# reinterpretcat/qwen3-rs

Measured on NVIDIA B200. Metric: decode_tokens_per_s, higher is better.
Workload: dtype int8 weights x int8 activations, int32 group dots, f32 accumulate

## Files before the change

### qwen3_rs_b200/csrc/q3_engine.cu

```cuda
#include "../../include/qwen3_cuda.h"
#include "q3_kernels.cuh"
#include "q3_mega.cuh"
#include "q3_prefill.cuh"
#include "q3_sampler.cuh"
#include <cudaTypedefs.h>

#include <cuda_runtime.h>
#include <fcntl.h>
#include <math.h>
#include <stdarg.h>
#include <stdio.h>
#include <stdlib.h>
#include <string.h>
#include <sys/mman.h>
#include <sys/stat.h>
#include <unistd.h>

#include <string>
#include <vector>

using namespace q3;

static thread_local char g_err[1024] = "";
static int fail(int code, const char *fmt, ...) {
    va_list ap;
    va_start(ap, fmt);
    vsnprintf(g_err, sizeof g_err, fmt, ap);
    va_end(ap);
    return code;
}
#define CK(call)                                                                                        \
    do {                                                                                                \
        cudaError_t e_ = (call);                                                                        \
        if (e_ != cudaSuccess)                                                                          \
            return fail(Q3_ECUDA, "CUDA error %s at %s:%d: %s", cudaGetErrorName(e_), __FILE__, __LINE__, \
                        cudaGetErrorString(e_));                                                        \
    } while (0)

extern "C" const char *q3_last_error(void) { return g_err; }
extern "C" const char *q3_version(void) { return "qwen3cuda 0.1 (sm_100a)"; }

struct DevQT {
    int8_t *q = nullptr;
    float *s = nullptr;
    int rows = 0, K = 0;
    float *sT = nullptr;
    CUtensorMap map{};
    bool has_map = false;
};

struct LayerDev {
    DevQT qkv;
    DevQT wo;
    DevQT w13;
    DevQT w2;
    float *rms_att = nullptr, *rms_ffn = nullptr, *q_ln = nullptr, *k_ln = nullptr;
};

struct q3_handle {
    q3_config cfg{};
    int device = 0;
    int tp_rank = 0, tp_size = 1;
    int n_heads_l = 0, n_kv_l = 0, AH_l = 0, KV_l = 0, H_l = 0, kv_mul = 1;
    int num_sms = 148;
    std::vector<LayerDev> layers;
    DevQT embed, wcls;
    float *rms_final = nullptr;
    float *rope = nullptr;
    float *x = nullptr, *xb = nullptr, *q = nullptr, *hb = nullptr, *logits = nullptr, *attn_part = nullptr;
    unsigned *att_cnt = nullptr;
    int8_t *xq = nullptr, *hq = nullptr;
    float *xs = nullptr, *hs = nullptr;
    float *kc = nullptr, *vc = nullptr;
    int *d_tokpos = nullptr;
    int *d_history = nullptr;
    int history_cap = 0;
    float *h_logits = nullptr;
    int *h_small = nullptr;
    cudaStream_t stream = nullptr;
    cudaGraphExec_t g_fwd[32] = {}, g_greedy[32] = {};
    int exact = 0;
    float *att = nullptr;
    int decode_path = 0;
    int launches_per_step = 0, graph_launches_per_step = 0;
    bool mega_ok = false;
    std::string mega_why;
    MegaArgs margs{};
    unsigned long long bar_base = 0, xbar_base = 0;
    int *d_status = nullptr;
    unsigned long long *part_buf[2] = {nullptr, nullptr};
    unsigned long long *zq = nullptr, *za = nullptr, *zh = nullptr, *zr[2] = {nullptr, nullptr};
    int logits_root = -1;
    bool poisoned = false;
    unsigned long long *d_best = nullptr, *d_bar = nullptr;
    unsigned int *d_flags = nullptr;
    uint8_t *xchg = nullptr;
    size_t xchg_bytes = 0, off_part[2] = {0, 0}, off_best = 0, off_flags = 0, off_logits = 0;
    size_t off_pf_part[2] = {0, 0}, off_pf_ctr = 0;
    int pf_tp_cap = 0;
    PfPeers pf_peers[2]{};
    unsigned long long pf_xbar_count = 0;
    bool tp_connected = false;
    std::vector<void *> peer_maps;
    size_t mega_smem = 0;
    unsigned long long ll_count = 0;
    void *mega_fn = nullptr;
    bool pf_ok = false;
    std::string pf_why;
    __half *pf_kvh = nullptr;
    size_t pf_kvh_rows = 0;
    int pf_cap = 0;
    float *pf_x = nullptr, *pf_q = nullptr, *pf_att = nullptr, *pf_hb = nullptr, *pf_xsT = nullptr, *pf_hsT = nullptr;
    int8_t *pf_xq = nullptr, *pf_hq = nullptr;
    int *pf_tokens = nullptr;
    float samp_temperature = 0.0f, samp_topp = 0.9f;
    unsigned long long *d_rng = nullptr, *d_keys = nullptr;
    float *d_probs = nullptr;
    size_t dev_bytes = 0;
    std::vector<void *> allocs;
};

static int dmalloc(q3_handle *h, void **p, size_t bytes) {
    CK(cudaMalloc(p, bytes ? bytes : 16));
    h->allocs.push_back(*p);
    h->dev_bytes += bytes;
    return 0;
}

struct HostQT {
    const int8_t *q;
    const float *s;
};
struct Ckpt {
    uint8_t *map = nullptr;
    size_t len = 0, off = 0;
    q3_config cfg{};
    const float *rms_att, *rms_ffn, *rms_final, *q_ln, *k_ln;
    HostQT embed, wcls;
    std::vector<HostQT> wq, wk, wv, wo, w1, w2, w3;
    ~Ckpt() {
        if (map) munmap(map, len);
    }
    const void *take(size_t bytes) {
        if (off + bytes > len) return nullptr;
        const void *p = map + off;
        off += bytes;
        return p;
    }
};

static int open_ckpt(const char *path, int ctx_len, Ckpt &c) {
    int fd = open(path, O_RDONLY);
    if (fd < 0) return fail(Q3_EIO, "Failed to open checkpoint: %s", path);
    struct stat st;
    fstat(fd, &st);
    c.len = (size_t)st.st_size;
    void *m = mmap(nullptr, c.len ? c.len : 1, PROT_READ, MAP_PRIVATE, fd, 0);
    close(fd);
    if (m == MAP_FAILED) return fail(Q3_EIO, "Failed to create memory mapping");
    c.map = (uint8_t *)m;
    const int32_t *hd = (const int32_t *)c.take(13 * 4);
    if (!hd) return fail(Q3_EFORMAT, "Insufficient data for config: need 52 bytes, got %zu", c.len);
    if (hd[0] != 0x616a6331)
        return fail(Q3_EFORMAT, "Invalid checkpoint magic number: expected 0x616a6331, got %#x", hd[0]);
    if (hd[1] != 1) return fail(Q3_EFORMAT, "Unsupported checkpoint version: expected 1, got %d", hd[1]);
    const char *names[8] = {"architecture_id", "dim", "n_layers", "n_heads", "n_kv_heads", "vocab_size", "seq_len", "head_dim"};
    int32_t vals[8] = {hd[2], hd[3], hd[5], hd[6], hd[7], hd[8], hd[9], hd[10]};
    for (int i = 0; i < 8; i++)
        if (vals[i] <= 0) return fail(Q3_EFORMAT, "Invalid %s: must be positive, got %d", names[i], vals[i]);
    if (!c.take(256 - 52)) return fail(Q3_EFORMAT, "Cannot skip %d bytes: insufficient data", 256 - 52);
    q3_config &cf = c.cfg;
    cf.architecture_id = hd[2]; cf.dim = hd[3]; cf.hidden_dim = hd[4]; cf.n_layers = hd[5];
    cf.n_heads = hd[6]; cf.n_kv_heads = hd[7]; cf.vocab_size = hd[8]; cf.seq_len = hd[9];
    cf.head_dim = hd[10]; cf.shared_classifier = hd[11] != 0; cf.group_size = hd[12];
    if (ctx_len > 0 && ctx_len < cf.seq_len) cf.seq_len = ctx_len;
    if (cf.architecture_id != 1) return fail(Q3_EFORMAT, "Unknown architecture_id: %d", cf.architecture_id);
    if (cf.hidden_dim <= 0 || cf.group_size <= 0) return fail(Q3_EFORMAT, "Invalid hidden_dim/group_size");

    const int L = cf.n_layers, dim = cf.dim, hdm = cf.head_dim, gs = cf.group_size;
    const size_t AH = (size_t)cf.n_heads * hdm, KV = (size_t)cf.n_kv_heads * hdm, H = cf.hidden_dim, V = cf.vocab_size;
#define TAKE_F32(dst, n, what)                                                         \
    if (!((dst) = (const float *)c.take((size_t)(n) * 4)))                             \
        return fail(Q3_EFORMAT, "Failed to read %s: Insufficient data", what);
    TAKE_F32(c.rms_att, (size_t)L * dim, "attention normalization weights");
    TAKE_F32(c.rms_ffn, (size_t)L * dim, "FFN normalization weights");
    TAKE_F32(c.rms_final, dim, "final normalization weights");
    TAKE_F32(c.q_ln, (size_t)L * hdm, "query layer norm weights");
    TAKE_F32(c.k_ln, (size_t)L * hdm, "key layer norm weights");
    auto take_qts = [&](std::vector<HostQT> &v, int n, size_t size_each, const char *what) -> int {
        v.resize(n);
        for (int i = 0; i < n; i++) {
            v[i].q = (const int8_t *)c.take(size_each);
            v[i].s = (const float *)c.take(size_each / gs * 4);
            if (!v[i].q || !v[i].s)
                return fail(Q3_EFORMAT, "Failed to read quantized tensor %d data (%s): Insufficient data", i, what);
        }
        return 0;
    };
    std::vector<HostQT> one;
    int rc;
    if ((rc = take_qts(one, 1, V * dim, "token embedding"))) return rc;
    c.embed = one[0];
    if ((rc = take_qts(c.wq, L, (size_t)dim * AH, "wq"))) return rc;
    if ((rc = take_qts(c.wk, L, (size_t)dim * KV, "wk"))) return rc;
    if ((rc = take_qts(c.wv, L, (size_t)dim * KV, "wv"))) return rc;
    if ((rc = take_qts(c.wo, L, AH * dim, "wo"))) return rc;
    if ((rc = take_qts(c.w1, L, (size_t)dim * H, "w1"))) return rc;
    if ((rc = take_qts(c.w2, L, H * dim, "w2"))) return rc;
    if ((rc = take_qts(c.w3, L, (size_t)dim * H, "w3"))) return rc;
    if (cf.shared_classifier) c.wcls = c.embed;
    else {
        if ((rc = take_qts(one, 1, (size_t)dim * V, "classifier"))) return rc;
        c.wcls = one[0];
    }
    return 0;
}

struct Stager {
    uint8_t *buf = nullptr;
    size_t cap = 0;
    ~Stager() {
        if (buf) cudaFreeHost(buf);
    }
    int ensure(size_t n) {
        if (n <= cap) return 0;
        if (buf) cudaFreeHost(buf);
        buf = nullptr;
        cap = 0;
        CK(cudaMallocHost((void **)&buf, n));
        cap = n;
        return 0;
    }
};

struct RowPiece {
    HostQT src;
    int src_row0, nrows, srcK;
};
static int upload_rows(q3_handle *h, Stager &st, DevQT &dst, const std::vector<RowPiece> &pieces, int K, int col0,
                       int gs, bool interleave2 = false) {
    int rows = 0;
    for (auto &p : pieces) rows += p.nrows;
    dst.rows = rows;
    dst.K = K;
    const int ng = K / gs;
    size_t qbytes = (size_t)rows * K, sbytes = (size_t)rows * ng * 4;
    int rc;
    if ((rc = dmalloc(h, (void **)&dst.q, qbytes))) return rc;
    if ((rc = dmalloc(h, (void **)&dst.s, sbytes))) return rc;
    if ((rc = st.ensure(qbytes + sbytes))) return rc;
    int8_t *hq = (int8_t *)st.buf;
    float *hs = (float *)(st.buf + qbytes);
    if (interleave2) {
        const RowPiece &a = pieces[0], &b = pieces[1];
        for (int j = 0; j < a.nrows; j++) {
            const RowPiece *pp[2] = {&a, &b};
            for (int t = 0; t < 2; t++) {
                size_t sr = (size_t)pp[t]->src_row0 + j;
                memcpy(hq + (size_t)(2 * j + t) * K, pp[t]->src.q + sr * pp[t]->srcK + col0, K);
                memcpy(hs + (size_t)(2 * j + t) * ng, pp[t]->src.s + sr * (pp[t]->srcK / gs) + col0 / gs, (size_t)ng * 4);
            }
        }
    } else {
        size_t r = 0;
        for (auto &p : pieces) {
            if (p.srcK == K && col0 == 0) {
                memcpy(hq + r * K, p.src.q + (size_t)p.src_row0 * K, (size_t)p.nrows * K);
                memcpy(hs + r * ng, p.src.s + (size_t)p.src_row0 * ng, (size_t)p.nrows * ng * 4);
            } else {
                for (int j = 0; j < p.nrows; j++) {
                    size_t sr = (size_t)p.src_row0 + j;
                    memcpy(hq + (r + j) * K, p.src.q + sr * p.srcK + col0, K);
                    memcpy(hs + (r + j) * ng, p.src.s + sr * (p.srcK / gs) + col0 / gs, (size_t)ng * 4);
                }
            }
            r += p.nrows;
        }
    }
    CK(cudaMemcpy(dst.q, hq, qbytes, cudaMemcpyHostToDevice));
    CK(cudaMemcpy(dst.s, hs, sbytes, cudaMemcpyHostToDevice));
    return 0;
}
static int upload_f32(q3_handle *h, float **dst, const float *src, size_t n) {
    int rc;
    if ((rc = dmalloc(h, (void **)dst, n * 4))) return rc;
    CK(cudaMemcpy(*dst, src, n * 4, cudaMemcpyHostToDevice));
    return 0;
}

#define GS_DISPATCH(gs, CALL)                \
    switch (gs) {                            \
    case 32: { constexpr int GS = 32; CALL; } break;   \
    case 64: { constexpr int GS = 64; CALL; } break;   \
    case 128: { constexpr int GS = 128; CALL; } break; \
    default: break;                          \
    }

template <int GS, int EPI>
static void launch_gemv_t(const q3_handle *h, GemvArgs a, cudaStream_t s) {
    int npairs = a.rows / 2;
    int grid = (npairs + 7) / 8;
    int cap = h->num_sms * 8;
    if (grid > cap) grid = cap;
    if (grid < 1) grid = 1;
    size_t smem = (size_t)a.K + (size_t)(a.K / GS) * 4;
    const bool expref = EPI == EPI_SWIGLU && (h->exact & 16);
    if (h->exact & 2) {
        smem += (size_t)16 * (a.K / GS) * 4;
        if (expref) k_gemv<GS, EPI, true, true><<<grid, 256, smem, s>>>(a);
        else k_gemv<GS, EPI, true, false><<<grid, 256, smem, s>>>(a);
    } else {
        if (expref) k_gemv<GS, EPI, false, true><<<grid, 256, smem, s>>>(a);
        else k_gemv<GS, EPI, false, false><<<grid, 256, smem, s>>>(a);
    }
}
template <int EPI>
static void launch_gemv(const q3_handle *h, const GemvArgs &a, cudaStream_t s) {
    GS_DISPATCH(h->cfg.group_size, (launch_gemv_t<GS, EPI>(h, a, s)));
}

static int launch_norm_quant(const q3_handle *h, const NormQuantArgs &a, cudaStream_t s) {
    if (h->exact & 1) {
        GS_DISPATCH(h->cfg.group_size, (k_rmsnorm_quant<GS, true><<<1, 1024, (size_t)a.n * 4, s>>>(a)));
    } else {
        GS_DISPATCH(h->cfg.group_size, (k_rmsnorm_quant<GS, false><<<1, 1024, 0, s>>>(a)));
    }
    return 1;
}

static int launch_layer(q3_handle *h, int l, bool first_from_embed, cudaStream_t s) {
    const q3_config &c = h->cfg;
    const LayerDev &W = h->layers[l];
    const int gs = c.group_size, dim = c.dim;
    const int *d_token = h->d_tokpos, *d_pos = h->d_tokpos + 1;
    float *kc_l = h->kc + (size_t)l * c.seq_len * h->KV_l;
    float *vc_l = h->vc + (size_t)l * c.seq_len * h->KV_l;
    int n = 0;
    NormQuantArgs na{};
    na.x = h->x; na.w = W.rms_att; na.q = h->xq; na.s = h->xs; na.n = dim;
    if (first_from_embed) { na.embed_q = h->embed.q; na.embed_s = h->embed.s; na.token = d_token; }
    n += launch_norm_quant(h, na, s);
    GemvArgs g{};
    g.wq = W.qkv.q; g.ws = W.qkv.s; g.xq = h->xq; g.xs = h->xs; g.K = dim; g.rows = W.qkv.rows;
    g.q = h->q; g.kc = kc_l; g.vc = vc_l; g.AH = h->AH_l; g.KV = h->KV_l; g.pos = d_pos;
    launch_gemv<EPI_QKV>(h, g, s); n++;
    int nh = h->n_heads_l + h->n_kv_l;
    if (h->exact & 4)
        k_qknorm_rope<true><<<(nh + 3) / 4, 128, 0, s>>>(h->q, kc_l, W.q_ln, W.k_ln, h->rope, d_pos, h->n_heads_l, h->n_kv_l, h->KV_l);
    else
        k_qknorm_rope<false><<<(nh + 3) / 4, 128, 0, s>>>(h->q, kc_l, W.q_ln, W.k_ln, h->rope, d_pos, h->n_heads_l, h->n_kv_l, h->KV_l);
    n++;
    dim3 ag(h->n_kv_l, ATTN_MAX_SPLITS);
    if (h->exact & 8) {
        k_attn_ordered<<<h->n_heads_l, 128, 0, s>>>(h->q, kc_l, vc_l, h->att, h->xb, d_pos, h->KV_l, h->kv_mul, c.seq_len);
        int n4 = h->AH_l / 4, grid = (n4 + 255) / 256;
        GS_DISPATCH(gs, (k_quantize<GS><<<grid, 256, 0, s>>>(h->xb, h->AH_l, h->xq, h->xs)));
        n += 2;
    } else {
    switch (h->kv_mul) {
    case 1: k_attn_partial<1><<<ag, 128, 0, s>>>(h->q, kc_l, vc_l, h->attn_part, d_pos, h->KV_l, h->n_heads_l); break;
    case 2: k_attn_partial<2><<<ag, 128, 0, s>>>(h->q, kc_l, vc_l, h->attn_part, d_pos, h->KV_l, h->n_heads_l); break;
    case 4: k_attn_partial<4><<<ag, 128, 0, s>>>(h->q, kc_l, vc_l, h->attn_part, d_pos, h->KV_l, h->n_heads_l); break;
    case 8: k_attn_partial<8><<<ag, 128, 0, s>>>(h->q, kc_l, vc_l, h->attn_part, d_pos, h->KV_l, h->n_heads_l); break;
    }
    n++;
    GS_DISPATCH(gs, (k_attn_combine_quant<GS><<<h->n_heads_l, 128, 0, s>>>(h->attn_part, d_pos, h->xb, h->xq, h->xs)));
    n++;
    }
    GemvArgs o{};
    o.wq = W.wo.q; o.ws = W.wo.s; o.xq = h->xq; o.xs = h->xs; o.K = h->AH_l; o.rows = dim; o.out = h->x;
    launch_gemv<EPI_RESID>(h, o, s); n++;
    NormQuantArgs nf{};
    nf.x = h->x; nf.w = W.rms_ffn; nf.q = h->xq; nf.s = h->xs; nf.n = dim;
    n += launch_norm_quant(h, nf, s);
    GemvArgs gu{};
    gu.wq = W.w13.q; gu.ws = W.w13.s; gu.xq = h->xq; gu.xs = h->xs; gu.K = dim; gu.rows = W.w13.rows; gu.out = h->hb;
    launch_gemv<EPI_SWIGLU>(h, gu, s); n++;
    {
        int n4 = h->H_l / 4, grid = (n4 + 255) / 256;
        GS_DISPATCH(gs, (k_quantize<GS><<<grid, 256, 0, s>>>(h->hb, h->H_l, h->hq, h->hs)));
        n++;
    }
    GemvArgs dn{};
    dn.wq = W.w2.q; dn.ws = W.w2.s; dn.xq = h->hq; dn.xs = h->hs; dn.K = h->H_l; dn.rows = dim; dn.out = h->x;
    launch_gemv<EPI_RESID>(h, dn, s); n++;
    return n;
}

static int launch_head(q3_handle *h, cudaStream_t s) {
    const q3_config &c = h->cfg;
    NormQuantArgs na{};
    na.x = h->x; na.w = h->rms_final; na.q = h->xq; na.s = h->xs; na.n = c.dim; na.write_normed = 1;
    int n = launch_norm_quant(h, na, s);
    GemvArgs g{};
    g.wq = h->wcls.q; g.ws = h->wcls.s; g.xq = h->xq; g.xs = h->xs; g.K = c.dim; g.rows = c.vocab_size; g.out = h->logits;
    launch_gemv<EPI_STORE>(h, g, s); n++;
    return n;
}

static int launch_argmax(q3_handle *h, bool feedback, cudaStream_t s) {
    int *tp = h->d_tokpos;
    k_argmax<<<1, 1024, 0, s>>>(h->logits, h->cfg.vocab_size, tp + 2, feedback ? tp : nullptr, feedback ? tp + 1 : nullptr,
                                feedback ? h->d_history : nullptr, tp + 3);
    return 1;
}

static int launch_step(q3_handle *h, bool argmax, bool feedback, cudaStream_t s) {
    int n = 0;
    for (int l = 0; l < h->cfg.n_layers; l++) n += launch_layer(h, l, l == 0, s);
    n += launch_head(h, s);
    if (argmax) n += launch_argmax(h, feedback, s);
    return n;
}

static int build_graphs(q3_handle *h) {
    const int ex = h->exact;
    for (int which = 0; which < 2; which++) {
        cudaGraphExec_t *slot = which ? &h->g_greedy[ex] : &h->g_fwd[ex];
        cudaGraph_t g;
        CK(cudaStreamBeginCapture(h->stream, cudaStreamCaptureModeThreadLocal));
        int n = launch_step(h, which == 1, which == 1, h->stream);
        cudaError_t e = cudaStreamEndCapture(h->stream, &g);
        if (e != cudaSuccess) return fail(Q3_ECUDA, "graph capture failed: %s", cudaGetErrorString(e));
        if (!*slot) CK(cudaGraphInstantiate(slot, g, 0));
        CK(cudaGraphDestroy(g));
        if (which == 1) h->launches_per_step = n;
    }
    return 0;
}

template <class K>
static int allow_smem(K kernel, int bytes) {
    CK(cudaFuncSetAttribute(kernel, cudaFuncAttributeMaxDynamicSharedMemorySize, bytes));
    return 0;
}
static int prepare_exact_kernels() {
    int rc;
    if ((rc = allow_smem(k_rmsnorm_quant<32, true>, 65536))) return rc;
    if ((rc = allow_smem(k_rmsnorm_quant<64, true>, 65536))) return rc;
    if ((rc = allow_smem(k_rmsnorm_quant<128, true>, 65536))) return rc;
#define ALLOW_GEMV(GS)                                                      \
    if ((rc = allow_smem(k_gemv<GS, EPI_STORE, true, false>, 131072))) return rc;  \
    if ((rc = allow_smem(k_gemv<GS, EPI_QKV, true, false>, 131072))) return rc;    \
    if ((rc = allow_smem(k_gemv<GS, EPI_RESID, true, false>, 131072))) return rc;  \
    if ((rc = allow_smem(k_gemv<GS, EPI_SWIGLU, true, false>, 131072))) return rc; \
    if ((rc = allow_smem(k_gemv<GS, EPI_SWIGLU, true, true>, 131072))) return rc;  \
    if ((rc = allow_smem(k_gemv<GS, EPI_STORE, false, false>, 98304))) return rc;  \
    if ((rc = allow_smem(k_gemv<GS, EPI_QKV, false, false>, 98304))) return rc;    \
    if ((rc = allow_smem(k_gemv<GS, EPI_RESID, false, false>, 98304))) return rc;  \
    if ((rc = allow_smem(k_gemv<GS, EPI_SWIGLU, false, false>, 98304))) return rc; \
    if ((rc = allow_smem(k_gemv<GS, EPI_SWIGLU, false, true>, 98304))) return rc;
    ALLOW_GEMV(32)
    ALLOW_GEMV(64)
    ALLOW_GEMV(128)
#undef ALLOW_GEMV
    return 0;
}

static int pick_n_kt(int K, int gs) {
    for (int n = (K + MEGA_MAX_KT - 1) / MEGA_MAX_KT; n <= 64; n++)
        if (K % (n * gs) == 0 && (K / n) % 16 == 0 && K / n <= MEGA_MAX_KT) return n;
    return 0;
}

template <int GS>
static void *mega_kernel_for(int kvmul) {
    switch (kvmul) {
    case 1: return (void *)k_mega_decode<GS, 1>;
    case 2: return (void *)k_mega_decode<GS, 2>;
    case 4: return (void *)k_mega_decode<GS, 4>;
    case 8: return (void *)k_mega_decode<GS, 8>;
    }
    return nullptr;
}

static int build_stream(q3_handle *h, MegaGemv &g, const std::vector<const DevQT *> &src, int units, int K, bool pair) {
    const int gs = h->cfg.group_size;
    g.units = units;
    g.K = K;
    g.n_kt = pick_n_kt(K, gs);
    if (!g.n_kt) return fail(Q3_EUNSUPPORTED, "no K tiling for K=%d gs=%d", K, gs);
    g.KT = K / g.n_kt;
    g.G = g.KT / gs;
    g.tile_bytes = g.KT + ((4 * g.G + 15) & ~15);
    const size_t rows = (size_t)units * (pair ? 2 : 1);
    g.layer_stride = (long long)(rows * g.n_kt * g.tile_bytes);
    uint8_t *buf = nullptr;
    int rc;
    if ((rc = dmalloc(h, (void **)&buf, (size_t)g.layer_stride * src.size()))) return rc;
    g.base = buf;
    for (size_t l = 0; l < src.size(); l++) {
        dim3 grid(units, g.n_kt);
        GS_DISPATCH(gs, (k_build_stream<GS><<<grid, 256, 0, h->stream>>>(src[l]->q, src[l]->s, buf + l * g.layer_stride, units, K,
                                                                        g.n_kt, h->num_sms, pair ? 1 : 0)));
    }
    CK(cudaGetLastError());
    return 0;
}

static PFN_cuTensorMapEncodeTiled_v12000 get_encode_fn();
static int make_map_kv(CUtensorMap *map, const float *base, size_t rows, int KV_l) {
    auto enc = get_encode_fn();
    if (!enc) return fail(Q3_ECUDA, "cuTensorMapEncodeTiled unavailable");
    cuuint64_t dims[2] = {(cuuint64_t)KV_l, (cuuint64_t)rows};
    cuuint64_t strides[1] = {(cuuint64_t)KV_l * 4};
    cuuint32_t box[2] = {(cuuint32_t)HEAD_DIM, (cuuint32_t)MEGA_KV_ROWS};
    cuuint32_t estr[2] = {1, 1};
    CUresult r = enc(map, CU_TENSOR_MAP_DATA_TYPE_FLOAT32, 2, const_cast<float *>(base), dims, strides, box, estr, CU_TENSOR_MAP_INTERLEAVE_NONE,
                     CU_TENSOR_MAP_SWIZZLE_NONE, CU_TENSOR_MAP_L2_PROMOTION_L2_128B, CU_TENSOR_MAP_FLOAT_OOB_FILL_NONE);
    if (r != CUDA_SUCCESS) return fail(Q3_ECUDA, "cuTensorMapEncodeTiled (KV cache) failed (%d) rows %zu KV %d", (int)r, rows, KV_l);
    return 0;
}

static int build_mega(q3_handle *h, const float *rms_att_all, const float *rms_ffn_all, const float *q_ln_all, const float *k_ln_all) {
    const q3_config &c = h->cfg;
    const int gs = c.group_size, L = c.n_layers, dim = c.dim;
    h->mega_ok = false;
    if (dim > MEGA_MAX_KT) { h->mega_why = "dim > 4096 (QKV/gate-up/lm_head phases need a single K tile)"; return 0; }
    if (!pick_n_kt(h->AH_l, gs) || !pick_n_kt(h->H_l, gs)) { h->mega_why = "no K tiling for o_proj/down"; return 0; }
    if (h->AH_l > 16384 || h->H_l > 16384 || dim > 16384) { h->mega_why = "activation vector > 16384"; return 0; }
    if (c.vocab_size % h->tp_size) { h->mega_why = "vocab not divisible by tp"; return 0; }
    if (h->layers[0].qkv.rows < h->num_sms || h->H_l < h->num_sms) { h->mega_why = "fewer qkv rows / FFN units than SMs"; return 0; }
    if (!get_encode_fn()) { h->mega_why = "cuTensorMapEncodeTiled unavailable"; return 0; }
    MegaArgs &a = h->margs;
    a = MegaArgs{};
    {
        int rck;
        if ((rck = make_map_kv(&a.map_k, h->kc, (size_t)L * c.seq_len, h->KV_l))) return rck;
        if ((rck = make_map_kv(&a.map_v, h->vc, (size_t)L * c.seq_len, h->KV_l))) return rck;
    }
    a.dim = dim; a.n_layers = L; a.n_heads_l = h->n_heads_l; a.n_kv_l = h->n_kv_l; a.AH_l = h->AH_l; a.KV_l = h->KV_l;
    a.H_l = h->H_l; a.seq_len = c.seq_len; a.tp_rank = h->tp_rank; a.tp_size = h->tp_size;
    a.vocab_l = c.vocab_size / h->tp_size;
    a.vocab_row0 = a.vocab_l * h->tp_rank;
    int rc;
    std::vector<const DevQT *> v;
    for (auto &W : h->layers) v.push_back(&W.qkv);
    if ((rc = build_stream(h, a.g[PH_QKV], v, h->layers[0].qkv.rows, dim, false))) return rc;
    v.clear();
    for (auto &W : h->layers) v.push_back(&W.wo);
    if ((rc = build_stream(h, a.g[PH_O], v, dim, h->AH_l, false))) return rc;
    v.clear();
    for (auto &W : h->layers) v.push_back(&W.w13);
    if ((rc = build_stream(h, a.g[PH_GU], v, h->H_l, dim, true))) return rc;
    v.clear();
    for (auto &W : h->layers) v.push_back(&W.w2);
    if ((rc = build_stream(h, a.g[PH_DN], v, dim, h->H_l, false))) return rc;
    DevQT head_slice = h->wcls;
    head_slice.q = h->wcls.q + (size_t)a.vocab_row0 * dim;
    head_slice.s = h->wcls.s + (size_t)a.vocab_row0 * (dim / gs);
    v.assign(1, &head_slice);
    if ((rc = build_stream(h, a.g[PH_HEAD], v, a.vocab_l, dim, false))) return rc;
    CK(cudaStreamSynchronize(h->stream));
    float *p;
    if ((rc = upload_f32(h, &p, rms_att_all, (size_t)L * dim))) return rc; a.rms_att = p;
    if ((rc = upload_f32(h, &p, rms_ffn_all, (size_t)L * dim))) return rc; a.rms_ffn = p;
    if ((rc = upload_f32(h, &p, q_ln_all, (size_t)L * HEAD_DIM))) return rc; a.q_ln = p;
    if ((rc = upload_f32(h, &p, k_ln_all, (size_t)L * HEAD_DIM))) return rc; a.k_ln = p;
    a.rms_final = h->rms_final;
    a.embed_q = h->embed.q; a.embed_s = h->embed.s; a.rope = h->rope; a.kc = h->kc; a.vc = h->vc;
    for (int i = 0; i < 2; i++) h->part_buf[i] = (unsigned long long *)(h->xchg + h->off_part[i]);
    {
        struct { unsigned long long **p; size_t words; } zones[] = {
            {&h->zq, (size_t)h->AH_l + 2 * (size_t)h->KV_l},
            {&h->za, (size_t)h->AH_l / 4 + (size_t)h->AH_l / gs},
            {&h->zh, (size_t)h->H_l},
            {&h->zr[0], (size_t)dim},
            {&h->zr[1], (size_t)dim}};
        for (auto &z : zones) {
            if ((rc = dmalloc(h, (void **)z.p, (z.words + 2) * 8))) return rc;
            CK(cudaMemset(*z.p, 0, (z.words + 2) * 8));
        }
    }
    h->d_best = (unsigned long long *)(h->xchg + h->off_best);
    h->d_flags = (unsigned int *)(h->xchg + h->off_flags);
    if ((rc = dmalloc(h, (void **)&h->d_bar, 64))) return rc;
    CK(cudaMemset(h->d_bar, 0, 64));
    if ((rc = dmalloc(h, (void **)&h->d_status, 64))) return rc;
    CK(cudaMemset(h->d_status, 0, 64));
    int *d_status = h->d_status;
    a.x = h->x;
    a.zq = h->zq; a.za = h->za; a.zh = h->zh; a.zr[0] = h->zr[0]; a.zr[1] = h->zr[1];
    a.attn_part = h->attn_part; a.att_cnt = h->att_cnt;
    a.bar = h->d_bar; a.status = d_status; a.tokpos = h->d_tokpos; a.history = h->d_history;
    for (int r = 0; r < MEGA_MAX_TP; r++) {
        a.part[0][r] = h->part_buf[0]; a.part[1][r] = h->part_buf[1];
        a.logits[r] = h->logits; a.best[r] = h->d_best; a.xbar[r] = (unsigned long long *)h->d_flags;
    }
    GS_DISPATCH(gs, (h->mega_fn = mega_kernel_for<GS>(h->kv_mul)));
    if (!h->mega_fn) { h->mega_why = "no kernel for this GQA factor"; return 0; }
    const size_t slot = (size_t)MEGA_GW * (MEGA_MAX_KT + 4 * (MEGA_MAX_KT / gs));
    h->mega_smem = MEGA_NSTAGE * slot + MEGA_SCRATCH + 1024 + MEGA_MAX_KT * 4;
    CK(cudaFuncSetAttribute(h->mega_fn, cudaFuncAttributeMaxDynamicSharedMemorySize, (int)h->mega_smem));
    int occ = 0;
    CK(cudaOccupancyMaxActiveBlocksPerMultiprocessor(&occ, h->mega_fn, MEGA_THREADS, h->mega_smem));
    if (occ < 1) { h->mega_why = "megakernel does not fit on an SM"; return 0; }
    h->mega_ok = true;
    return 0;
}

static int launch_mega(q3_handle *h, int l0, int l1, bool from_embed, bool run_head, bool feedback, bool gather) {
    MegaArgs a = h->margs;
    a.layer0 = l0; a.layer1 = l1; a.from_embed = from_embed; a.run_head = run_head; a.feedback = feedback;
    a.gather_logits = h->tp_size > 1 ? (h->logits_root >= 0 ? (1 << h->logits_root) : (gather ? (1 << h->tp_size) - 1 : 0)) : 0;
    a.bar_base = h->bar_base;
    a.xbar_base = h->xbar_base;
    if (h->poisoned) return fail(Q3_ECOMM, "tensor-parallel handle is unusable after a timed-out wait (ranks may have diverged): destroy and re-create every rank");
    const int nbar = run_head ? 1 : 0;
    const int nx = h->tp_size > 1 ? nbar : 0;
    a.ll_base = (unsigned)(h->ll_count % 0xFFFFFFFFull);
    h->ll_count += (unsigned long long)MEGA_EDGES * (unsigned)(l1 - l0 + 1);
    void *params[] = {&a};
    CK(cudaLaunchCooperativeKernel(h->mega_fn, dim3(h->num_sms), dim3(MEGA_THREADS), params, h->mega_smem, h->stream));
    h->bar_base += (unsigned long long)(nbar - nx) * h->num_sms;
    h->xbar_base += (unsigned long long)nx * h->tp_size * h->num_sms;
    return 0;
}

static int check_tok_pos(const q3_handle *h, int token, int pos);
static int mega_status_async(q3_handle *h) {
    if (!h->d_status || h->decode_path != 1) return 0;
    CK(cudaMemcpyAsync(h->h_small + 16, h->d_status, 4, cudaMemcpyDeviceToHost, h->stream));
    return 0;
}
static int mega_check(q3_handle *h, bool queued = false) {
    if (!h->d_status || h->decode_path != 1) return 0;
    int code = 0;
    if (queued) code = h->h_small[16];
    else CK(cudaMemcpy(&code, h->d_status, 4, cudaMemcpyDeviceToHost));
    if (code) {
        cudaMemset(h->d_status, 0, 64);
        if (h->tp_size > 1) {
            h->poisoned = true;
        } else {
            h->bar_base = 0;
            h->xbar_base = 0;
            cudaMemset(h->d_bar, 0, 64);
            cudaMemset(h->d_flags, 0, 64 * 4);
            if (h->att_cnt) cudaMemset(h->att_cnt, 0, (size_t)h->cfg.n_layers * h->n_kv_l * 4);
        }
        return fail(Q3_ECUDA, "persistent decode kernel: a wait timed out (status %d: 1 grid barrier, 2 stage ring, 3 cross-GPU barrier, 4 producer order, "
                              "6-10 flagged exchange: 6 o/down rows, 7 attention output, 8 SwiGLU outputs, 9 qkv rows, 10 TP partials; 11 prefill cross-GPU barrier)%s", code,
                    h->tp_size > 1 ? "; tensor-parallel handle poisoned" : "");
    }
    return 0;
}
extern "C" int q3_debug_profile(q3_handle *h, int token, int pos, unsigned long long *out, size_t out_words, int *n_rows_out,
                                int *n_events_out) {
    if (!h) return fail(Q3_EINVAL, "null argument");
    if (n_rows_out) *n_rows_out = 3 * h->num_sms;
    if (n_events_out) *n_events_out = MEGA_PROF_EVENTS;
    if (!out) return out_words == 0 ? Q3_OK : fail(Q3_EINVAL, "null argument");
    if (!h->mega_ok) return fail(Q3_EUNSUPPORTED, "persistent decode kernel unavailable: %s", h->mega_why.c_str());
    if (out_words < (size_t)3 * h->num_sms * MEGA_PROF_EVENTS)
        return fail(Q3_EINVAL, "profile buffer too small: %zu words, need %zu", out_words, (size_t)3 * h->num_sms * MEGA_PROF_EVENTS);
    if (int rc0 = check_tok_pos(h, token, pos)) return rc0;
    CK(cudaSetDevice(h->device));
    h->h_small[0] = token; h->h_small[1] = pos; h->h_small[2] = 0; h->h_small[3] = 0;
    CK(cudaMemcpyAsync(h->d_tokpos, h->h_small, 16, cudaMemcpyHostToDevice, h->stream));
    unsigned long long *d = nullptr;
    size_t bytes = (size_t)3 * h->num_sms * MEGA_PROF_EVENTS * 8;
    CK(cudaMalloc((void **)&d, bytes));
    CK(cudaMemsetAsync(d, 0, bytes, h->stream));
    h->margs.prof = d;
    int rc = launch_mega(h, 0, h->cfg.n_layers, true, true, false, false);
    h->margs.prof = nullptr;
    if (!rc) {
        cudaError_t e = cudaStreamSynchronize(h->stream);
        if (e == cudaSuccess) e = cudaMemcpy(out, d, bytes, cudaMemcpyDeviceToHost);
        if (e != cudaSuccess) rc = fail(Q3_ECUDA, "profile run failed: %s", cudaGetErrorString(e));
    }
    cudaFree(d);
    if (!rc) rc = mega_check(h);
    return rc;
}
extern "C" int q3_num_sms(const q3_handle *h) { return h ? h->num_sms : 0; }
extern "C" int q3_debug_set_epoch(q3_handle *h, unsigned long long exchanges_issued) {
    if (!h) return fail(Q3_EINVAL, "null handle");
    h->ll_count = exchanges_issued;
    return Q3_OK;
}

static inline bool use_mega(const q3_handle *h) { return h->decode_path == 1 && h->mega_ok && !h->exact; }
static int tp_ready(const q3_handle *h) {
    if (h->tp_size > 1 && !h->tp_connected) return fail(Q3_ECOMM, "tensor-parallel handle used before q3_tp_connect");
    if (h->tp_size > 1 && !use_mega(h)) return fail(Q3_EUNSUPPORTED, "under tensor parallelism only the persistent fast path is available");
    return 0;
}

static PFN_cuTensorMapEncodeTiled_v12000 get_encode_fn() {
    static PFN_cuTensorMapEncodeTiled_v12000 fn = nullptr;
    if (!fn) {
        void *p = nullptr;
        cudaDriverEntryPointQueryResult qres;
        if (cudaGetDriverEntryPoint("cuTensorMapEncodeTiled", &p, cudaEnableDefault, &qres) == cudaSuccess && qres == cudaDriverEntryPointSuccess)
            fn = (PFN_cuTensorMapEncodeTiled_v12000)p;
    }
    return fn;
}
static int make_map_i8(CUtensorMap *map, const void *base, int rows, int K) {
    auto enc = get_encode_fn();
    if (!enc) return fail(Q3_ECUDA, "cuTensorMapEncodeTiled unavailable");
    cuuint64_t dims[2] = {(cuuint64_t)K, (cuuint64_t)rows};
    cuuint64_t strides[1] = {(cuuint64_t)K};
    cuuint32_t box[2] = {(cuuint32_t)PF_BK, (cuuint32_t)PF_BM};
    cuuint32_t estr[2] = {1, 1};
    CUresult r = enc(map, CU_TENSOR_MAP_DATA_TYPE_UINT8, 2, const_cast<void *>(base), dims, strides, box, estr,
                     CU_TENSOR_MAP_INTERLEAVE_NONE, CU_TENSOR_MAP_SWIZZLE_128B, CU_TENSOR_MAP_L2_PROMOTION_L2_256B,
                     CU_TENSOR_MAP_FLOAT_OOB_FILL_NONE);
    if (r != CUDA_SUCCESS) return fail(Q3_ECUDA, "cuTensorMapEncodeTiled failed (%d) rows %d K %d", (int)r, rows, K);
    return 0;
}

static int make_map_scales(CUtensorMap *map, const float *base, int groups, int cols) {
    auto enc = get_encode_fn();
    if (!enc) return fail(Q3_ECUDA, "cuTensorMapEncodeTiled unavailable");
    cuuint64_t dims[2] = {(cuuint64_t)cols, (cuuint64_t)groups};
    cuuint64_t strides[1] = {(cuuint64_t)cols * 4};
    cuuint32_t box[2] = {128, 2};
    cuuint32_t estr[2] = {1, 1};
    CUresult r = enc(map, CU_TENSOR_MAP_DATA_TYPE_FLOAT32, 2, const_cast<float *>(base), dims, strides, box, estr, CU_TENSOR_MAP_INTERLEAVE_NONE,
                     CU_TENSOR_MAP_SWIZZLE_NONE, CU_TENSOR_MAP_L2_PROMOTION_L2_128B, CU_TENSOR_MAP_FLOAT_OOB_FILL_NONE);
    if (r != CUDA_SUCCESS) return fail(Q3_ECUDA, "cuTensorMapEncodeTiled (scales) failed (%d) groups %d cols %d", (int)r, groups, cols);
    return 0;
}

template <int GS, int EPI, bool EXACT>
static int launch_gemm_q8_t(const CUtensorMap &mx, const CUtensorMap &mw, const PrefillGemmArgs &a, cudaStream_t s) {
    static bool attr = false;
    if (!attr) {
        CK(cudaFuncSetAttribute(k_gemm_q8<GS, EPI, EXACT>, cudaFuncAttributeMaxDynamicSharedMemorySize, PF_SMEM));
        attr = true;
    }
    static int num_sms = 0;
    if (!num_sms) {
        int dev = 0;
        CK(cudaGetDevice(&dev));
        CK(cudaDeviceGetAttribute(&num_sms, cudaDevAttrMultiProcessorCount, dev));
    }
    CUtensorMap mxs, mws;
    int rc;
    if ((rc = make_map_scales(&mxs, a.xsT, a.K / GS, a.Tpad)) || (rc = make_map_scales(&mws, a.wsT, a.K / GS, a.N))) return rc;
    const int tiles = (a.N / PF_BN) * (a.Tpad / PF_BM);
    k_gemm_q8<GS, EPI, EXACT><<<tiles < num_sms ? tiles : num_sms, PF_THREADS, PF_SMEM, s>>>(mx, mw, mxs, mws, a);
    return 0;
}
template <int EPI>
static int launch_gemm_q8(int gs, const CUtensorMap &mx, const CUtensorMap &mw, const PrefillGemmArgs &a, cudaStream_t s, int mode = 0) {
    int rc = 0;
    if (mode == 0) {
        GS_DISPATCH(gs, (rc = launch_gemm_q8_t<GS, EPI, false>(mx, mw, a, s)));
    } else if (mode == 1 && EPI == PF_EPI_STORE) {
        GS_DISPATCH(gs, (rc = launch_gemm_q8_t<GS, PF_EPI_STORE, true>(mx, mw, a, s)));
    } else {
        return fail(Q3_EINVAL, "prefill GEMM mode %d: 0 = fast drain, 1 = exact drain (plain store epilogue only)", mode);
    }
    return rc;
}

static int prefill_prepare_tensor(q3_handle *h, DevQT &t) {
    if (t.has_map) return 0;
    const int gs = h->cfg.group_size, ng = t.K / gs;
    int rc;
    if ((rc = dmalloc(h, (void **)&t.sT, (size_t)ng * t.rows * 4))) return rc;
    dim3 grid((ng + 31) / 32, (t.rows + 31) / 32);
    k_transpose_f32<<<grid, dim3(32, 8), 0, h->stream>>>(t.s, t.sT, t.rows, ng);
    CK(cudaGetLastError());
    if ((rc = make_map_i8(&t.map, t.q, t.rows, t.K))) return rc;
    t.has_map = true;
    return 0;
}

static int prefill_init(q3_handle *h) {
    const q3_config &c = h->cfg;
    h->pf_ok = false;
    if (c.dim % 128 || h->AH_l % 128 || h->H_l % 128 || h->layers[0].qkv.rows % 128 || (2 * h->H_l) % 128) {
        h->pf_why = "matrix dimensions must be multiples of 128";
        return 0;
    }
    if ((c.dim / c.group_size) % 2 || (h->AH_l / c.group_size) % 2 || (h->H_l / c.group_size) % 2) {
        h->pf_why = "the tensor-core GEMM hands accumulators over in pairs: rows need an even number of quantisation groups";
        return 0;
    }
    if (!get_encode_fn()) { h->pf_why = "cuTensorMapEncodeTiled unavailable"; return 0; }
    CK(cudaFuncSetAttribute(k_pf_attention_h<1>, cudaFuncAttributeMaxDynamicSharedMemorySize, PFH_SMEM));
    CK(cudaFuncSetAttribute(k_pf_attention_h<2>, cudaFuncAttributeMaxDynamicSharedMemorySize, PFH_SMEM));
    CK(cudaFuncSetAttribute(k_pf_attention_h<4>, cudaFuncAttributeMaxDynamicSharedMemorySize, PFH_SMEM));
    CK(cudaFuncSetAttribute(k_pf_attention_h<8>, cudaFuncAttributeMaxDynamicSharedMemorySize, PFH_SMEM));
    int rc;
    for (auto &W : h->layers) {
        if ((rc = prefill_prepare_tensor(h, W.qkv))) return rc;
        if ((rc = prefill_prepare_tensor(h, W.wo))) return rc;
        if ((rc = prefill_prepare_tensor(h, W.w13))) return rc;
        if ((rc = prefill_prepare_tensor(h, W.w2))) return rc;
    }
    CK(cudaStreamSynchronize(h->stream));
    h->pf_ok = true;
    return 0;
}

static void prefill_release(q3_handle *h) {
    if (h->pf_kvh) cudaFree(h->pf_kvh);
    h->pf_kvh = nullptr;
    h->pf_kvh_rows = 0;
    void **ps[] = {(void **)&h->pf_x, (void **)&h->pf_q, (void **)&h->pf_att, (void **)&h->pf_hb, (void **)&h->pf_xsT, (void **)&h->pf_hsT,
                   (void **)&h->pf_xq, (void **)&h->pf_hq, (void **)&h->pf_tokens};
    for (void **p : ps) {
        if (*p) cudaFree(*p);
        *p = nullptr;
    }
    h->pf_cap = 0;
}
static int prefill_reserve(q3_handle *h, int T) {
    const int Tpad = (T + 127) / 128 * 128;
    if (Tpad <= h->pf_cap) return 0;
    const q3_config &c = h->cfg;
    const int gs = c.group_size, dim = c.dim, AH = h->AH_l, H = h->H_l;
    const int maxd = AH > dim ? AH : dim;
    prefill_release(h);
    struct { void **p; size_t bytes; } want[] = {
        {(void **)&h->pf_x, (size_t)Tpad * dim * 4},          {(void **)&h->pf_q, (size_t)Tpad * AH * 4},
        {(void **)&h->pf_att, (size_t)Tpad * AH * 4},         {(void **)&h->pf_hb, (size_t)Tpad * H * 4},
        {(void **)&h->pf_xsT, (size_t)(maxd / gs) * Tpad * 4}, {(void **)&h->pf_hsT, (size_t)(H / gs) * Tpad * 4},
        {(void **)&h->pf_xq, (size_t)Tpad * maxd},            {(void **)&h->pf_hq, (size_t)Tpad * H},
        {(void **)&h->pf_tokens, (size_t)Tpad * 4}};
    for (auto &w : want) {
        cudaError_t e = cudaMalloc(w.p, w.bytes);
        if (e != cudaSuccess) {
            *w.p = nullptr;
            prefill_release(h);
            cudaGetLastError();
            return fail(Q3_ECUDA, "prefill buffers for %d tokens: %s", T, cudaGetErrorString(e));
        }
    }
    CK(cudaMemset(h->pf_xq, 0, (size_t)Tpad * maxd));
    CK(cudaMemset(h->pf_hq, 0, (size_t)Tpad * H));
    CK(cudaMemset(h->pf_xsT, 0, (size_t)(maxd / gs) * Tpad * 4));
    CK(cudaMemset(h->pf_hsT, 0, (size_t)(H / gs) * Tpad * 4));
    h->pf_cap = Tpad;
    return 0;
}

static int prefill_tp_rowparallel(q3_handle *h, int which, const CUtensorMap &mx, const CUtensorMap &mw, PrefillGemmArgs g, int T) {
    int rc;
    g.out = const_cast<float *>(h->pf_peers[which].part[h->tp_rank]);
    if ((rc = launch_gemm_q8<PF_EPI_STORE>(h->cfg.group_size, mx, mw, g, h->stream))) return rc;
    h->pf_xbar_count++;
    k_pf_xbarrier<<<1, 32, 0, h->stream>>>(h->pf_peers[which], h->tp_size, h->tp_rank, h->pf_xbar_count * (unsigned long long)h->tp_size, h->d_status);
    const size_t n4 = (size_t)T * h->cfg.dim / 4;
    if (h->tp_size > 2) {
        k_pf_reduce_scatter<<<h->num_sms * 2, 256, 0, h->stream>>>(h->pf_peers[which], g.out, h->tp_size, h->tp_rank, n4);
        h->pf_xbar_count++;
        k_pf_xbarrier<<<1, 32, 0, h->stream>>>(h->pf_peers[which], h->tp_size, h->tp_rank, h->pf_xbar_count * (unsigned long long)h->tp_size, h->d_status);
        k_pf_allgather_resid<<<dim3(h->num_sms / 2, h->tp_size), 256, 0, h->stream>>>(h->pf_x, h->pf_peers[which], h->tp_size, n4);
    } else {
        k_pf_allreduce_resid<<<h->num_sms * 4, 256, 0, h->stream>>>(h->pf_x, h->pf_peers[which], h->tp_size, n4);
    }
    CK(cudaGetLastError());
    return 0;
}

static int prefill_run(q3_handle *h, const int *tokens_host, int T, int pos0);
static int prefill_chunks(q3_handle *h, const int *tokens_host, int n, int pos0) {
    const int cap = h->tp_size > 1 ? h->pf_tp_cap : n;
    for (int off = 0; off < n; off += cap) {
        int rc = prefill_run(h, tokens_host + off, n - off < cap ? n - off : cap, pos0 + off);
        if (rc) return rc;
    }
    return 0;
}

static int prefill_run(q3_handle *h, const int *tokens_host, int T, int pos0) {
    const q3_config &c = h->cfg;
    const int gs = c.group_size, dim = c.dim, AH = h->AH_l, KV = h->KV_l, H = h->H_l;
    int rc;
    if ((rc = prefill_reserve(h, T))) return rc;
    if ((size_t)pos0 + T > h->pf_kvh_rows) {
        if (h->pf_kvh) cudaFree(h->pf_kvh);
        h->pf_kvh = nullptr;
        h->pf_kvh_rows = 0;
        const size_t rows = ((size_t)pos0 + T + 127) / 128 * 128;
        cudaError_t e = cudaMalloc((void **)&h->pf_kvh, 4 * rows * KV * sizeof(__half));
        if (e != cudaSuccess) {
            h->pf_kvh = nullptr;
            cudaGetLastError();
            return fail(Q3_ECUDA, "prefill K/V split buffer for %zu rows: %s", rows, cudaGetErrorString(e));
        }
        h->pf_kvh_rows = rows;
    }
    const int Tpad = (T + 127) / 128 * 128;
    cudaStream_t s = h->stream;
    CK(cudaMemcpyAsync(h->pf_tokens, tokens_host, (size_t)T * 4, cudaMemcpyHostToDevice, s));
    CUtensorMap mx_dim, mx_ah, mx_h;
    if ((rc = make_map_i8(&mx_dim, h->pf_xq, Tpad, dim))) return rc;
    if ((rc = make_map_i8(&mx_ah, h->pf_xq, Tpad, AH))) return rc;
    if ((rc = make_map_i8(&mx_h, h->pf_hq, Tpad, H))) return rc;
    for (int l = 0; l < c.n_layers; l++) {
        LayerDev &W = h->layers[l];
        float *kc_l = h->kc + (size_t)l * c.seq_len * KV;
        float *vc_l = h->vc + (size_t)l * c.seq_len * KV;
        if (dim <= 4096) {
            GS_DISPATCH(gs, (k_pf_norm_quant<GS, 4><<<T, 256, 0, s>>>(h->pf_x, W.rms_att, h->pf_xq, h->pf_xsT, dim, Tpad,
                                                                     l == 0 ? h->embed.q : nullptr, h->embed.s, h->pf_tokens, 0)));
        } else {
            GS_DISPATCH(gs, (k_pf_norm_quant<GS><<<T, 256, 0, s>>>(h->pf_x, W.rms_att, h->pf_xq, h->pf_xsT, dim, Tpad,
                                                                  l == 0 ? h->embed.q : nullptr, h->embed.s, h->pf_tokens, 0)));
        }
        PrefillGemmArgs g{};
        g.T = T; g.Tpad = Tpad; g.K = dim; g.N = W.qkv.rows; g.wsT = W.qkv.sT; g.xsT = h->pf_xsT;
        g.q = h->pf_q; g.kc = kc_l; g.vc = vc_l; g.AH = AH; g.KV = KV; g.pos0 = pos0;
        if ((rc = launch_gemm_q8<PF_EPI_QKV>(gs, mx_dim, W.qkv.map, g, s))) return rc;
        dim3 rg((h->n_heads_l + h->n_kv_l + 3) / 4, T);
        k_pf_qknorm_rope<<<rg, 128, 0, s>>>(h->pf_q, kc_l, W.q_ln, W.k_ln, h->rope, pos0, h->n_heads_l, h->n_kv_l, AH, KV);
        const size_t rows = (size_t)pos0 + T, plane = h->pf_kvh_rows * KV;
        k_pf_split_kv<<<h->num_sms * 4, 256, 0, s>>>(kc_l, vc_l, h->pf_kvh, rows * KV / 4, plane);
        const int bq = PFH_R / h->kv_mul;
        dim3 ag(h->n_kv_l, (T + bq - 1) / bq);
        switch (h->kv_mul) {
        case 1: k_pf_attention_h<1><<<ag, 128, PFH_SMEM, s>>>(h->pf_q, h->pf_kvh, plane, h->pf_att, T, pos0, AH, KV); break;
        case 2: k_pf_attention_h<2><<<ag, 128, PFH_SMEM, s>>>(h->pf_q, h->pf_kvh, plane, h->pf_att, T, pos0, AH, KV); break;
        case 4: k_pf_attention_h<4><<<ag, 128, PFH_SMEM, s>>>(h->pf_q, h->pf_kvh, plane, h->pf_att, T, pos0, AH, KV); break;
        case 8: k_pf_attention_h<8><<<ag, 128, PFH_SMEM, s>>>(h->pf_q, h->pf_kvh, plane, h->pf_att, T, pos0, AH, KV); break;
        }
        GS_DISPATCH(gs, (k_pf_quantize<GS><<<T, 256, 0, s>>>(h->pf_att, h->pf_xq, h->pf_xsT, AH, Tpad)));
        PrefillGemmArgs o{};
        o.T = T; o.Tpad = Tpad; o.K = AH; o.N = dim; o.wsT = W.wo.sT; o.xsT = h->pf_xsT; o.out = h->pf_x; o.ld_out = dim;
        if (h->tp_size == 1) {
            if ((rc = launch_gemm_q8<PF_EPI_RESID>(gs, mx_ah, W.wo.map, o, s))) return rc;
        } else if ((rc = prefill_tp_rowparallel(h, 0, mx_ah, W.wo.map, o, T))) return rc;
        if (dim <= 4096) {
            GS_DISPATCH(gs, (k_pf_norm_quant<GS, 4><<<T, 256, 0, s>>>(h->pf_x, W.rms_ffn, h->pf_xq, h->pf_xsT, dim, Tpad, nullptr, nullptr, nullptr, 0)));
        } else {
            GS_DISPATCH(gs, (k_pf_norm_quant<GS><<<T, 256, 0, s>>>(h->pf_x, W.rms_ffn, h->pf_xq, h->pf_xsT, dim, Tpad, nullptr, nullptr, nullptr, 0)));
        }
        PrefillGemmArgs gu{};
        gu.T = T; gu.Tpad = Tpad; gu.K = dim; gu.N = W.w13.rows; gu.wsT = W.w13.sT; gu.xsT = h->pf_xsT; gu.out = h->pf_hb; gu.ld_out = H;
        if ((rc = launch_gemm_q8<PF_EPI_SWIGLU>(gs, mx_dim, W.w13.map, gu, s))) return rc;
        GS_DISPATCH(gs, (k_pf_quantize<GS><<<T, 256, 0, s>>>(h->pf_hb, h->pf_hq, h->pf_hsT, H, Tpad)));
        PrefillGemmArgs dn{};
        dn.T = T; dn.Tpad = Tpad; dn.K = H; dn.N = dim; dn.wsT = W.w2.sT; dn.xsT = h->pf_hsT; dn.out = h->pf_x; dn.ld_out = dim;
        if (h->tp_size == 1) {
            if ((rc = launch_gemm_q8<PF_EPI_RESID>(gs, mx_h, W.w2.map, dn, s))) return rc;
        } else if ((rc = prefill_tp_rowparallel(h, 1, mx_h, W.w2.map, dn, T))) return rc;
    }
    CK(cudaMemcpyAsync(h->x, h->pf_x + (size_t)(T - 1) * dim, (size_t)dim * 4, cudaMemcpyDeviceToDevice, s));
    CK(cudaGetLastError());
    return 0;
}

static int create_impl(const char *path, int ctx_len, int device, int tp_rank, int tp_size, q3_handle **out) {
    if (!path || !out) return fail(Q3_EINVAL, "null argument");
    if (tp_size < 1 || tp_rank < 0 || tp_rank >= tp_size) return fail(Q3_EINVAL, "bad tp rank/size %d/%d", tp_rank, tp_size);
    *out = nullptr;
    Ckpt ck;
    int rc = open_ckpt(path, ctx_len, ck);
    if (rc) return rc;
    const q3_config &c = ck.cfg;
    const int gs = c.group_size;
    if (c.head_dim != HEAD_DIM) return fail(Q3_EUNSUPPORTED, "head_dim %d unsupported (kernels are built for 128)", c.head_dim);
    if (gs != 32 && gs != 64 && gs != 128) return fail(Q3_EUNSUPPORTED, "group_size %d unsupported (32/64/128)", gs);
    if (c.n_heads % c.n_kv_heads) return fail(Q3_EUNSUPPORTED, "n_heads %% n_kv_heads != 0");
    int kv_mul = c.n_heads / c.n_kv_heads;
    if (kv_mul != 1 && kv_mul != 2 && kv_mul != 4 && kv_mul != 8) return fail(Q3_EUNSUPPORTED, "GQA factor %d unsupported", kv_mul);
    if (c.dim % 128 || c.hidden_dim % 128) return fail(Q3_EUNSUPPORTED, "dim/hidden_dim must be multiples of 128");
    if (c.dim > 16384 || c.hidden_dim > 65536) return fail(Q3_EUNSUPPORTED, "dim/hidden_dim too large");
    if (c.n_kv_heads % tp_size || (c.hidden_dim / tp_size) % gs || c.hidden_dim % tp_size)
        return fail(Q3_EUNSUPPORTED, "tp_size %d does not divide kv heads / hidden groups", tp_size);
    if (c.vocab_size % 2) return fail(Q3_EUNSUPPORTED, "odd vocab_size");

    int ndev = 0;
    CK(cudaGetDeviceCount(&ndev));
    if (device < 0 || device >= ndev) return fail(Q3_EINVAL, "device %d out of range (%d visible)", device, ndev);
    CK(cudaSetDevice(device));
    q3_handle *h = new q3_handle();
    h->cfg = c;
    h->device = device;
    h->tp_rank = tp_rank;
    h->tp_size = tp_size;
    h->kv_mul = kv_mul;
    h->n_heads_l = c.n_heads / tp_size;
    h->n_kv_l = c.n_kv_heads / tp_size;
    h->AH_l = h->n_heads_l * HEAD_DIM;
    h->KV_l = h->n_kv_l * HEAD_DIM;
    h->H_l = c.hidden_dim / tp_size;
    cudaDeviceProp prop;
    cudaGetDeviceProperties(&prop, device);
    h->num_sms = prop.multiProcessorCount;

    auto guard_fail = [&](int code) {
        q3_destroy(h);
        return code;
    };
#define TRY(x)                         \
    do {                               \
        int rc_ = (x);                 \
        if (rc_) return guard_fail(rc_); \
    } while (0)
#define CKH(call)                                                                                         \
    do {                                                                                                  \
        cudaError_t e_ = (call);                                                                          \
        if (e_ != cudaSuccess)                                                                            \
            return guard_fail(fail(Q3_ECUDA, "CUDA error %s at %s:%d: %s", cudaGetErrorName(e_), __FILE__, \
                                   __LINE__, cudaGetErrorString(e_)));                                    \
    } while (0)

    CKH(cudaStreamCreateWithFlags(&h->stream, cudaStreamNonBlocking));
    const int L = c.n_layers, dim = c.dim, H = c.hidden_dim;
    const int AH = c.n_heads * HEAD_DIM;
    Stager st;
    h->layers.resize(L);
    const int r = tp_rank;
    for (int l = 0; l < L; l++) {
        LayerDev &W = h->layers[l];
        TRY(upload_rows(h, st, W.qkv,
                        {{ck.wq[l], r * h->AH_l, h->AH_l, dim}, {ck.wk[l], r * h->KV_l, h->KV_l, dim}, {ck.wv[l], r * h->KV_l, h->KV_l, dim}},
                        dim, 0, gs));
        TRY(upload_rows(h, st, W.wo, {{ck.wo[l], 0, dim, AH}}, h->AH_l, r * h->AH_l, gs));
        TRY(upload_rows(h, st, W.w13, {{ck.w1[l], r * h->H_l, h->H_l, dim}, {ck.w3[l], r * h->H_l, h->H_l, dim}}, dim, 0, gs, true));
        TRY(upload_rows(h, st, W.w2, {{ck.w2[l], 0, dim, H}}, h->H_l, r * h->H_l, gs));
        TRY(upload_f32(h, &W.rms_att, ck.rms_att + (size_t)l * dim, dim));
        TRY(upload_f32(h, &W.rms_ffn, ck.rms_ffn + (size_t)l * dim, dim));
        TRY(upload_f32(h, &W.q_ln, ck.q_ln + (size_t)l * HEAD_DIM, HEAD_DIM));
        TRY(upload_f32(h, &W.k_ln, ck.k_ln + (size_t)l * HEAD_DIM, HEAD_DIM));
    }
    TRY(upload_rows(h, st, h->embed, {{ck.embed, 0, c.vocab_size, dim}}, dim, 0, gs));
    if (c.shared_classifier) h->wcls = h->embed;
    else TRY(upload_rows(h, st, h->wcls, {{ck.wcls, 0, c.vocab_size, dim}}, dim, 0, gs));
    TRY(upload_f32(h, &h->rms_final, ck.rms_final, dim));

    {
        size_t n = (size_t)c.seq_len * HEAD_DIM;
        std::vector<float> tab(n);
        const int half = HEAD_DIM / 2;
        std::vector<float> freq(half);
        for (int i = 0; i < half; i++) freq[i] = powf(1e6f, -((float)i) / (float)half);
        for (int p = 0; p < c.seq_len; p++)
            for (int i = 0; i < half; i++) {
                float ang = (float)p * freq[i];
                tab[(size_t)p * HEAD_DIM + 2 * i] = cosf(ang);
                tab[(size_t)p * HEAD_DIM + 2 * i + 1] = sinf(ang);
            }
        TRY(upload_f32(h, &h->rope, tab.data(), n));
    }
    const int maxd = (h->AH_l > dim ? h->AH_l : dim);
    TRY(dmalloc(h, (void **)&h->x, (size_t)dim * 4));
    TRY(dmalloc(h, (void **)&h->xb, (size_t)maxd * 4));
    TRY(dmalloc(h, (void **)&h->q, (size_t)h->AH_l * 4));
    TRY(dmalloc(h, (void **)&h->hb, (size_t)h->H_l * 4));
    {
        auto al = [](size_t v) { return (v + 255) & ~(size_t)255; };
        size_t o = 0;
        h->off_part[0] = o; o = al(o + (size_t)tp_size * dim * 8);
        h->off_part[1] = o; o = al(o + (size_t)tp_size * dim * 8);
        h->off_best = o; o = al(o + (size_t)tp_size * h->num_sms * 8);
        h->off_flags = o; o = al(o + 64 * 4);
        h->off_logits = o; o = al(o + (size_t)c.vocab_size * 4);
        if (tp_size > 1) {
            h->pf_tp_cap = c.seq_len < 2048 ? (c.seq_len + 127) / 128 * 128 : 2048;
            h->off_pf_ctr = o; o = al(o + 64);
            for (int i = 0; i < 2; i++) { h->off_pf_part[i] = o; o = al(o + (size_t)h->pf_tp_cap * dim * 4); }
        }
        h->xchg_bytes = o;
        TRY(dmalloc(h, (void **)&h->xchg, o));
        CKH(cudaMemset(h->xchg, 0, o));
        h->logits = (float *)(h->xchg + h->off_logits);
    }
    TRY(dmalloc(h, (void **)&h->xq, (size_t)maxd));
    TRY(dmalloc(h, (void **)&h->xs, (size_t)(maxd / gs + 1) * 4));
    TRY(dmalloc(h, (void **)&h->hq, (size_t)h->H_l));
    TRY(dmalloc(h, (void **)&h->hs, (size_t)(h->H_l / gs + 1) * 4));
    TRY(dmalloc(h, (void **)&h->attn_part, (size_t)h->n_heads_l * ATTN_MAX_SPLITS * ATTN_PART_STRIDE * 4));
    TRY(dmalloc(h, (void **)&h->att_cnt, (size_t)h->cfg.n_layers * h->n_kv_l * 4));
    CKH(cudaMemset(h->att_cnt, 0, (size_t)h->cfg.n_layers * h->n_kv_l * 4));
    TRY(dmalloc(h, (void **)&h->att, (size_t)h->n_heads_l * c.seq_len * 4));
    TRY(prepare_exact_kernels());
    size_t kvn = (size_t)L * c.seq_len * h->KV_l;
    TRY(dmalloc(h, (void **)&h->kc, kvn * 4));
    TRY(dmalloc(h, (void **)&h->vc, kvn * 4));
    CKH(cudaMemset(h->kc, 0, kvn * 4));
    CKH(cudaMemset(h->vc, 0, kvn * 4));
    h->history_cap = c.seq_len + 8;
    TRY(dmalloc(h, (void **)&h->d_tokpos, 16 * 4));
    TRY(dmalloc(h, (void **)&h->d_history, (size_t)h->history_cap * 4));
    CKH(cudaMemset(h->d_tokpos, 0, 16 * 4));
    CKH(cudaMemset(h->x, 0, (size_t)dim * 4));
    CKH(cudaMallocHost((void **)&h->h_logits, (size_t)c.vocab_size * 4));
    CKH(cudaMallocHost((void **)&h->h_small, 64 * 4));
    CKH(cudaDeviceSynchronize());
    TRY(build_graphs(h));
    h->graph_launches_per_step = h->launches_per_step;
    TRY(build_mega(h, ck.rms_att, ck.rms_ffn, ck.q_ln, ck.k_ln));
    if (h->mega_ok) {
        h->decode_path = 1;
        h->launches_per_step = 1;
    }
    TRY(prefill_init(h));
    CKH(cudaDeviceSynchronize());
    *out = h;
    return Q3_OK;
}

extern "C" int q3_create(const char *path, int ctx_len, int device, q3_handle **out) {
    return create_impl(path, ctx_len, device, 0, 1, out);
}
extern "C" int q3_create_tp(const char *path, int ctx_len, int device, int tp_rank, int tp_size, q3_handle **out) {
    if (tp_size > MEGA_MAX_TP) return fail(Q3_EUNSUPPORTED, "tp_size %d > %d", tp_size, MEGA_MAX_TP);
    int rc = create_impl(path, ctx_len, device, tp_rank, tp_size, out);
    if (rc) return rc;
    if (tp_size > 1 && !(*out)->mega_ok) {
        std::string why = (*out)->mega_why;
        q3_destroy(*out);
        *out = nullptr;
        return fail(Q3_EUNSUPPORTED, "tensor parallelism needs the persistent decode kernel, unavailable here: %s", why.c_str());
    }
    return Q3_OK;
}

struct TpBlob {
    uint32_t magic, rank, tp_size, device;
    uint64_t pid, raw_ptr, bytes;
    cudaIpcMemHandle_t ipc;
};
static_assert(sizeof(TpBlob) <= 256, "blob too large");
extern "C" size_t q3_tp_blob_size(void) { return 256; }

extern "C" int q3_tp_export(q3_handle *h, void *blob_out) {
    if (!h || !blob_out) return fail(Q3_EINVAL, "null argument");
    CK(cudaSetDevice(h->device));
    memset(blob_out, 0, 256);
    TpBlob b{};
    b.magic = 0x51335450;
    b.rank = h->tp_rank; b.tp_size = h->tp_size; b.device = h->device;
    b.pid = (uint64_t)getpid();
    b.raw_ptr = (uint64_t)(uintptr_t)h->xchg;
    b.bytes = h->xchg_bytes;
    CK(cudaIpcGetMemHandle(&b.ipc, h->xchg));
    memcpy(blob_out, &b, sizeof b);
    return Q3_OK;
}

extern "C" int q3_tp_connect(q3_handle *h, const void *blobs) {
    if (!h || !blobs) return fail(Q3_EINVAL, "null argument");
    if (h->tp_size == 1) return Q3_OK;
    CK(cudaSetDevice(h->device));
    MegaArgs &a = h->margs;
    for (int r = 0; r < h->tp_size; r++) {
        TpBlob b;
        memcpy(&b, (const uint8_t *)blobs + (size_t)r * 256, sizeof b);
        if (b.magic != 0x51335450 || (int)b.rank != r || (int)b.tp_size != h->tp_size || b.bytes != h->xchg_bytes)
            return fail(Q3_ECOMM, "rank %d: bad exchange blob (rank %u, tp %u, %llu bytes)", r, b.rank, b.tp_size,
                        (unsigned long long)b.bytes);
        uint8_t *base = nullptr;
        if (r == h->tp_rank) {
            base = h->xchg;
        } else if (b.pid == (uint64_t)getpid()) {
            int can = 0;
            CK(cudaDeviceCanAccessPeer(&can, h->device, (int)b.device));
            if (!can) return fail(Q3_ECOMM, "device %d cannot access peer device %u", h->device, b.device);
            cudaError_t e = cudaDeviceEnablePeerAccess((int)b.device, 0);
            if (e != cudaSuccess && e != cudaErrorPeerAccessAlreadyEnabled)
                return fail(Q3_ECOMM, "cudaDeviceEnablePeerAccess: %s", cudaGetErrorString(e));
            cudaGetLastError();
            base = (uint8_t *)(uintptr_t)b.raw_ptr;
        } else {
            void *p = nullptr;
            cudaError_t e = cudaIpcOpenMemHandle(&p, b.ipc, cudaIpcMemLazyEnablePeerAccess);
            if (e != cudaSuccess) return fail(Q3_ECOMM, "cudaIpcOpenMemHandle(rank %d): %s", r, cudaGetErrorString(e));
            h->peer_maps.push_back(p);
            base = (uint8_t *)p;
        }
        a.part[0][r] = (unsigned long long *)(base + h->off_part[0]);
        a.part[1][r] = (unsigned long long *)(base + h->off_part[1]);
        a.best[r] = (unsigned long long *)(base + h->off_best);
        a.xbar[r] = (unsigned long long *)(base + h->off_flags);
        a.logits[r] = (float *)(base + h->off_logits);
        for (int i = 0; i < 2; i++) {
            h->pf_peers[i].part[r] = (const float *)(base + h->off_pf_part[i]);
            h->pf_peers[i].ctr[r] = (unsigned long long *)(base + h->off_pf_ctr);
        }
    }
    h->tp_connected = true;
    return Q3_OK;
}

extern "C" int q3_tp_set_logits_root(q3_handle *h, int root) {
    if (!h) return fail(Q3_EINVAL, "null handle");
    if (root >= h->tp_size) return fail(Q3_EINVAL, "logits root %d outside the tensor-parallel group of %d", root, h->tp_size);
    h->logits_root = root < 0 ? -1 : root;
    return Q3_OK;
}

extern "C" void q3_destroy(q3_handle *h) {
    if (!h) return;
    cudaSetDevice(h->device);
    if (h->stream) cudaStreamSynchronize(h->stream);
    for (int e = 0; e < 32; e++) {
        if (h->g_fwd[e]) cudaGraphExecDestroy(h->g_fwd[e]);
        if (h->g_greedy[e]) cudaGraphExecDestroy(h->g_greedy[e]);
    }
    prefill_release(h);
    for (void *p : h->peer_maps) cudaIpcCloseMemHandle(p);
    for (void *p : h->allocs) cudaFree(p);
    if (h->h_logits) cudaFreeHost(h->h_logits);
    if (h->h_small) cudaFreeHost(h->h_small);
    if (h->stream) cudaStreamDestroy(h->stream);
    delete h;
}

extern "C" const q3_config *q3_get_config(const q3_handle *h) { return h ? &h->cfg : nullptr; }
extern "C" const float *q3_logits_device(const q3_handle *h) { return h ? h->logits : nullptr; }
extern "C" float *q3_logits_host(q3_handle *h) { return h ? h->h_logits : nullptr; }
extern "C" int q3_launches_per_step(const q3_handle *h) { return h ? h->launches_per_step : 0; }
extern "C" int q3_set_decode_path(q3_handle *h, int path) {
    if (!h) return fail(Q3_EINVAL, "null handle");
    if (path != 0 && path != 1) return fail(Q3_EINVAL, "decode path %d unknown", path);
    if (path == 0 && h->tp_size > 1) return fail(Q3_EUNSUPPORTED, "the multi-kernel path has no tensor-parallel exchange");
    if (path == 1 && !h->mega_ok)
        return fail(Q3_EUNSUPPORTED, "persistent decode kernel unavailable for this shape: %s", h->mega_why.c_str());
    h->decode_path = path;
    h->launches_per_step = path == 1 ? 1 : h->graph_launches_per_step;
    return Q3_OK;
}

extern "C" int q3_set_exact_mask(q3_handle *h, int mask) {
    if (!h) return fail(Q3_EINVAL, "null handle");
    if (mask < 0 || mask > 31) return fail(Q3_EINVAL, "exact mask %d outside 0..31", mask);
    CK(cudaSetDevice(h->device));
    if (mask && h->tp_size > 1) return fail(Q3_EUNSUPPORTED, "exact mode is single-GPU");
    if (mask && h->cfg.dim > 16384) return fail(Q3_EUNSUPPORTED, "exact mode needs dim <= 16384");
    h->exact = mask;
    if (!h->g_fwd[h->exact]) return build_graphs(h);
    return Q3_OK;
}
extern "C" int q3_set_exact(q3_handle *h, int on) { return q3_set_exact_mask(h, on ? 31 : 0); }

static int check_tok_pos(const q3_handle *h, int token, int pos) {
    if (!h) return fail(Q3_EINVAL, "null handle");
    if (int rc = tp_ready(h)) return rc;
    if (token < 0 || token >= h->cfg.vocab_size)
        return fail(Q3_EINVAL, "index out of bounds: token %d >= vocab_size %d", token, h->cfg.vocab_size);
    if (pos < 0 || pos >= h->cfg.seq_len)
        return fail(Q3_EINVAL, "index out of bounds: pos %d >= seq_len %d", pos, h->cfg.seq_len);
    return 0;
}

static int set_tok_pos(q3_handle *h, int token, int pos) {
    h->h_small[0] = token;
    h->h_small[1] = pos;
    h->h_small[2] = 0;
    h->h_small[3] = 0;
    CK(cudaMemcpyAsync(h->d_tokpos, h->h_small, 16, cudaMemcpyHostToDevice, h->stream));
    return 0;
}

extern "C" int q3_forward(q3_handle *h, int token, int pos, float *logits_host) {
    int rc = check_tok_pos(h, token, pos);
    if (rc) return rc;
    CK(cudaSetDevice(h->device));
    if ((rc = set_tok_pos(h, token, pos))) return rc;
    if (logits_host && h->tp_size > 1 && h->logits_root >= 0 && h->logits_root != h->tp_rank)
        return fail(Q3_EINVAL, "rank %d asked for logits but the logits root is rank %d", h->tp_rank, h->logits_root);
    if (use_mega(h)) {
        if ((rc = launch_mega(h, 0, h->cfg.n_layers, true, true, false, logits_host != nullptr))) return rc;
    } else {
        CK(cudaGraphLaunch(h->g_fwd[h->exact], h->stream));
    }
    if ((rc = mega_status_async(h))) return rc;
    if (logits_host) {
        CK(cudaMemcpyAsync(h->h_logits, h->logits, (size_t)h->cfg.vocab_size * 4, cudaMemcpyDeviceToHost, h->stream));
        CK(cudaStreamSynchronize(h->stream));
        if (logits_host != h->h_logits) memcpy(logits_host, h->h_logits, (size_t)h->cfg.vocab_size * 4);
    } else {
        CK(cudaStreamSynchronize(h->stream));
    }
    return mega_check(h, true);
}

extern "C" int q3_forward_argmax(q3_handle *h, int token, int pos, int *next_token) {
    int rc = check_tok_pos(h, token, pos);
    if (rc) return rc;
    if (!next_token) return fail(Q3_EINVAL, "null next_token");
    CK(cudaSetDevice(h->device));
    if ((rc = set_tok_pos(h, token, pos))) return rc;
    if (use_mega(h)) {
        if ((rc = launch_mega(h, 0, h->cfg.n_layers, true, true, true, false))) return rc;
    } else {
        CK(cudaGraphLaunch(h->g_greedy[h->exact], h->stream));
    }
    CK(cudaMemcpyAsync(h->h_small + 8, h->d_tokpos + 2, 4, cudaMemcpyDeviceToHost, h->stream));
    if ((rc = mega_status_async(h))) return rc;
    CK(cudaStreamSynchronize(h->stream));
    *next_token = h->h_small[8];
    return mega_check(h, true);
}

extern "C" int q3_decode_greedy(q3_handle *h, int first_token, int pos0, int n, int *tokens_out) {
    int rc = check_tok_pos(h, first_token, pos0);
    if (rc) return rc;
    if (n < 0 || pos0 + n > h->cfg.seq_len) return fail(Q3_EINVAL, "pos0 + n = %d exceeds seq_len %d", pos0 + n, h->cfg.seq_len);
    if (n > h->history_cap) return fail(Q3_EINVAL, "n too large");
    CK(cudaSetDevice(h->device));
    if ((rc = set_tok_pos(h, first_token, pos0))) return rc;
    for (int i = 0; i < n; i++) {
        if (use_mega(h)) {
            if ((rc = launch_mega(h, 0, h->cfg.n_layers, true, true, true, false))) return rc;
        } else {
            CK(cudaGraphLaunch(h->g_greedy[h->exact], h->stream));
        }
    }
    if (tokens_out && n > 0) {
        CK(cudaMemcpyAsync(tokens_out, h->d_history, (size_t)n * 4, cudaMemcpyDeviceToHost, h->stream));
    }
    CK(cudaStreamSynchronize(h->stream));
    return mega_check(h);
}

static size_t next_pow2(size_t n) {
    size_t p = 1;
    while (p < n) p <<= 1;
    return p;
}
extern "C" int q3_sampler_set(q3_handle *h, float temperature, float topp, unsigned long long rng_seed) {
    if (!h) return fail(Q3_EINVAL, "null handle");
    if (!(temperature >= 0.0f)) return fail(Q3_EINVAL, "Temperature must be non-negative");
    if (!(topp >= 0.0f && topp <= 1.0f)) return fail(Q3_EINVAL, "Top-p must be between 0.0 and 1.0");
    CK(cudaSetDevice(h->device));
    int rc;
    if (!h->d_rng) {
        if ((rc = dmalloc(h, (void **)&h->d_rng, 64))) return rc;
        if ((rc = dmalloc(h, (void **)&h->d_probs, (size_t)h->cfg.vocab_size * 4))) return rc;
        if ((rc = dmalloc(h, (void **)&h->d_keys, next_pow2((size_t)h->cfg.vocab_size) * 8))) return rc;
    }
    h->samp_temperature = temperature;
    h->samp_topp = topp;
    CK(cudaMemcpyAsync(h->d_rng, &rng_seed, 8, cudaMemcpyHostToDevice, h->stream));
    CK(cudaStreamSynchronize(h->stream));
    return Q3_OK;
}
extern "C" int q3_sampler_state(q3_handle *h, unsigned long long *rng_state_out) {
    if (!h || !rng_state_out) return fail(Q3_EINVAL, "null argument");
    if (!h->d_rng) return fail(Q3_EINVAL, "q3_sampler_set has not been called");
    CK(cudaSetDevice(h->device));
    CK(cudaStreamSynchronize(h->stream));
    CK(cudaMemcpy(rng_state_out, h->d_rng, 8, cudaMemcpyDeviceToHost));
    return Q3_OK;
}
extern "C" int q3_sampler_skip(q3_handle *h, int n_draws) {
    if (!h || n_draws < 0) return fail(Q3_EINVAL, "bad argument");
    if (!h->d_rng) return fail(Q3_EINVAL, "q3_sampler_set has not been called");
    CK(cudaSetDevice(h->device));
    if (h->samp_temperature != 0.0f && n_draws > 0) k_rng_skip<<<1, 1, 0, h->stream>>>(h->d_rng, n_draws);
    CK(cudaGetLastError());
    return Q3_OK;
}
static int launch_sampled_step(q3_handle *h, bool feedback) {
    int rc;
    const bool greedy = h->samp_temperature == 0.0f;
    if (use_mega(h)) {
        if ((rc = launch_mega(h, 0, h->cfg.n_layers, true, true, greedy && feedback, !greedy))) return rc;
    } else if (greedy) {
        if (feedback) CK(cudaGraphLaunch(h->g_greedy[h->exact], h->stream));
        else {
            CK(cudaGraphLaunch(h->g_fwd[h->exact], h->stream));
            launch_argmax(h, false, h->stream);
        }
    } else {
        CK(cudaGraphLaunch(h->g_fwd[h->exact], h->stream));
    }
    if (!greedy) {
        SampleArgs a{};
        a.logits = h->logits; a.n = h->cfg.vocab_size; a.temperature = h->samp_temperature; a.topp = h->samp_topp;
        a.rng_state = h->d_rng; a.p = h->d_probs; a.keys = h->d_keys; a.token_out = h->d_tokpos + 2;
        if (feedback) { a.token_feedback = h->d_tokpos; a.pos_advance = h->d_tokpos + 1; a.history = h->d_history; a.history_idx = h->d_tokpos + 3; }
        k_sample<<<1, SAMPLE_THREADS, 0, h->stream>>>(a);
        CK(cudaGetLastError());
    }
    return 0;
}
extern "C" int q3_forward_sample(q3_handle *h, int token, int pos, int *next_token) {
    int rc = check_tok_pos(h, token, pos);
    if (rc) return rc;
    if (!next_token) return fail(Q3_EINVAL, "null next_token");
    if (!h->d_rng) return fail(Q3_EINVAL, "q3_sampler_set has not been called");
    CK(cudaSetDevice(h->device));
    if ((rc = set_tok_pos(h, token, pos))) return rc;
    if ((rc = launch_sampled_step(h, false))) return rc;
    CK(cudaMemcpyAsync(h->h_small + 8, h->d_tokpos + 2, 4, cudaMemcpyDeviceToHost, h->stream));
    if ((rc = mega_status_async(h))) return rc;
    CK(cudaStreamSynchronize(h->stream));
    *next_token = h->h_small[8];
    return mega_check(h, true);
}
extern "C" int q3_decode_sample(q3_handle *h, int first_token, int pos0, int n, int *tokens_out) {
    int rc = check_tok_pos(h, first_token, pos0);
    if (rc) return rc;
    if (n < 0 || pos0 + n > h->cfg.seq_len) return fail(Q3_EINVAL, "pos0 + n = %d exceeds seq_len %d", pos0 + n, h->cfg.seq_len);
    if (n > h->history_cap) return fail(Q3_EINVAL, "n too large");
    if (!h->d_rng) return fail(Q3_EINVAL, "q3_sampler_set has not been called");
    CK(cudaSetDevice(h->device));
    if ((rc = set_tok_pos(h, first_token, pos0))) return rc;
    for (int i = 0; i < n; i++)
        if ((rc = launch_sampled_step(h, true))) return rc;
    if (tokens_out && n > 0) CK(cudaMemcpyAsync(tokens_out, h->d_history, (size_t)n * 4, cudaMemcpyDeviceToHost, h->stream));
    CK(cudaStreamSynchronize(h->stream));
    return mega_check(h);
}

extern "C" int q3_bench_decode(q3_handle *h, int first_token, int pos0, int steps, float *ms_out) {
    int rc = check_tok_pos(h, first_token, pos0);
    if (rc) return rc;
    if (steps < 1 || pos0 + steps > h->cfg.seq_len) return fail(Q3_EINVAL, "pos0 + steps exceeds seq_len");
    CK(cudaSetDevice(h->device));
    if ((rc = set_tok_pos(h, first_token, pos0))) return rc;
    cudaEvent_t e0, e1;
    CK(cudaEventCreate(&e0));
    CK(cudaEventCreate(&e1));
    CK(cudaStreamSynchronize(h->stream));
    CK(cudaEventRecord(e0, h->stream));
    for (int i = 0; i < steps; i++) {
        if (use_mega(h)) {
            if ((rc = launch_mega(h, 0, h->cfg.n_layers, true, true, true, false))) return rc;
        } else {
            CK(cudaGraphLaunch(h->g_greedy[h->exact], h->stream));
        }
    }
    CK(cudaEventRecord(e1, h->stream));
    CK(cudaEventSynchronize(e1));
    float ms = 0;
    CK(cudaEventElapsedTime(&ms, e0, e1));
    cudaEventDestroy(e0);
    cudaEventDestroy(e1);
    if (ms_out) *ms_out = ms;
    return mega_check(h);
}

extern "C" int q3_bench_kernel(q3_handle *h, int kind, int pos, int reps, float *ms_out, int *launches_out,
                               double *bytes_out) {
    if (!h || kind < 0 || kind > 5 || reps < 1) return fail(Q3_EINVAL, "bad bench arguments");
    if (pos < 0 || pos >= h->cfg.seq_len) return fail(Q3_EINVAL, "index out of bounds: pos %d", pos);
    CK(cudaSetDevice(h->device));
    int rc;
    if ((rc = set_tok_pos(h, 0, pos))) return rc;
    const q3_config &c = h->cfg;
    const int gs = c.group_size, dim = c.dim, L = c.n_layers;
    auto one = [&](int l) {
        const LayerDev &W = h->layers[l];
        float *kc_l = h->kc + (size_t)l * c.seq_len * h->KV_l;
        float *vc_l = h->vc + (size_t)l * c.seq_len * h->KV_l;
        GemvArgs g{};
        g.xq = h->xq; g.xs = h->xs; g.pos = h->d_tokpos + 1;
        switch (kind) {
        case 0:
            g.wq = W.qkv.q; g.ws = W.qkv.s; g.K = dim; g.rows = W.qkv.rows; g.q = h->q; g.kc = kc_l; g.vc = vc_l;
            g.AH = h->AH_l; g.KV = h->KV_l;
            launch_gemv<EPI_QKV>(h, g, h->stream);
            break;
        case 1:
            g.wq = W.wo.q; g.ws = W.wo.s; g.K = h->AH_l; g.rows = dim; g.out = h->xb;
            launch_gemv<EPI_STORE>(h, g, h->stream);
            break;
        case 2:
            g.wq = W.w13.q; g.ws = W.w13.s; g.K = dim; g.rows = W.w13.rows; g.out = h->hb;
            launch_gemv<EPI_SWIGLU>(h, g, h->stream);
            break;
        case 3:
            g.wq = W.w2.q; g.ws = W.w2.s; g.xq = h->hq; g.xs = h->hs; g.K = h->H_l; g.rows = dim; g.out = h->xb;
            launch_gemv<EPI_STORE>(h, g, h->stream);
            break;
        case 4:
            g.wq = h->wcls.q; g.ws = h->wcls.s; g.K = dim; g.rows = c.vocab_size; g.out = h->logits;
            launch_gemv<EPI_STORE>(h, g, h->stream);
            break;
        case 5: {
            dim3 ag(h->n_kv_l, ATTN_MAX_SPLITS);
            switch (h->kv_mul) {
            case 1: k_attn_partial<1><<<ag, 128, 0, h->stream>>>(h->q, kc_l, vc_l, h->attn_part, h->d_tokpos + 1, h->KV_l, h->n_heads_l); break;
            case 2: k_attn_partial<2><<<ag, 128, 0, h->stream>>>(h->q, kc_l, vc_l, h->attn_part, h->d_tokpos + 1, h->KV_l, h->n_heads_l); break;
            case 4: k_attn_partial<4><<<ag, 128, 0, h->stream>>>(h->q, kc_l, vc_l, h->attn_part, h->d_tokpos + 1, h->KV_l, h->n_heads_l); break;
            case 8: k_attn_partial<8><<<ag, 128, 0, h->stream>>>(h->q, kc_l, vc_l, h->attn_part, h->d_tokpos + 1, h->KV_l, h->n_heads_l); break;
            }
        } break;
        }
    };
    double bytes = 0;
    const double sc = 1.0 + 4.0 / gs;
    switch (kind) {
    case 0: bytes = (double)h->layers[0].qkv.rows * dim * sc; break;
    case 1: bytes = (double)dim * h->AH_l * sc; break;
    case 2: bytes = (double)h->layers[0].w13.rows * dim * sc; break;
    case 3: bytes = (double)dim * h->H_l * sc; break;
    case 4: bytes = (double)c.vocab_size * dim * sc; break;
    case 5: bytes = 2.0 * (pos + 1) * h->KV_l * 4; break;
    }
    for (int l = 0; l < L; l++) one(l);
    cudaEvent_t e0, e1;
    CK(cudaEventCreate(&e0));
    CK(cudaEventCreate(&e1));
    CK(cudaStreamSynchronize(h->stream));
    CK(cudaEventRecord(e0, h->stream));
    for (int r = 0; r < reps; r++)
        for (int l = 0; l < L; l++) one(l);
    CK(cudaEventRecord(e1, h->stream));
    CK(cudaEventSynchronize(e1));
    CK(cudaGetLastError());
    float ms = 0;
    CK(cudaEventElapsedTime(&ms, e0, e1));
    cudaEventDestroy(e0);
    cudaEventDestroy(e1);
    if (ms_out) *ms_out = ms;
    if (launches_out) *launches_out = reps * L;
    if (bytes_out) *bytes_out = bytes;
    return Q3_OK;
}

extern "C" int q3_prefill(q3_handle *h, const int *tokens, int n, int pos0, float *last_logits_host) {
    if (!h || !tokens || n <= 0) return fail(Q3_EINVAL, "bad prefill arguments");
    if (pos0 < 0 || pos0 + n > h->cfg.seq_len) return fail(Q3_EINVAL, "index out of bounds: pos0 + n = %d > seq_len %d", pos0 + n, h->cfg.seq_len);
    for (int i = 0; i < n; i++)
        if (tokens[i] < 0 || tokens[i] >= h->cfg.vocab_size) return fail(Q3_EINVAL, "index out of bounds: token %d", tokens[i]);
    CK(cudaSetDevice(h->device));
    if (!h->pf_ok || h->exact) {
        for (int i = 0; i < n; i++) {
            int rc = q3_forward(h, tokens[i], pos0 + i, i == n - 1 ? last_logits_host : nullptr);
            if (rc) return rc;
        }
        return Q3_OK;
    }
    int rc;
    if (h->tp_size > 1 && !h->tp_connected) return fail(Q3_ECOMM, "tensor-parallel handle used before q3_tp_connect");
    if ((rc = prefill_chunks(h, tokens, n, pos0))) return rc;
    if ((rc = set_tok_pos(h, tokens[n - 1], pos0 + n - 1))) return rc;
    if (use_mega(h)) {
        if ((rc = launch_mega(h, 0, 0, false, true, false, last_logits_host != nullptr))) return rc;
    } else {
        launch_head(h, h->stream);
    }
    if (last_logits_host) {
        CK(cudaMemcpyAsync(h->h_logits, h->logits, (size_t)h->cfg.vocab_size * 4, cudaMemcpyDeviceToHost, h->stream));
        CK(cudaStreamSynchronize(h->stream));
        if (last_logits_host != h->h_logits) memcpy(last_logits_host, h->h_logits, (size_t)h->cfg.vocab_size * 4);
    } else {
        CK(cudaStreamSynchronize(h->stream));
    }
    CK(cudaGetLastError());
    return mega_check(h);
}

extern "C" int q3_bench_prefill(q3_handle *h, const int *tokens, int n, int pos0, float *ms_out) {
    if (!h || !tokens || n <= 0) return fail(Q3_EINVAL, "bad prefill arguments");
    if (!h->pf_ok) return fail(Q3_EUNSUPPORTED, "batched prefill unavailable: %s", h->pf_why.c_str());
    if (pos0 < 0 || pos0 + n > h->cfg.seq_len) return fail(Q3_EINVAL, "index out of bounds");
    CK(cudaSetDevice(h->device));
    int rc;
    if (h->tp_size > 1 && !h->tp_connected) return fail(Q3_ECOMM, "tensor-parallel handle used before q3_tp_connect");
    if ((rc = prefill_chunks(h, tokens, n, pos0))) return rc;
    cudaEvent_t e0, e1;
    CK(cudaEventCreate(&e0));
    CK(cudaEventCreate(&e1));
    CK(cudaStreamSynchronize(h->stream));
    CK(cudaEventRecord(e0, h->stream));
    if ((rc = prefill_chunks(h, tokens, n, pos0))) return rc;
    CK(cudaEventRecord(e1, h->stream));
    CK(cudaEventSynchronize(e1));
    CK(cudaGetLastError());
    float ms = 0;
    CK(cudaEventElapsedTime(&ms, e0, e1));
    cudaEventDestroy(e0);
    cudaEventDestroy(e1);
    if (ms_out) *ms_out = ms;
    return h->tp_size > 1 ? mega_check(h) : Q3_OK;
}

extern "C" int q3_reset(q3_handle *h) {
    if (!h) return fail(Q3_EINVAL, "null handle");
    CK(cudaSetDevice(h->device));
    size_t kvn = (size_t)h->cfg.n_layers * h->cfg.seq_len * h->KV_l;
    CK(cudaMemsetAsync(h->kc, 0, kvn * 4, h->stream));
    CK(cudaMemsetAsync(h->vc, 0, kvn * 4, h->stream));
    CK(cudaStreamSynchronize(h->stream));
    return Q3_OK;
}

static int kv_rw(q3_handle *h, int layer, int pos0, int n, float *k, float *v, bool write) {
    if (!h) return fail(Q3_EINVAL, "null handle");
    if (layer < 0 || layer >= h->cfg.n_layers || pos0 < 0 || n < 0 || pos0 + n > h->cfg.seq_len)
        return fail(Q3_EINVAL, "kv range out of bounds");
    CK(cudaSetDevice(h->device));
    size_t off = ((size_t)layer * h->cfg.seq_len + pos0) * h->KV_l, bytes = (size_t)n * h->KV_l * 4;
    cudaMemcpyKind kind = write ? cudaMemcpyHostToDevice : cudaMemcpyDeviceToHost;
    CK(cudaStreamSynchronize(h->stream));
    if (k) CK(write ? cudaMemcpy(h->kc + off, k, bytes, kind) : cudaMemcpy(k, h->kc + off, bytes, kind));
    if (v) CK(write ? cudaMemcpy(h->vc + off, v, bytes, kind) : cudaMemcpy(v, h->vc + off, bytes, kind));
    return Q3_OK;
}
extern "C" int q3_kv_read(q3_handle *h, int layer, int pos0, int n, float *k, float *v) {
    return kv_rw(h, layer, pos0, n, k, v, false);
}
extern "C" int q3_kv_write(q3_handle *h, int layer, int pos0, int n, const float *k, const float *v) {
    return kv_rw(h, layer, pos0, n, (float *)k, (float *)v, true);
}

extern "C" int q3_forward_layers(q3_handle *h, int pos, int layer0, int layer1, float *x_host, int run_head,
                                 float *logits_host) {
    if (!h || !x_host) return fail(Q3_EINVAL, "null argument");
    if (pos < 0 || pos >= h->cfg.seq_len) return fail(Q3_EINVAL, "index out of bounds: pos %d", pos);
    if (layer0 < 0 || layer1 > h->cfg.n_layers || layer0 > layer1) return fail(Q3_EINVAL, "bad layer range");
    CK(cudaSetDevice(h->device));
    int rc;
    if ((rc = tp_ready(h))) return rc;
    if ((rc = set_tok_pos(h, 0, pos))) return rc;
    CK(cudaMemcpyAsync(h->x, x_host, (size_t)h->cfg.dim * 4, cudaMemcpyHostToDevice, h->stream));
    if (use_mega(h)) {
        if (layer1 > layer0 && (rc = launch_mega(h, layer0, layer1, false, false, false, false))) return rc;
    } else {
        for (int l = layer0; l < layer1; l++) launch_layer(h, l, false, h->stream);
    }
    CK(cudaMemcpyAsync(x_host, h->x, (size_t)h->cfg.dim * 4, cudaMemcpyDeviceToHost, h->stream));
    if (run_head) {
        if (use_mega(h)) {
            if ((rc = launch_mega(h, 0, 0, false, true, false, true))) return rc;
        } else
        launch_head(h, h->stream);
        if (logits_host)
            CK(cudaMemcpyAsync(logits_host, h->logits, (size_t)h->cfg.vocab_size * 4, cudaMemcpyDeviceToHost, h->stream));
    }
    CK(cudaStreamSynchronize(h->stream));
    CK(cudaGetLastError());
    return mega_check(h);
}

struct DevBuf {
    void *p = nullptr;
    ~DevBuf() {
        if (p) cudaFree(p);
    }
    int alloc(size_t n) { CK(cudaMalloc(&p, n ? n : 16)); return 0; }
    template <class T> T *as() { return (T *)p; }
};
static int op_prologue(int device, int gs) {
    CK(cudaSetDevice(device));
    if (gs != 32 && gs != 64 && gs != 128) return fail(Q3_EUNSUPPORTED, "group_size %d unsupported (32/64/128)", gs);
    return 0;
}

extern "C" int q3_op_quantize(int device, const float *x, int n, int gs, int8_t *q_out, float *s_out) {
    int rc = op_prologue(device, gs);
    if (rc) return rc;
    if (n < 0 || n % gs) return fail(Q3_EINVAL, "n must be a multiple of group_size");
    if (n == 0) return Q3_OK;
    DevBuf dx, dq, ds;
    if ((rc = dx.alloc((size_t)n * 4)) || (rc = dq.alloc(n)) || (rc = ds.alloc((size_t)n / gs * 4))) return rc;
    CK(cudaMemcpy(dx.p, x, (size_t)n * 4, cudaMemcpyHostToDevice));
    int grid = (n / 4 + 255) / 256;
    GS_DISPATCH(gs, (k_quantize<GS><<<grid, 256>>>(dx.as<float>(), n, dq.as<int8_t>(), ds.as<float>())));
    CK(cudaGetLastError());
    CK(cudaMemcpy(q_out, dq.p, n, cudaMemcpyDeviceToHost));
    CK(cudaMemcpy(s_out, ds.p, (size_t)n / gs * 4, cudaMemcpyDeviceToHost));
    return Q3_OK;
}

__global__ void k_expf_ref(const float *x, float *out, int n) {
    int i = blockIdx.x * blockDim.x + threadIdx.x;
    if (i < n) out[i] = expf_ref(x[i]);
}
extern "C" int q3_op_expf(int device, const float *x, int n, float *out) {
    CK(cudaSetDevice(device));
    if (n <= 0) return Q3_OK;
    DevBuf dx, dout;
    int rc;
    if ((rc = dx.alloc((size_t)n * 4)) || (rc = dout.alloc((size_t)n * 4))) return rc;
    CK(cudaMemcpy(dx.p, x, (size_t)n * 4, cudaMemcpyHostToDevice));
    k_expf_ref<<<(n + 255) / 256, 256>>>(dx.as<float>(), dout.as<float>(), n);
    CK(cudaGetLastError());
    CK(cudaMemcpy(out, dout.p, (size_t)n * 4, cudaMemcpyDeviceToHost));
    return Q3_OK;
}

extern "C" int q3_op_matmul(int device, const int8_t *xq, const float *xs, const int8_t *wq, const float *ws, int n,
                            int d, int gs, int exact, float *out, int32_t *group_dots_out) {
    int rc = op_prologue(device, gs);
    if (rc) return rc;
    if (n <= 0 || d < 0 || n % gs || n % 16 || d % 2) return fail(Q3_EINVAL, "need n %% gs == 0, n %% 16 == 0, d even");
    if (d == 0) return Q3_OK;
    const int ng = n / gs;
    DevBuf dxq, dxs, dwq, dws, dout, ddots;
    if ((rc = dxq.alloc(n)) || (rc = dxs.alloc((size_t)ng * 4)) || (rc = dwq.alloc((size_t)d * n)) ||
        (rc = dws.alloc((size_t)d * ng * 4)) || (rc = dout.alloc((size_t)d * 4)))
        return rc;
    if (group_dots_out && (rc = ddots.alloc((size_t)d * ng * 4))) return rc;
    CK(cudaMemcpy(dxq.p, xq, n, cudaMemcpyHostToDevice));
    CK(cudaMemcpy(dxs.p, xs, (size_t)ng * 4, cudaMemcpyHostToDevice));
    CK(cudaMemcpy(dwq.p, wq, (size_t)d * n, cudaMemcpyHostToDevice));
    CK(cudaMemcpy(dws.p, ws, (size_t)d * ng * 4, cudaMemcpyHostToDevice));
    GemvArgs a{};
    a.wq = dwq.as<int8_t>(); a.ws = dws.as<float>(); a.xq = dxq.as<int8_t>(); a.xs = dxs.as<float>();
    a.K = n; a.rows = d; a.out = dout.as<float>(); a.dots = group_dots_out ? ddots.as<int32_t>() : nullptr;
    q3_handle fake;
    cudaDeviceProp prop;
    cudaGetDeviceProperties(&prop, device);
    fake.num_sms = prop.multiProcessorCount;
    fake.cfg.group_size = gs;
    fake.exact = exact ? 31 : 0;
    if ((rc = prepare_exact_kernels())) return rc;
    launch_gemv<EPI_STORE>(&fake, a, 0);
    CK(cudaGetLastError());
    CK(cudaMemcpy(out, dout.p, (size_t)d * 4, cudaMemcpyDeviceToHost));
    if (group_dots_out) CK(cudaMemcpy(group_dots_out, ddots.p, (size_t)d * ng * 4, cudaMemcpyDeviceToHost));
    return Q3_OK;
}

extern "C" int q3_op_gemm_q8(int device, const int8_t *xq, const float *xs, const int8_t *wq, const float *ws, int T, int N,
                             int K, int gs, int exact, float *out) {
    int rc = op_prologue(device, gs);
    if (rc) return rc;
    if (T <= 0 || N % 128 || K % 128 || K % gs || (K / gs) % 2) return fail(Q3_EINVAL, "need N %% 128 == 0, K %% 128 == 0 and an even number of groups per row");
    if (exact != 0 && exact != 1) return fail(Q3_EINVAL, "exact must be 0 (fast drain) or 1 (exact drain), not %d", exact);
    const int Tpad = (T + 127) / 128 * 128, ng = K / gs;
    DevBuf dxq, dxsT, dwq, dws, dwsT, dout;
    if ((rc = dxq.alloc((size_t)Tpad * K)) || (rc = dxsT.alloc((size_t)ng * Tpad * 4)) || (rc = dwq.alloc((size_t)N * K)) ||
        (rc = dws.alloc((size_t)N * ng * 4)) || (rc = dwsT.alloc((size_t)N * ng * 4)) || (rc = dout.alloc((size_t)Tpad * N * 4)))
        return rc;
    CK(cudaMemset(dout.p, 0xFF, (size_t)Tpad * N * 4));
    CK(cudaMemset(dxq.p, 0, (size_t)Tpad * K));
    CK(cudaMemcpy(dxq.p, xq, (size_t)T * K, cudaMemcpyHostToDevice));
    std::vector<float> xsT((size_t)ng * Tpad, 0.0f);
    for (int t = 0; t < T; t++)
        for (int g = 0; g < ng; g++) xsT[(size_t)g * Tpad + t] = xs[(size_t)t * ng + g];
    CK(cudaMemcpy(dxsT.p, xsT.data(), xsT.size() * 4, cudaMemcpyHostToDevice));
    CK(cudaMemcpy(dwq.p, wq, (size_t)N * K, cudaMemcpyHostToDevice));
    CK(cudaMemcpy(dws.p, ws, (size_t)N * ng * 4, cudaMemcpyHostToDevice));
    dim3 tg((ng + 31) / 32, (N + 31) / 32);
    k_transpose_f32<<<tg, dim3(32, 8)>>>(dws.as<float>(), dwsT.as<float>(), N, ng);
    CUtensorMap mx, mw;
    if ((rc = make_map_i8(&mx, dxq.p, Tpad, K)) || (rc = make_map_i8(&mw, dwq.p, N, K))) return rc;
    PrefillGemmArgs a{};
    a.T = T; a.Tpad = Tpad; a.N = N; a.K = K; a.wsT = dwsT.as<float>(); a.xsT = dxsT.as<float>(); a.out = dout.as<float>(); a.ld_out = N;
    if ((rc = launch_gemm_q8<PF_EPI_STORE>(gs, mx, mw, a, 0, exact))) return rc;
    CK(cudaGetLastError());
    CK(cudaDeviceSynchronize());
    CK(cudaMemcpy(out, dout.p, (size_t)T * N * 4, cudaMemcpyDeviceToHost));
    std::vector<uint32_t> pad((size_t)(Tpad - T) * N);
    if (!pad.empty()) {
        CK(cudaMemcpy(pad.data(), dout.as<float>() + (size_t)T * N, pad.size() * 4, cudaMemcpyDeviceToHost));
        for (size_t i = 0; i < pad.size(); i++)
            if (pad[i] != 0xFFFFFFFFu)
                return fail(Q3_ECUDA, "GEMM wrote padding row %d (T %d) at column %d", T + (int)(i / N), T, (int)(i % N));
    }
    return Q3_OK;
}

extern "C" int q3_op_sample(int device, const float *logits, int n, float temperature, float topp, unsigned long long *rng_state,
                            int *token_out) {
    CK(cudaSetDevice(device));
    if (!logits || !rng_state || !token_out || n <= 0) return fail(Q3_EINVAL, "bad argument");
    if (!(temperature > 0.0f)) return fail(Q3_EINVAL, "temperature must be positive (0 = greedy: use the argmax path)");
    DevBuf dl, dp, dk, dr, dt;
    int rc;
    if ((rc = dl.alloc((size_t)n * 4)) || (rc = dp.alloc((size_t)n * 4)) || (rc = dk.alloc(next_pow2((size_t)n) * 8)) || (rc = dr.alloc(8)) ||
        (rc = dt.alloc(4)))
        return rc;
    CK(cudaMemcpy(dl.p, logits, (size_t)n * 4, cudaMemcpyHostToDevice));
    CK(cudaMemcpy(dr.p, rng_state, 8, cudaMemcpyHostToDevice));
    SampleArgs a{};
    a.logits = dl.as<float>(); a.n = n; a.temperature = temperature; a.topp = topp < 0.f ? 0.f : (topp > 1.f ? 1.f : topp);
    a.rng_state = dr.as<unsigned long long>(); a.p = dp.as<float>(); a.keys = dk.as<unsigned long long>(); a.token_out = dt.as<int>();
    k_sample<<<1, SAMPLE_THREADS>>>(a);
    CK(cudaGetLastError());
    CK(cudaMemcpy(rng_state, dr.p, 8, cudaMemcpyDeviceToHost));
    CK(cudaMemcpy(token_out, dt.p, 4, cudaMemcpyDeviceToHost));
    return Q3_OK;
}

extern "C" int q3_op_prefill_attention(int device, const float *q, const float *k, const float *v, int T, int pos0, int n_heads, int n_kv,
                                       float *out) {
    CK(cudaSetDevice(device));
    if (!q || !k || !v || !out || T <= 0 || pos0 < 0 || n_kv <= 0 || n_heads % n_kv) return fail(Q3_EINVAL, "bad attention arguments");
    const int kv_mul = n_heads / n_kv;
    if (kv_mul != 1 && kv_mul != 2 && kv_mul != 4 && kv_mul != 8) return fail(Q3_EUNSUPPORTED, "GQA factor %d unsupported", kv_mul);
    const int AH = n_heads * HEAD_DIM, KV = n_kv * HEAD_DIM, nk = pos0 + T;
    DevBuf dq, dk, dv, dout, dkvh;
    int rc;
    if ((rc = dq.alloc((size_t)T * AH * 4)) || (rc = dk.alloc((size_t)nk * KV * 4)) || (rc = dv.alloc((size_t)nk * KV * 4)) ||
        (rc = dout.alloc((size_t)T * AH * 4)) || (rc = dkvh.alloc((size_t)4 * nk * KV * 2)))
        return rc;
    CK(cudaMemcpy(dq.p, q, (size_t)T * AH * 4, cudaMemcpyHostToDevice));
    CK(cudaMemcpy(dk.p, k, (size_t)nk * KV * 4, cudaMemcpyHostToDevice));
    CK(cudaMemcpy(dv.p, v, (size_t)nk * KV * 4, cudaMemcpyHostToDevice));
    CK(cudaFuncSetAttribute(k_pf_attention_h<1>, cudaFuncAttributeMaxDynamicSharedMemorySize, PFH_SMEM));
    CK(cudaFuncSetAttribute(k_pf_attention_h<2>, cudaFuncAttributeMaxDynamicSharedMemorySize, PFH_SMEM));
    CK(cudaFuncSetAttribute(k_pf_attention_h<4>, cudaFuncAttributeMaxDynamicSharedMemorySize, PFH_SMEM));
    CK(cudaFuncSetAttribute(k_pf_attention_h<8>, cudaFuncAttributeMaxDynamicSharedMemorySize, PFH_SMEM));
    const size_t plane = (size_t)nk * KV;
    k_pf_split_kv<<<296, 256>>>(dk.as<float>(), dv.as<float>(), dkvh.as<__half>(), plane / 4, plane);
    const int bq = PFH_R / kv_mul;
    dim3 ag(n_kv, (T + bq - 1) / bq);
    switch (kv_mul) {
    case 1: k_pf_attention_h<1><<<ag, 128, PFH_SMEM>>>(dq.as<float>(), dkvh.as<__half>(), plane, dout.as<float>(), T, pos0, AH, KV); break;
    case 2: k_pf_attention_h<2><<<ag, 128, PFH_SMEM>>>(dq.as<float>(), dkvh.as<__half>(), plane, dout.as<float>(), T, pos0, AH, KV); break;
    case 4: k_pf_attention_h<4><<<ag, 128, PFH_SMEM>>>(dq.as<float>(), dkvh.as<__half>(), plane, dout.as<float>(), T, pos0, AH, KV); break;
    case 8: k_pf_attention_h<8><<<ag, 128, PFH_SMEM>>>(dq.as<float>(), dkvh.as<__half>(), plane, dout.as<float>(), T, pos0, AH, KV); break;
    }
    CK(cudaGetLastError());
    CK(cudaDeviceSynchronize());
    CK(cudaMemcpy(out, dout.p, (size_t)T * AH * 4, cudaMemcpyDeviceToHost));
    return Q3_OK;
}

__global__ void k_fill_i8(int8_t *p, size_t n, unsigned seed) {
    for (size_t i = (size_t)blockIdx.x * blockDim.x + threadIdx.x; i < n; i += (size_t)gridDim.x * blockDim.x) {
        unsigned h = (unsigned)i * 2654435761u + seed;
        h ^= h >> 15;
        p[i] = (int8_t)((h * 2246822519u >> 24) - 128);
    }
}
__global__ void k_fill_f32(float *p, size_t n, float v) {
    for (size_t i = (size_t)blockIdx.x * blockDim.x + threadIdx.x; i < n; i += (size_t)gridDim.x * blockDim.x) p[i] = v;
}
extern "C" int q3_bench_gemm_q8(int device, int T, int N, int K, int gs, int mode, int reps, float *ms_out) {
    int rc = op_prologue(device, gs);
    if (rc) return rc;
    if (T <= 0 || N % 128 || K % 128 || K % gs || (K / gs) % 2 || reps < 1 || (mode != 0 && mode != 1)) return fail(Q3_EINVAL, "bad gemm bench arguments");
    const int Tpad = (T + 127) / 128 * 128, ng = K / gs;
    DevBuf dxq, dxsT, dwq, dwsT, dout;
    if ((rc = dxq.alloc((size_t)Tpad * K)) || (rc = dxsT.alloc((size_t)ng * Tpad * 4)) || (rc = dwq.alloc((size_t)N * K)) ||
        (rc = dwsT.alloc((size_t)N * ng * 4)) || (rc = dout.alloc((size_t)T * N * 4)))
        return rc;
    k_fill_i8<<<592, 256>>>(dxq.as<int8_t>(), (size_t)Tpad * K, 1);
    k_fill_i8<<<592, 256>>>(dwq.as<int8_t>(), (size_t)N * K, 2);
    k_fill_f32<<<592, 256>>>(dxsT.as<float>(), (size_t)ng * Tpad, 0.01f);
    k_fill_f32<<<592, 256>>>(dwsT.as<float>(), (size_t)N * ng, 0.02f);
    CUtensorMap mx, mw;
    if ((rc = make_map_i8(&mx, dxq.p, Tpad, K)) || (rc = make_map_i8(&mw, dwq.p, N, K))) return rc;
    PrefillGemmArgs a{};
    a.T = T; a.Tpad = Tpad; a.N = N; a.K = K; a.wsT = dwsT.as<float>(); a.xsT = dxsT.as<float>(); a.out = dout.as<float>(); a.ld_out = N;
    if ((rc = launch_gemm_q8<PF_EPI_STORE>(gs, mx, mw, a, 0, mode))) return rc;
    CK(cudaDeviceSynchronize());
    cudaEvent_t e0, e1;
    CK(cudaEventCreate(&e0));
    CK(cudaEventCreate(&e1));
    float best = 1e30f;
    for (int r = 0; r < reps; r++) {
        CK(cudaEventRecord(e0, 0));
        if ((rc = launch_gemm_q8<PF_EPI_STORE>(gs, mx, mw, a, 0, mode))) return rc;
        CK(cudaEventRecord(e1, 0));
        CK(cudaEventSynchronize(e1));
        float ms = 0;
        CK(cudaEventElapsedTime(&ms, e0, e1));
        best = ms < best ? ms : best;
    }
    CK(cudaGetLastError());
    cudaEventDestroy(e0);
    cudaEventDestroy(e1);
    if (ms_out) *ms_out = best;
    return Q3_OK;
}

extern "C" int q3_op_rmsnorm(int device, const float *x, const float *w, int n, float *out) {
    CK(cudaSetDevice(device));
    if (n <= 0) return fail(Q3_EINVAL, "n must be positive");
    DevBuf dx, dw, dout;
    int rc;
    if ((rc = dx.alloc((size_t)n * 4)) || (rc = dw.alloc((size_t)n * 4)) || (rc = dout.alloc((size_t)n * 4))) return rc;
    CK(cudaMemcpy(dx.p, x, (size_t)n * 4, cudaMemcpyHostToDevice));
    CK(cudaMemcpy(dw.p, w, (size_t)n * 4, cudaMemcpyHostToDevice));
    k_rmsnorm<<<1, 1024>>>(dx.as<float>(), dw.as<float>(), dout.as<float>(), n);
    CK(cudaGetLastError());
    CK(cudaMemcpy(out, dout.p, (size_t)n * 4, cudaMemcpyDeviceToHost));
    return Q3_OK;
}

extern "C" int q3_op_quantize_q80_dev(int device, const float *w_dev, size_t n, int gs, int8_t *q_dev, float *s_dev) {
    int rc = op_prologue(device, gs);
    if (rc) return rc;
    if (n % gs) return fail(Q3_EINVAL, "Weight length is not a multiple of group_size");
    if (n == 0) return Q3_OK;
    if (!w_dev || !q_dev || !s_dev) return fail(Q3_EINVAL, "null argument");
    size_t blocks = (n / 4 + 255) / 256;
    int grid = (int)(blocks > 148 * 16 ? 148 * 16 : blocks);
    GS_DISPATCH(gs, (k_quantize_q80<GS><<<grid, 256>>>(w_dev, n, q_dev, s_dev)));
    CK(cudaGetLastError());
    CK(cudaDeviceSynchronize());
    return Q3_OK;
}

extern "C" int q3_op_quantize_q80(int device, const float *w, size_t n, int gs, int8_t *q_out, float *s_out) {
    int rc = op_prologue(device, gs);
    if (rc) return rc;
    if (n % gs) return fail(Q3_EINVAL, "Weight length is not a multiple of group_size");
    if (n == 0) return Q3_OK;
    DevBuf dw, dq, ds;
    if ((rc = dw.alloc(n * 4)) || (rc = dq.alloc(n)) || (rc = ds.alloc(n / gs * 4))) return rc;
    CK(cudaMemcpy(dw.p, w, n * 4, cudaMemcpyHostToDevice));
    size_t blocks = (n / 4 + 255) / 256;
    int grid = (int)(blocks > 148 * 16 ? 148 * 16 : blocks);
    GS_DISPATCH(gs, (k_quantize_q80<GS><<<grid, 256>>>(dw.as<float>(), n, dq.as<int8_t>(), ds.as<float>())));
    CK(cudaGetLastError());
    CK(cudaMemcpy(q_out, dq.p, n, cudaMemcpyDeviceToHost));
    CK(cudaMemcpy(s_out, ds.p, n / gs * 4, cudaMemcpyDeviceToHost));
    return Q3_OK;
}
```

### qwen3_rs_b200/csrc/q3_prefill.cuh

```cuda
#pragma once
#include <cuda.h>
#include <cuda_fp16.h>
#include <cuda_runtime.h>
#include <stdint.h>

#include "q3_mega.cuh"

namespace q3 {

constexpr int PF_BM = 128, PF_BN = 128, PF_BK = 128;
constexpr int PF_STAGES = 4;
constexpr int PF_NACC = 4;
constexpr int PF_EPI_WARPS = 16;
constexpr int PF_THREADS = (3 + PF_EPI_WARPS) * 32;
constexpr int PF_MMA_WARP = PF_EPI_WARPS, PF_TMA_WARP = PF_EPI_WARPS + 1, PF_SCALE_WARP = PF_EPI_WARPS + 2;
constexpr int PF_COLS = PF_BN / (PF_EPI_WARPS / 4);
constexpr int PF_SG = 2;
constexpr int PF_SRING = 8;
constexpr int PF_PATCH_LD = 36;
constexpr int PF_SMEM = PF_STAGES * (PF_BM * PF_BK + PF_BN * PF_BK) + PF_SRING * PF_SG * 1024 + 1024  +
                        PF_EPI_WARPS * 32 * PF_PATCH_LD * 4 + 1024 ;
static_assert(PF_SMEM <= 232448, "shared memory per CTA");

enum { PF_EPI_STORE = 0, PF_EPI_QKV = 1, PF_EPI_RESID = 2, PF_EPI_SWIGLU = 3 };

struct PrefillGemmArgs {
    const float *wsT;
    const float *xsT;
    int T, Tpad, N, K;
    float *out;
    int ld_out;
    float *q;
    float *kc, *vc;
    int AH, KV, pos0;
};

__device__ __forceinline__ uint64_t umma_desc_k_sw128(uint32_t saddr) {
    return (uint64_t)((saddr & 0x3FFFF) >> 4) | (1ULL << 16) | ((uint64_t)(1024 >> 4) << 32) | (1ULL << 46) | (2ULL << 61);
}
__device__ __forceinline__ void umma_i8(uint32_t tmem_d, uint64_t adesc, uint64_t bdesc, uint32_t idesc, uint32_t accumulate) {
    asm volatile(
        "{\n.reg .pred p;\nsetp.ne.b32 p, %4, 0;\ntcgen05.mma.cta_group::1.kind::i8 [%0], %1, %2, %3, p;\n}\n" ::"r"(tmem_d),
        "l"(adesc), "l"(bdesc), "r"(idesc), "r"(accumulate)
        : "memory");
}
__device__ __forceinline__ void umma_commit(uint64_t *bar) {
    asm volatile("tcgen05.commit.cta_group::1.mbarrier::arrive::one.shared::cluster.b64 [%0];" ::"r"(smem_u32(bar)) : "memory");
}
__device__ __forceinline__ void mbar_wait_spin(uint64_t *bar, uint32_t parity) {
    long long t0 = clock64();
    unsigned spins = 0;
    while (!mbar_try_wait(bar, parity)) {
        if ((++spins & 1023u) == 0 && clock64() - t0 > 4000000000LL) __trap();
    }
}
__device__ __forceinline__ void pf_wait(uint32_t bar, uint32_t parity) {
    uint32_t n = 0;
    while (true) {
        uint32_t ok;
        asm volatile("{\n.reg .pred p;\nmbarrier.try_wait.parity.shared::cta.b64 p, [%1], %2;\nselp.u32 %0, 1, 0, p;\n}"
                     : "=r"(ok)
                     : "r"(bar), "r"(parity)
                     : "memory");
        if (ok) break;
        if (++n > (1u << 22)) __trap();
    }
}
__device__ __forceinline__ uint32_t pf_try(uint32_t bar, uint32_t parity) {
    uint32_t ok;
    asm volatile("{\n.reg .pred p;\nmbarrier.try_wait.parity.shared::cta.b64 p, [%1], %2;\nselp.u32 %0, 1, 0, p;\n}"
                 : "=r"(ok)
                 : "r"(bar), "r"(parity)
                 : "memory");
    return ok;
}
__device__ __forceinline__ bool pf_elect() {
    uint32_t pred;
    asm volatile("{\n.reg .pred p;\nelect.sync _|p, 0xffffffff;\nselp.u32 %0, 1, 0, p;\n}" : "=r"(pred));
    return pred != 0;
}
__device__ __forceinline__ void pf_arrive(uint32_t bar) { asm volatile("mbarrier.arrive.shared::cta.b64 _, [%0];" ::"r"(bar) : "memory"); }
__device__ __forceinline__ float4 lds128f(uint32_t saddr) {
    float4 r;
    asm volatile("ld.shared.v4.f32 {%0,%1,%2,%3}, [%4];" : "=f"(r.x), "=f"(r.y), "=f"(r.z), "=f"(r.w) : "r"(saddr));
    return r;
}
#define PF_LD16(d, taddr)                                                                                                            \
    asm volatile("tcgen05.ld.sync.aligned.32x32b.x16.b32 {%0,%1,%2,%3,%4,%5,%6,%7,%8,%9,%10,%11,%12,%13,%14,%15}, [%16];"            \
                 : "=r"(d[0]), "=r"(d[1]), "=r"(d[2]), "=r"(d[3]), "=r"(d[4]), "=r"(d[5]), "=r"(d[6]), "=r"(d[7]), "=r"(d[8]),        \
                   "=r"(d[9]), "=r"(d[10]), "=r"(d[11]), "=r"(d[12]), "=r"(d[13]), "=r"(d[14]), "=r"(d[15])                           \
                 : "r"(taddr)                                                                                                        \
                 : "memory")
__device__ __forceinline__ void pf_wait_ld() { asm volatile("tcgen05.wait::ld.sync.aligned;" ::: "memory"); }

template <bool EXACT>
__device__ __forceinline__ void pf_scale16(float *acc, const uint32_t (&d)[16], uint32_t ws_saddr, float xs) {
    const float2 xs2 = make_float2(xs, xs);
#pragma unroll
    for (int j4 = 0; j4 < 4; j4++) {
        const float4 w = lds128f(ws_saddr + 16 * j4);
        if (EXACT) {
            acc[4 * j4 + 0] = __fadd_rn(acc[4 * j4 + 0], __fmul_rn(__fmul_rn((float)(int)d[4 * j4 + 0], w.x), xs));
            acc[4 * j4 + 1] = __fadd_rn(acc[4 * j4 + 1], __fmul_rn(__fmul_rn((float)(int)d[4 * j4 + 1], w.y), xs));
            acc[4 * j4 + 2] = __fadd_rn(acc[4 * j4 + 2], __fmul_rn(__fmul_rn((float)(int)d[4 * j4 + 2], w.z), xs));
            acc[4 * j4 + 3] = __fadd_rn(acc[4 * j4 + 3], __fmul_rn(__fmul_rn((float)(int)d[4 * j4 + 3], w.w), xs));
        } else {
            float2 *ac = reinterpret_cast<float2 *>(acc + 4 * j4);
            const float2 p01 = __fmul2_rn(make_float2(w.x, w.y), xs2), p23 = __fmul2_rn(make_float2(w.z, w.w), xs2);
            ac[0] = __ffma2_rn(make_float2((float)(int)d[4 * j4 + 0], (float)(int)d[4 * j4 + 1]), p01, ac[0]);
            ac[1] = __ffma2_rn(make_float2((float)(int)d[4 * j4 + 2], (float)(int)d[4 * j4 + 3]), p23, ac[1]);
        }
    }
}

constexpr uint32_t PF_OFF_A = 0;
constexpr uint32_t PF_OFF_B = PF_STAGES * PF_BM * PF_BK;
constexpr uint32_t PF_OFF_SCALE = PF_STAGES * (PF_BM + PF_BN) * PF_BK;
constexpr uint32_t PF_OFF_BAR = PF_OFF_SCALE + PF_SRING * PF_SG * 1024;
constexpr uint32_t PF_BAR_FULL = PF_OFF_BAR, PF_BAR_EMPTY = PF_BAR_FULL + 8 * PF_STAGES, PF_BAR_TFULL = PF_BAR_EMPTY + 8 * PF_STAGES,
                   PF_BAR_TEMPTY = PF_BAR_TFULL + 16 , PF_BAR_SFULL = PF_BAR_TEMPTY + 32,
                   PF_BAR_SEMPTY = PF_BAR_SFULL + 8 * PF_SRING, PF_OFF_TMEM = PF_BAR_SEMPTY + 8 * PF_SRING;
constexpr uint32_t PF_OFF_PATCH = PF_OFF_BAR + 1024;
static_assert(PF_OFF_TMEM + 4 <= PF_OFF_PATCH, "barrier block");
static_assert(PF_OFF_PATCH + PF_EPI_WARPS * 32 * PF_PATCH_LD * 4 + 1024 <= PF_SMEM, "shared memory budget");

__device__ __forceinline__ void sts128f(uint32_t saddr, float4 v) {
    asm volatile("st.shared.v4.f32 [%0], {%1,%2,%3,%4};" ::"r"(saddr), "f"(v.x), "f"(v.y), "f"(v.z), "f"(v.w) : "memory");
}

template <bool EXACT>
__device__ __forceinline__ void pf_drain_pair(float (&acc)[PF_COLS], uint32_t (&d0)[16], uint32_t (&d1)[16], uint32_t taddr, uint32_t ws0, uint32_t xsa,
                                              uint32_t tempty_bar, int lane, uint32_t nxt_taddr, uint32_t nxt_bar, uint32_t nxt_parity) {
    const float xs = lds_f32(xsa);
    pf_wait_ld();
    PF_LD16(d1, taddr + 16);
    pf_scale16<EXACT>(acc, d0, ws0, xs);
    pf_wait_ld();
    asm volatile("tcgen05.fence::before_thread_sync;" ::: "memory");
    __syncwarp();
    if (lane == 0) pf_arrive(tempty_bar);
    PF_LD16(d0, taddr + PF_BN);
    const float xsb = lds_f32(xsa + 512);
    pf_scale16<EXACT>(acc + 16, d1, ws0 + 64, xs);
    pf_wait_ld();
    PF_LD16(d1, taddr + PF_BN + 16);
    const uint32_t nxt_ok = pf_try(nxt_bar, nxt_parity);
    pf_scale16<EXACT>(acc, d0, ws0 + 512, xsb);
    pf_wait_ld();
    asm volatile("tcgen05.fence::before_thread_sync;" ::: "memory");
    __syncwarp();
    if (lane == 0) pf_arrive(tempty_bar + 8);
    if (!nxt_ok) pf_wait(nxt_bar, nxt_parity);
    asm volatile("tcgen05.fence::after_thread_sync;" ::: "memory");
    PF_LD16(d0, nxt_taddr);
    pf_scale16<EXACT>(acc + 16, d1, ws0 + 512 + 64, xsb);
}

template <int GS, int EPI, bool EXACT>
__global__ void __launch_bounds__(PF_THREADS, 1)
    k_gemm_q8(const __grid_constant__ CUtensorMap map_x, const __grid_constant__ CUtensorMap map_w, const __grid_constant__ CUtensorMap map_xs,
              const __grid_constant__ CUtensorMap map_ws, const PrefillGemmArgs a) {
    extern __shared__ __align__(1024) uint8_t pf_smem_raw[];
    uint8_t *smem = reinterpret_cast<uint8_t *>((reinterpret_cast<uintptr_t>(pf_smem_raw) + 1023) & ~(uintptr_t)1023);
    const uint32_t sb = smem_u32(smem);
    const int warp = threadIdx.x >> 5, lane = threadIdx.x & 31;
    const int mt = a.Tpad / PF_BM, ntile = mt * (a.N / PF_BN);
    const int nkb = a.K / PF_BK;
    constexpr int GPS = PF_BK / GS;
    constexpr int KPG = GS / 32;
    const int npair = (a.K / GS) >> 1;
    static_assert(PF_NACC == 4 && PF_SG == 2 && (PF_SRING & (PF_SRING - 1)) == 0, "pairs");

    if (threadIdx.x == 0) {
        for (int s = 0; s < PF_STAGES; s++) {
            mbar_init(reinterpret_cast<uint64_t *>(smem + PF_BAR_FULL) + s, 1);
            mbar_init(reinterpret_cast<uint64_t *>(smem + PF_BAR_EMPTY) + s, 1);
        }
        for (int b = 0; b < 2; b++) mbar_init(reinterpret_cast<uint64_t *>(smem + PF_BAR_TFULL) + b, 1);
        for (int b = 0; b < 4; b++) mbar_init(reinterpret_cast<uint64_t *>(smem + PF_BAR_TEMPTY) + b, PF_EPI_WARPS);
        for (int b = 0; b < PF_SRING; b++) {
            mbar_init(reinterpret_cast<uint64_t *>(smem + PF_BAR_SFULL) + b, 1);
            mbar_init(reinterpret_cast<uint64_t *>(smem + PF_BAR_SEMPTY) + b, PF_EPI_WARPS);
        }
        asm volatile("fence.mbarrier_init.release.cluster;" ::: "memory");
        asm volatile("prefetch.tensormap [%0];" ::"l"(&map_x) : "memory");
        asm volatile("prefetch.tensormap [%0];" ::"l"(&map_w) : "memory");
        asm volatile("prefetch.tensormap [%0];" ::"l"(&map_xs) : "memory");
        asm volatile("prefetch.tensormap [%0];" ::"l"(&map_ws) : "memory");
    }
    if (warp == PF_MMA_WARP) {
        asm volatile("tcgen05.alloc.cta_group::1.sync.aligned.shared::cta.b32 [%0], %1;" ::"r"(sb + PF_OFF_TMEM), "n"(512) : "memory");
        asm volatile("tcgen05.relinquish_alloc_permit.cta_group::1.sync.aligned;" ::: "memory");
    }
    asm volatile("tcgen05.fence::before_thread_sync;" ::: "memory");
    __syncthreads();
    asm volatile("tcgen05.fence::after_thread_sync;" ::: "memory");
    const uint32_t tmem_base = *reinterpret_cast<uint32_t *>(smem + PF_OFF_TMEM);

    if (warp == PF_TMA_WARP) {
        int kbt = 0;
        for (int tile = blockIdx.x; tile < ntile; tile += gridDim.x) {
            const int m0 = (tile % mt) * PF_BM, n0 = (tile / mt) * PF_BN;
            for (int kb = 0; kb < nkb; kb++, kbt++) {
                const int s = kbt % PF_STAGES;
                pf_wait(sb + PF_BAR_EMPTY + 8 * s, ((kbt / PF_STAGES) & 1) ^ 1);
                if (pf_elect()) {
                    uint64_t *bar = reinterpret_cast<uint64_t *>(smem + PF_BAR_FULL) + s;
                    mbar_expect_tx(bar, (PF_BM + PF_BN) * PF_BK);
                    tma_load_2d(smem + PF_OFF_A + (size_t)s * PF_BM * PF_BK, &map_x, kb * PF_BK, m0, bar);
                    tma_load_2d(smem + PF_OFF_B + (size_t)s * PF_BN * PF_BK, &map_w, kb * PF_BK, n0, bar);
                }
                __syncwarp();
            }
        }
    } else if (warp == PF_SCALE_WARP) {
        int sc = 0;
        for (int tile = blockIdx.x; tile < ntile; tile += gridDim.x) {
            const int m0 = (tile % mt) * PF_BM, n0 = (tile / mt) * PF_BN;
            for (int c = 0; c < npair; c++, sc++) {
                const int sl = sc & (PF_SRING - 1);
                pf_wait(sb + PF_BAR_SEMPTY + 8 * sl, ((sc / PF_SRING) & 1) ^ 1);
                if (pf_elect()) {
                    uint64_t *bar = reinterpret_cast<uint64_t *>(smem + PF_BAR_SFULL) + sl;
                    mbar_expect_tx(bar, 2048);
                    tma_load_2d(smem + PF_OFF_SCALE + sl * 2048, &map_ws, n0, 2 * c, bar);
                    tma_load_2d(smem + PF_OFF_SCALE + sl * 2048 + 1024, &map_xs, m0, 2 * c, bar);
                }
                __syncwarp();
            }
        }
    } else if (warp == PF_MMA_WARP) {
        constexpr uint32_t IDESC = (2u << 4) | (1u << 7) | (1u << 10) | ((PF_BN >> 3) << 17) | ((PF_BM >> 4) << 24);
        uint64_t *tfull = reinterpret_cast<uint64_t *>(smem + PF_BAR_TFULL), *empty = reinterpret_cast<uint64_t *>(smem + PF_BAR_EMPTY);
        int kbt = 0, pt = 0;
        const uint64_t desc_a0 = umma_desc_k_sw128(sb + PF_OFF_A), desc_b0 = umma_desc_k_sw128(sb + PF_OFF_B);
        for (int tile = blockIdx.x; tile < ntile; tile += gridDim.x) {
            int gi = 0;
            for (int kb = 0; kb < nkb; kb++, kbt++) {
                const int s = kbt % PF_STAGES;
                pf_wait(sb + PF_BAR_FULL + 8 * s, (kbt / PF_STAGES) & 1);
                asm volatile("tcgen05.fence::after_thread_sync;" ::: "memory");
                const uint64_t da = desc_a0 + (uint64_t)(s * (PF_BM * PF_BK / 16)), db = desc_b0 + (uint64_t)(s * (PF_BN * PF_BK / 16));
#pragma unroll
                for (int gg = 0; gg < GPS; gg++, gi++) {
                    const int ps = pt & 1;
                    const uint32_t col = ps * 2 * PF_BN + (gi & 1) * PF_BN;
                    pf_wait(sb + PF_BAR_TEMPTY + 8 * (2 * ps + (gi & 1)), ((pt >> 1) & 1) ^ 1);
                    asm volatile("tcgen05.fence::after_thread_sync;" ::: "memory");
                    if (pf_elect()) {
#pragma unroll
                        for (int kk = 0; kk < KPG; kk++) {
                            const uint32_t koff = (gg * GS + kk * 32) >> 4;
                            umma_i8(tmem_base + col, da + koff, db + koff, IDESC, kk > 0);
                        }
                        if (gi & 1) umma_commit(&tfull[ps]);
                    }
                    __syncwarp();
                    if (gi & 1) pt++;
                }
                if (pf_elect()) umma_commit(&empty[s]);
                __syncwarp();
            }
        }
        if (pf_elect()) umma_commit(&tfull[pt & 1]);
        __syncwarp();
    } else if (warp < PF_EPI_WARPS) {
        const int quad = warp & 3;
        const int part = warp >> 2;
        const uint32_t tq = tmem_base + ((uint32_t)(quad * 32) << 16) + part * PF_COLS;
        const uint32_t wsx = sb + PF_OFF_SCALE + part * (PF_COLS * 4);
        const uint32_t xsx = sb + PF_OFF_SCALE + 1024 + (quad * 32 + lane) * 4;
        int pt = 0;
        uint32_t d0[16], d1[16];
        uint32_t s_ok = 0;
        pf_wait(sb + PF_BAR_TFULL, 0);
        asm volatile("tcgen05.fence::after_thread_sync;" ::: "memory");
        PF_LD16(d0, tq);
        for (int tile = blockIdx.x; tile < ntile; tile += gridDim.x) {
            float acc[PF_COLS];
#pragma unroll
            for (int j = 0; j < PF_COLS; j++) acc[j] = 0.0f;
#pragma unroll 1
            for (int c = 0; c < npair; c++, pt++) {
                const uint32_t ps = pt & 1, sl = pt & (PF_SRING - 1);
                if (!s_ok) pf_wait(sb + PF_BAR_SFULL + 8 * sl, (pt / PF_SRING) & 1);
                s_ok = pf_try(sb + PF_BAR_SFULL + 8 * ((pt + 1) & (PF_SRING - 1)), ((pt + 1) / PF_SRING) & 1);
                pf_drain_pair<EXACT>(acc, d0, d1, tq + ps * (2 * PF_BN), wsx + sl * 2048, xsx + sl * 2048, sb + PF_BAR_TEMPTY + 16 * ps, lane,
                                     tq + (ps ^ 1) * (2 * PF_BN), sb + PF_BAR_TFULL + 8 * (ps ^ 1), ((pt + 1) >> 1) & 1);
                __syncwarp();
                if (lane == 0) pf_arrive(sb + PF_BAR_SEMPTY + 8 * sl);
            }
            {
                const int m0 = (tile % mt) * PF_BM, n0 = (tile / mt) * PF_BN;
                const uint32_t patch = sb + PF_OFF_PATCH + warp * (32 * PF_PATCH_LD * 4);
#pragma unroll
                for (int j4 = 0; j4 < PF_COLS / 4; j4++)
                    sts128f(patch + (lane * PF_PATCH_LD + 4 * j4) * 4, make_float4(acc[4 * j4], acc[4 * j4 + 1], acc[4 * j4 + 2], acc[4 * j4 + 3]));
                __syncwarp();
                const int r4 = lane >> 3, c4 = lane & 7;
                const int c0 = n0 + part * PF_COLS;
                float *base;
                int ld;
                if (EPI == PF_EPI_STORE || EPI == PF_EPI_RESID) { base = a.out + c0; ld = a.ld_out; }
                else if (EPI == PF_EPI_SWIGLU) { base = a.out + c0 / 2; ld = a.ld_out; }
                else if (c0 < a.AH) { base = a.q + c0; ld = a.AH; }
                else if (c0 < a.AH + a.KV) { base = a.kc + (size_t)a.pos0 * a.KV + (c0 - a.AH); ld = a.KV; }
                else { base = a.vc + (size_t)a.pos0 * a.KV + (c0 - a.AH - a.KV); ld = a.KV; }
#pragma unroll
                for (int k = 0; k < 8; k++) {
                    const int row = 4 * k + r4, tr = m0 + quad * 32 + row;
                    const float4 v = lds128f(patch + (row * PF_PATCH_LD + 4 * c4) * 4);
                    if (tr < a.T) {
                        if (EPI == PF_EPI_SWIGLU) {
                            const float s0 = __fmul_rn(v.x, __fdiv_rn(1.0f, __fadd_rn(1.0f, expf(-v.x))));
                            const float s1 = __fmul_rn(v.z, __fdiv_rn(1.0f, __fadd_rn(1.0f, expf(-v.z))));
                            *reinterpret_cast<float2 *>(base + (size_t)tr * ld + 2 * c4) = make_float2(__fmul_rn(s0, v.y), __fmul_rn(s1, v.w));
                        } else {
                            float4 *dst = reinterpret_cast<float4 *>(base + (size_t)tr * ld + 4 * c4);
                            if (EPI == PF_EPI_RESID) {
                                const float4 o = *dst;
                                *dst = make_float4(__fadd_rn(o.x, v.x), __fadd_rn(o.y, v.y), __fadd_rn(o.z, v.z), __fadd_rn(o.w, v.w));
                            } else {
                                *dst = v;
                            }
                        }
                    }
                }
                __syncwarp();
            }
        }
        pf_wait_ld();
    }
    asm volatile("tcgen05.fence::before_thread_sync;" ::: "memory");
    __syncthreads();
    if (warp == PF_MMA_WARP) {
        asm volatile("tcgen05.fence::after_thread_sync;" ::: "memory");
        asm volatile("tcgen05.dealloc.cta_group::1.sync.aligned.b32 %0, %1;" ::"r"(tmem_base), "n"(512) : "memory");
    }
}
#undef PF_LD16

template <int GS, int MAXV = 16>
__global__ void __launch_bounds__(256) k_pf_norm_quant(float *x, const float *w, int8_t *q, float *sT, int n, int Tpad,
                                                       const int8_t *embed_q, const float *embed_s, const int *tokens, int write_normed) {
    __shared__ float red[8];
    __shared__ float s_f;
    const int t = blockIdx.x, tid = threadIdx.x, lane = tid & 31, warp = tid >> 5;
    float *xr = x + (size_t)t * n;
    const int n4 = n >> 2;
    float4 v[MAXV];
    float ss = 0.0f;
#pragma unroll
    for (int k = 0; k < MAXV; k++) {
        int i4 = tid + k * 256;
        v[k] = make_float4(0.f, 0.f, 0.f, 0.f);
        if (i4 < n4) {
            if (embed_q) {
                size_t base = (size_t)tokens[t] * n + (size_t)i4 * 4;
                char4 e = *reinterpret_cast<const char4 *>(embed_q + base);
                float sc = embed_s[base / GS];
                v[k] = make_float4((float)e.x * sc, (float)e.y * sc, (float)e.z * sc, (float)e.w * sc);
                reinterpret_cast<float4 *>(xr)[i4] = v[k];
            } else {
                v[k] = reinterpret_cast<const float4 *>(xr)[i4];
            }
            ss += __fmul_rn(v[k].x, v[k].x);
            ss += __fmul_rn(v[k].y, v[k].y);
            ss += __fmul_rn(v[k].z, v[k].z);
            ss += __fmul_rn(v[k].w, v[k].w);
        }
    }
    ss = warp_sum(ss);
    if (lane == 0) red[warp] = ss;
    __syncthreads();
    if (tid == 0) {
        float tsum = 0.0f;
        for (int i = 0; i < 8; i++) tsum += red[i];
        s_f = __fdiv_rn(1.0f, sqrtf(__fadd_rn(__fdiv_rn(tsum, (float)n), NORM_EPS)));
    }
    __syncthreads();
    const float f = s_f;
#pragma unroll
    for (int k = 0; k < MAXV; k++) {
        int i4 = tid + k * 256;
        if (i4 - lane < n4) {
            float4 y = make_float4(0.f, 0.f, 0.f, 0.f);
            if (i4 < n4) {
                float4 wv = __ldg(reinterpret_cast<const float4 *>(w) + i4);
                y.x = __fmul_rn(wv.x, __fmul_rn(f, v[k].x));
                y.y = __fmul_rn(wv.y, __fmul_rn(f, v[k].y));
                y.z = __fmul_rn(wv.z, __fmul_rn(f, v[k].z));
                y.w = __fmul_rn(wv.w, __fmul_rn(f, v[k].w));
            }
            uint32_t packed;
            float scale;
            quantize_group4<GS>(y, packed, scale);
            if (i4 < n4) {
                reinterpret_cast<uint32_t *>(q + (size_t)t * n)[i4] = packed;
                if ((i4 % (GS / 4)) == 0) sT[(size_t)(i4 / (GS / 4)) * Tpad + t] = scale;
                if (write_normed) reinterpret_cast<float4 *>(xr)[i4] = y;
            }
        }
    }
}

template <int GS>
__global__ void __launch_bounds__(256) k_pf_quantize(const float *__restrict__ x, int8_t *q, float *sT, int n, int Tpad) {
    const int t = blockIdx.x, lane = threadIdx.x & 31;
    const int n4 = n >> 2;
    const float *xr = x + (size_t)t * n;
    for (int base = threadIdx.x - lane; base < n4; base += 256) {
        int i4 = base + lane;
        float4 y = (i4 < n4) ? reinterpret_cast<const float4 *>(xr)[i4] : make_float4(0.f, 0.f, 0.f, 0.f);
        uint32_t packed;
        float scale;
        quantize_group4<GS>(y, packed, scale);
        if (i4 < n4) {
            reinterpret_cast<uint32_t *>(q + (size_t)t * n)[i4] = packed;
            if ((i4 % (GS / 4)) == 0) sT[(size_t)(i4 / (GS / 4)) * Tpad + t] = scale;
        }
    }
}

__global__ void __launch_bounds__(128) k_pf_qknorm_rope(float *q, float *kc_layer, const float *q_ln, const float *k_ln,
                                                        const float *rope, int pos0, int n_heads, int n_kv, int AH, int KV) {
    const int lane = threadIdx.x & 31;
    const int head = blockIdx.x * 4 + (threadIdx.x >> 5);
    const int t = blockIdx.y;
    if (head >= n_heads + n_kv) return;
    const int pos = pos0 + t;
    float *p = head < n_heads ? q + (size_t)t * AH + (size_t)head * HEAD_DIM
                              : kc_layer + (size_t)pos * KV + (size_t)(head - n_heads) * HEAD_DIM;
    float4 v = reinterpret_cast<float4 *>(p)[lane];
    float4 r = qk_norm_rope(v, head < n_heads ? q_ln : k_ln, rope + (size_t)pos * HEAD_DIM, lane);
    reinterpret_cast<float4 *>(p)[lane] = r;
}

constexpr int PFH_R = 64, PFH_BK = 32;
constexpr int PFH_SMEM = 2 * PFH_R * HEAD_DIM * 2 + 2 * 4 * PFH_BK * HEAD_DIM * 2;

__global__ void __launch_bounds__(256) k_pf_split_kv(const float *__restrict__ kc, const float *__restrict__ vc, __half *out, size_t n4, size_t plane) {
    for (size_t i = (size_t)blockIdx.x * blockDim.x + threadIdx.x; i < 2 * n4; i += (size_t)gridDim.x * blockDim.x) {
        const bool isv = i >= n4;
        const size_t j = isv ? i - n4 : i;
        const float4 x = reinterpret_cast<const float4 *>(isv ? vc : kc)[j];
        const __half2 h0 = __floats2half2_rn(x.x, x.y), h1 = __floats2half2_rn(x.z, x.w);
        const float2 f0 = __half22float2(h0), f1 = __half22float2(h1);
        const __half2 l0 = __floats2half2_rn(__fsub_rn(x.x, f0.x), __fsub_rn(x.y, f0.y)), l1 = __floats2half2_rn(__fsub_rn(x.z, f1.x), __fsub_rn(x.w, f1.y));
        __half *dst = out + (isv ? 2 * plane : 0) + 4 * j;
        *reinterpret_cast<uint2 *>(dst) = make_uint2(*reinterpret_cast<const uint32_t *>(&h0), *reinterpret_cast<const uint32_t *>(&h1));
        *reinterpret_cast<uint2 *>(dst + plane) = make_uint2(*reinterpret_cast<const uint32_t *>(&l0), *reinterpret_cast<const uint32_t *>(&l1));
    }
}

__device__ __forceinline__ void mma_f16(float (&c)[4], uint32_t a0, uint32_t a1, uint32_t a2, uint32_t a3, uint32_t b0, uint32_t b1) {
    asm("mma.sync.aligned.m16n8k16.row.col.f32.f16.f16.f32 {%0,%1,%2,%3}, {%4,%5,%6,%7}, {%8,%9}, {%0,%1,%2,%3};"
                 : "+f"(c[0]), "+f"(c[1]), "+f"(c[2]), "+f"(c[3])
                 : "r"(a0), "r"(a1), "r"(a2), "r"(a3), "r"(b0), "r"(b1));
}
__device__ __forceinline__ void ldsm4(uint32_t (&r)[4], uint32_t saddr) {
    asm volatile("ldmatrix.sync.aligned.m8n8.x4.shared.b16 {%0,%1,%2,%3}, [%4];" : "=r"(r[0]), "=r"(r[1]), "=r"(r[2]), "=r"(r[3]) : "r"(saddr));
}
__device__ __forceinline__ void ldsm4t(uint32_t (&r)[4], uint32_t saddr) {
    asm volatile("ldmatrix.sync.aligned.m8n8.x4.trans.shared.b16 {%0,%1,%2,%3}, [%4];" : "=r"(r[0]), "=r"(r[1]), "=r"(r[2]), "=r"(r[3]) : "r"(saddr));
}
__device__ __forceinline__ void pfh_split2(float x, float y, uint32_t &hi, uint32_t &lo) {
    const __half2 h = __floats2half2_rn(x, y);
    const float2 f = __half22float2(h);
    const __half2 l = __floats2half2_rn(__fsub_rn(x, f.x), __fsub_rn(y, f.y));
    hi = *reinterpret_cast<const uint32_t *>(&h);
    lo = *reinterpret_cast<const uint32_t *>(&l);
}

template <int KVMUL>
__global__ void __launch_bounds__(128, 2) k_pf_attention_h(const float *__restrict__ q, const __half *__restrict__ kvh, size_t plane, float *out, int T,
                                                           int pos0, int AH, int KV) {
    extern __shared__ __align__(1024) uint8_t pfh_smem[];
    const uint32_t sQ = smem_u32(pfh_smem);
    const uint32_t sKV = sQ + 2 * PFH_R * HEAD_DIM * 2;
    constexpr uint32_t QL = PFH_R * HEAD_DIM * 2, ARR = PFH_BK * HEAD_DIM * 2, STAGE = 4 * ARR;
    constexpr int BQ = PFH_R / KVMUL;
    const int kvhd = blockIdx.x, q0 = ((int)gridDim.y - 1 - (int)blockIdx.y) * BQ;
    const int tid = threadIdx.x, lane = tid & 31, warp = tid >> 5, g = lane >> 2, t = lane & 3;
    const float scale = __fdiv_rn(1.0f, sqrtf((float)HEAD_DIM));
    int last_q = q0 + BQ - 1;
    if (last_q > T - 1) last_q = T - 1;
    const int nkeys = pos0 + last_q + 1;
    const int ntiles = (nkeys + PFH_BK - 1) / PFH_BK;

    auto load_stage = [&](int tile, int st) {
        const int k0 = tile * PFH_BK;
#pragma unroll
        for (int i = 0; i < 16; i++) {
            const int idx = tid + i * 128, arr = idx >> 9, p = (idx >> 4) & 31, c = idx & 15;
            const int key = k0 + p;
            const bool ok = key < nkeys;
            const __half *src = kvh + (size_t)arr * plane + (size_t)(ok ? key : 0) * KV + (size_t)kvhd * HEAD_DIM + c * 8;
            const uint32_t dst = sKV + st * STAGE + arr * ARR + p * 256 + ((c ^ (p & 7)) << 4);
            asm volatile("cp.async.cg.shared.global [%0], [%1], 16, %2;" ::"r"(dst), "l"(src), "r"(ok ? 16 : 0) : "memory");
        }
        asm volatile("cp.async.commit_group;" ::: "memory");
    };
    load_stage(0, 0);
    for (int i = tid; i < PFH_R * 16; i += 128) {
        const int r = i >> 4, c = i & 15;
        const int tq = q0 + r / KVMUL;
        float4 v0 = make_float4(0.f, 0.f, 0.f, 0.f), v1 = v0;
        if (tq < T) {
            const float4 *src = reinterpret_cast<const float4 *>(q + (size_t)tq * AH + (size_t)(kvhd * KVMUL + r % KVMUL) * HEAD_DIM + c * 8);
            v0 = src[0];
            v1 = src[1];
        }
        uint32_t h[4], l[4];
        pfh_split2(v0.x, v0.y, h[0], l[0]);
        pfh_split2(v0.z, v0.w, h[1], l[1]);
        pfh_split2(v1.x, v1.y, h[2], l[2]);
        pfh_split2(v1.z, v1.w, h[3], l[3]);
        const uint32_t off = r * 256 + ((c ^ (r & 7)) << 4);
        asm volatile("st.shared.v4.b32 [%0], {%1,%2,%3,%4};" ::"r"(sQ + off), "r"(h[0]), "r"(h[1]), "r"(h[2]), "r"(h[3]) : "memory");
        asm volatile("st.shared.v4.b32 [%0], {%1,%2,%3,%4};" ::"r"(sQ + QL + off), "r"(l[0]), "r"(l[1]), "r"(l[2]), "r"(l[3]) : "memory");
    }
    const int r0 = warp * 16 + g, r1 = r0 + 8;
    const int qp0 = pos0 + q0 + r0 / KVMUL, qp1 = pos0 + q0 + r1 / KVMUL;
    float m0 = -INFINITY, m1 = -INFINITY, l0 = 0.0f, l1 = 0.0f;
    float o[16][4];
#pragma unroll
    for (int j = 0; j < 16; j++) o[j][0] = o[j][1] = o[j][2] = o[j][3] = 0.0f;
    const int a_row = warp * 16 + (lane & 7) + ((lane >> 3) & 1) * 8, a_cg = (lane >> 4) & 1;
    const int b_key = (lane & 7) + ((lane >> 4) & 1) * 8, b_cg = (lane >> 3) & 1;
    const int v_key = (lane & 7) + ((lane >> 3) & 1) * 8, v_cg = (lane >> 4) & 1;

    for (int tile = 0; tile < ntiles; tile++) {
        const int st = tile & 1, k0 = tile * PFH_BK;
        if (tile + 1 < ntiles) {
            load_stage(tile + 1, st ^ 1);
            asm volatile("cp.async.wait_group 1;" ::: "memory");
        } else {
            asm volatile("cp.async.wait_group 0;" ::: "memory");
        }
        __syncthreads();
        const uint32_t sKh = sKV + st * STAGE, sKl = sKh + ARR, sVh = sKh + 2 * ARR, sVl = sKh + 3 * ARR;
        float s[4][4];
#pragma unroll
        for (int j = 0; j < 4; j++) s[j][0] = s[j][1] = s[j][2] = s[j][3] = 0.0f;
#pragma unroll
        for (int ks = 0; ks < 8; ks++) {
            uint32_t ah[4], al[4];
            const uint32_t aoff = a_row * 256 + (((2 * ks + a_cg) ^ (a_row & 7)) << 4);
            ldsm4(ah, sQ + aoff);
            ldsm4(al, sQ + QL + aoff);
            uint32_t bh[2][4], bl[2][4];
#pragma unroll
            for (int jj = 0; jj < 2; jj++) {
                const int key = 16 * jj + b_key;
                const uint32_t boff = key * 256 + (((2 * ks + b_cg) ^ (key & 7)) << 4);
                ldsm4(bh[jj], sKh + boff);
                ldsm4(bl[jj], sKl + boff);
            }
#pragma unroll
            for (int j = 0; j < 4; j++) mma_f16(s[j], al[0], al[1], al[2], al[3], bh[j >> 1][2 * (j & 1)], bh[j >> 1][2 * (j & 1) + 1]);
#pragma unroll
            for (int j = 0; j < 4; j++) mma_f16(s[j], ah[0], ah[1], ah[2], ah[3], bl[j >> 1][2 * (j & 1)], bl[j >> 1][2 * (j & 1) + 1]);
#pragma unroll
            for (int j = 0; j < 4; j++) mma_f16(s[j], ah[0], ah[1], ah[2], ah[3], bh[j >> 1][2 * (j & 1)], bh[j >> 1][2 * (j & 1) + 1]);
        }
        float mx0 = -INFINITY, mx1 = -INFINITY;
#pragma unroll
        for (int j = 0; j < 4; j++) {
            const int key = k0 + 8 * j + 2 * t;
            s[j][0] = (key <= qp0) ? __fmul_rn(s[j][0], scale) : -INFINITY;
            s[j][1] = (key + 1 <= qp0) ? __fmul_rn(s[j][1], scale) : -INFINITY;
            s[j][2] = (key <= qp1) ? __fmul_rn(s[j][2], scale) : -INFINITY;
            s[j][3] = (key + 1 <= qp1) ? __fmul_rn(s[j][3], scale) : -INFINITY;
            mx0 = fmaxf(mx0, fmaxf(s[j][0], s[j][1]));
            mx1 = fmaxf(mx1, fmaxf(s[j][2], s[j][3]));
        }
        mx0 = fmaxf(mx0, __shfl_xor_sync(0xffffffffu, mx0, 1));
        mx0 = fmaxf(mx0, __shfl_xor_sync(0xffffffffu, mx0, 2));
        mx1 = fmaxf(mx1, __shfl_xor_sync(0xffffffffu, mx1, 1));
        mx1 = fmaxf(mx1, __shfl_xor_sync(0xffffffffu, mx1, 2));
        const float mn0 = fmaxf(m0, mx0), mn1 = fmaxf(m1, mx1);
        const float c0 = (mn0 == -INFINITY) ? 1.0f : expf(m0 - mn0), c1 = (mn1 == -INFINITY) ? 1.0f : expf(m1 - mn1);
        m0 = mn0;
        m1 = mn1;
        l0 *= c0;
        l1 *= c1;
#pragma unroll
        for (int j = 0; j < 16; j++) {
            o[j][0] *= c0;
            o[j][1] *= c0;
            o[j][2] *= c1;
            o[j][3] *= c1;
        }
#pragma unroll
        for (int kk = 0; kk < 2; kk++) {
            uint32_t ph[4], pl[4];
#pragma unroll
            for (int h2 = 0; h2 < 2; h2++) {
                const float *sj = s[2 * kk + h2];
                const float p00 = (sj[0] == -INFINITY) ? 0.0f : expf(sj[0] - mn0), p01 = (sj[1] == -INFINITY) ? 0.0f : expf(sj[1] - mn0);
                const float p10 = (sj[2] == -INFINITY) ? 0.0f : expf(sj[2] - mn1), p11 = (sj[3] == -INFINITY) ? 0.0f : expf(sj[3] - mn1);
                l0 += p00 + p01;
                l1 += p10 + p11;
                pfh_split2(p00, p01, ph[2 * h2], pl[2 * h2]);
                pfh_split2(p10, p11, ph[2 * h2 + 1], pl[2 * h2 + 1]);
            }
            const int key = 16 * kk + v_key;
#pragma unroll
            for (int n4 = 0; n4 < 4; n4++) {
                uint32_t vh[2][4], vl[2][4];
#pragma unroll
                for (int h2 = 0; h2 < 2; h2++) {
                    const int nn = 2 * n4 + h2;
                    const uint32_t voff = key * 256 + (((2 * nn + v_cg) ^ (key & 7)) << 4);
                    ldsm4t(vh[h2], sVh + voff);
                    ldsm4t(vl[h2], sVl + voff);
                }
#pragma unroll
                for (int j = 0; j < 4; j++) mma_f16(o[4 * n4 + j], pl[0], pl[1], pl[2], pl[3], vh[j >> 1][2 * (j & 1)], vh[j >> 1][2 * (j & 1) + 1]);
#pragma unroll
                for (int j = 0; j < 4; j++) mma_f16(o[4 * n4 + j], ph[0], ph[1], ph[2], ph[3], vl[j >> 1][2 * (j & 1)], vl[j >> 1][2 * (j & 1) + 1]);
#pragma unroll
                for (int j = 0; j < 4; j++) mma_f16(o[4 * n4 + j], ph[0], ph[1], ph[2], ph[3], vh[j >> 1][2 * (j & 1)], vh[j >> 1][2 * (j & 1) + 1]);
            }
        }
        __syncthreads();
    }
    l0 += __shfl_xor_sync(0xffffffffu, l0, 1);
    l0 += __shfl_xor_sync(0xffffffffu, l0, 2);
    l1 += __shfl_xor_sync(0xffffffffu, l1, 1);
    l1 += __shfl_xor_sync(0xffffffffu, l1, 2);
    const float i0 = __fdiv_rn(1.0f, l0), i1 = __fdiv_rn(1.0f, l1);
    const int tq0 = q0 + r0 / KVMUL, tq1 = q0 + r1 / KVMUL;
    float *d0 = out + (size_t)tq0 * AH + (size_t)(kvhd * KVMUL + r0 % KVMUL) * HEAD_DIM + 2 * t;
    float *d1 = out + (size_t)tq1 * AH + (size_t)(kvhd * KVMUL + r1 % KVMUL) * HEAD_DIM + 2 * t;
#pragma unroll
    for (int n = 0; n < 16; n++) {
        if (tq0 < T) *reinterpret_cast<float2 *>(d0 + 8 * n) = make_float2(__fmul_rn(o[n][0], i0), __fmul_rn(o[n][1], i0));
        if (tq1 < T) *reinterpret_cast<float2 *>(d1 + 8 * n) = make_float2(__fmul_rn(o[n][2], i1), __fmul_rn(o[n][3], i1));
    }
}

struct PfPeers {
    const float *part[MEGA_MAX_TP];
    unsigned long long *ctr[MEGA_MAX_TP];
};
__global__ void k_pf_xbarrier(PfPeers p, int tp, int rank, unsigned long long target, int *status) {
    if (threadIdx.x != 0 || blockIdx.x != 0) return;
    __threadfence_system();
    for (int r = 0; r < tp; r++) asm volatile("red.release.sys.global.add.u64 [%0], %1;" ::"l"(p.ctr[r]), "l"(1ULL) : "memory");
    const long long t0 = clock64();
    unsigned long long v;
    do {
        asm volatile("ld.acquire.sys.global.u64 %0, [%1];" : "=l"(v) : "l"(p.ctr[rank]) : "memory");
        if (v < target && clock64() - t0 > 6000000000LL) {
            atomicExch(status, 11);
            return;
        }
    } while (v < target);
}
__global__ void __launch_bounds__(256) k_pf_reduce_scatter(PfPeers p, float *own, int tp, int rank, size_t n4) {
    const size_t lo = n4 * rank / tp, hi = n4 * (rank + 1) / tp;
    for (size_t i = lo + (size_t)blockIdx.x * blockDim.x + threadIdx.x; i < hi; i += (size_t)gridDim.x * blockDim.x) {
        float4 s = __ldcg(reinterpret_cast<const float4 *>(p.part[0]) + i);
        for (int r = 1; r < tp; r++) {
            const float4 v = __ldcg(reinterpret_cast<const float4 *>(p.part[r]) + i);
            s.x = __fadd_rn(s.x, v.x);
            s.y = __fadd_rn(s.y, v.y);
            s.z = __fadd_rn(s.z, v.z);
            s.w = __fadd_rn(s.w, v.w);
        }
        reinterpret_cast<float4 *>(own)[i] = s;
    }
}
__global__ void __launch_bounds__(256) k_pf_allgather_resid(float *x, PfPeers p, int tp, size_t n4) {
    const int r = blockIdx.y;
    const size_t lo = n4 * r / tp, hi = n4 * (r + 1) / tp;
    for (size_t i = lo + (size_t)blockIdx.x * blockDim.x + threadIdx.x; i < hi; i += (size_t)gridDim.x * blockDim.x) {
        const float4 s = __ldcg(reinterpret_cast<const float4 *>(p.part[r]) + i);
        float4 o = reinterpret_cast<float4 *>(x)[i];
        o.x = __fadd_rn(o.x, s.x);
        o.y = __fadd_rn(o.y, s.y);
        o.z = __fadd_rn(o.z, s.z);
        o.w = __fadd_rn(o.w, s.w);
        reinterpret_cast<float4 *>(x)[i] = o;
    }
}
__global__ void __launch_bounds__(256) k_pf_allreduce_resid(float *x, PfPeers p, int tp, size_t n4) {
    for (size_t i = (size_t)blockIdx.x * blockDim.x + threadIdx.x; i < n4; i += (size_t)gridDim.x * blockDim.x) {
        float4 s = __ldcg(reinterpret_cast<const float4 *>(p.part[0]) + i);
        for (int r = 1; r < tp; r++) {
            const float4 v = __ldcg(reinterpret_cast<const float4 *>(p.part[r]) + i);
            s.x = __fadd_rn(s.x, v.x);
            s.y = __fadd_rn(s.y, v.y);
            s.z = __fadd_rn(s.z, v.z);
            s.w = __fadd_rn(s.w, v.w);
        }
        float4 o = reinterpret_cast<float4 *>(x)[i];
        o.x = __fadd_rn(o.x, s.x);
        o.y = __fadd_rn(o.y, s.y);
        o.z = __fadd_rn(o.z, s.z);
        o.w = __fadd_rn(o.w, s.w);
        reinterpret_cast<float4 *>(x)[i] = o;
    }
}

__global__ void k_transpose_f32(const float *__restrict__ in, float *out, int rows, int cols) {
    __shared__ float tile[32][33];
    int c = blockIdx.x * 32 + threadIdx.x, r = blockIdx.y * 32 + threadIdx.y;
    for (int j = 0; j < 32; j += 8)
        if (r + j < rows && c < cols) tile[threadIdx.y + j][threadIdx.x] = in[(size_t)(r + j) * cols + c];
    __syncthreads();
    int oc = blockIdx.y * 32 + threadIdx.x, orow = blockIdx.x * 32 + threadIdx.y;
    for (int j = 0; j < 32; j += 8)
        if (orow + j < cols && oc < rows) out[(size_t)(orow + j) * rows + oc] = tile[threadIdx.x][threadIdx.y + j];
}

}
```

Before: 454.9.

## Rewrite prefill attention with tcgen05 UMMA, TMEM accumulators and TMA pipeline

Replaces the mma.sync flash-attention prefill kernel with a warp-specialized kernel. In the new kernel a TMA warp streams split-half K/V tiles through a 4-slot mbarrier ring, an MMA warp issues tcgen05 UMMA into tensor memory, and four softmax warps rescale the accumulators in TMEM. The change aims to raise tensor-core throughput and overlap loads with compute in prefill attention. It adds considerable complexity in descriptors, barriers and TMEM allocation, and it runs one CTA per SM with larger tiles.

```diff
diff --git a/qwen3_rs_b200/csrc/q3_engine.cu b/qwen3_rs_b200/csrc/q3_engine.cu
--- a/qwen3_rs_b200/csrc/q3_engine.cu
+++ b/qwen3_rs_b200/csrc/q3_engine.cu
@@ -712,6 +712,33 @@
     return 0;
 }
 
+static int make_map_kvh(CUtensorMap *map, const __half *base, size_t rows, int KV, size_t plane) {
+    auto enc = get_encode_fn();
+    if (!enc) return fail(Q3_ECUDA, "cuTensorMapEncodeTiled unavailable");
+    cuuint64_t dims[3] = {(cuuint64_t)KV, (cuuint64_t)rows, 4};
+    cuuint64_t strides[2] = {(cuuint64_t)KV * 2, (cuuint64_t)plane * 2};
+    cuuint32_t box[3] = {64, (cuuint32_t)PFA_BK, 1};
+    cuuint32_t estr[3] = {1, 1, 1};
+    CUresult r = enc(map, CU_TENSOR_MAP_DATA_TYPE_FLOAT16, 3, const_cast<__half *>(base), dims, strides, box, estr, CU_TENSOR_MAP_INTERLEAVE_NONE,
+                     CU_TENSOR_MAP_SWIZZLE_128B, CU_TENSOR_MAP_L2_PROMOTION_L2_256B, CU_TENSOR_MAP_FLOAT_OOB_FILL_NONE);
+    if (r != CUDA_SUCCESS) return fail(Q3_ECUDA, "cuTensorMapEncodeTiled (K/V split) failed (%d) rows %zu KV %d", (int)r, rows, KV);
+    return 0;
+}
+
+static int launch_pf_attention(const CUtensorMap &map_kv, const float *q, float *out, int T, int pos0, int n_kv, int kv_mul, int AH, cudaStream_t s) {
+    const int bq = PFA_M / kv_mul;
+    dim3 grid(n_kv, (T + bq - 1) / bq);
+    switch (kv_mul) {
+    case 1: k_pf_attention_tc<1><<<grid, PFA_THREADS, PFA_SMEM, s>>>(map_kv, q, out, T, pos0, AH); break;
+    case 2: k_pf_attention_tc<2><<<grid, PFA_THREADS, PFA_SMEM, s>>>(map_kv, q, out, T, pos0, AH); break;
+    case 4: k_pf_attention_tc<4><<<grid, PFA_THREADS, PFA_SMEM, s>>>(map_kv, q, out, T, pos0, AH); break;
+    case 8: k_pf_attention_tc<8><<<grid, PFA_THREADS, PFA_SMEM, s>>>(map_kv, q, out, T, pos0, AH); break;
+    default: return fail(Q3_EUNSUPPORTED, "GQA factor %d unsupported", kv_mul);
+    }
+    CK(cudaGetLastError());
+    return 0;
+}
+
 static int make_map_scales(CUtensorMap *map, const float *base, int groups, int cols) {
     auto enc = get_encode_fn();
     if (!enc) return fail(Q3_ECUDA, "cuTensorMapEncodeTiled unavailable");
@@ -783,10 +810,10 @@
         return 0;
     }
     if (!get_encode_fn()) { h->pf_why = "cuTensorMapEncodeTiled unavailable"; return 0; }
-    CK(cudaFuncSetAttribute(k_pf_attention_h<1>, cudaFuncAttributeMaxDynamicSharedMemorySize, PFH_SMEM));
-    CK(cudaFuncSetAttribute(k_pf_attention_h<2>, cudaFuncAttributeMaxDynamicSharedMemorySize, PFH_SMEM));
-    CK(cudaFuncSetAttribute(k_pf_attention_h<4>, cudaFuncAttributeMaxDynamicSharedMemorySize, PFH_SMEM));
-    CK(cudaFuncSetAttribute(k_pf_attention_h<8>, cudaFuncAttributeMaxDynamicSharedMemorySize, PFH_SMEM));
+    CK(cudaFuncSetAttribute(k_pf_attention_tc<1>, cudaFuncAttributeMaxDynamicSharedMemorySize, PFA_SMEM));
+    CK(cudaFuncSetAttribute(k_pf_attention_tc<2>, cudaFuncAttributeMaxDynamicSharedMemorySize, PFA_SMEM));
+    CK(cudaFuncSetAttribute(k_pf_attention_tc<4>, cudaFuncAttributeMaxDynamicSharedMemorySize, PFA_SMEM));
+    CK(cudaFuncSetAttribute(k_pf_attention_tc<8>, cudaFuncAttributeMaxDynamicSharedMemorySize, PFA_SMEM));
     int rc;
     for (auto &W : h->layers) {
         if ((rc = prefill_prepare_tensor(h, W.qkv))) return rc;
@@ -895,6 +922,9 @@
     if ((rc = make_map_i8(&mx_dim, h->pf_xq, Tpad, dim))) return rc;
     if ((rc = make_map_i8(&mx_ah, h->pf_xq, Tpad, AH))) return rc;
     if ((rc = make_map_i8(&mx_h, h->pf_hq, Tpad, H))) return rc;
+    CUtensorMap map_kv;
+    const size_t rows = (size_t)pos0 + T, plane = h->pf_kvh_rows * KV;
+    if ((rc = make_map_kvh(&map_kv, h->pf_kvh, rows, KV, plane))) return rc;
     for (int l = 0; l < c.n_layers; l++) {
         LayerDev &W = h->layers[l];
         float *kc_l = h->kc + (size_t)l * c.seq_len * KV;
@@ -912,16 +942,8 @@
         if ((rc = launch_gemm_q8<PF_EPI_QKV>(gs, mx_dim, W.qkv.map, g, s))) return rc;
         dim3 rg((h->n_heads_l + h->n_kv_l + 3) / 4, T);
         k_pf_qknorm_rope<<<rg, 128, 0, s>>>(h->pf_q, kc_l, W.q_ln, W.k_ln, h->rope, pos0, h->n_heads_l, h->n_kv_l, AH, KV);
-        const size_t rows = (size_t)pos0 + T, plane = h->pf_kvh_rows * KV;
         k_pf_split_kv<<<h->num_sms * 4, 256, 0, s>>>(kc_l, vc_l, h->pf_kvh, rows * KV / 4, plane);
-        const int bq = PFH_R / h->kv_mul;
-        dim3 ag(h->n_kv_l, (T + bq - 1) / bq);
-        switch (h->kv_mul) {
-        case 1: k_pf_attention_h<1><<<ag, 128, PFH_SMEM, s>>>(h->pf_q, h->pf_kvh, plane, h->pf_att, T, pos0, AH, KV); break;
-        case 2: k_pf_attention_h<2><<<ag, 128, PFH_SMEM, s>>>(h->pf_q, h->pf_kvh, plane, h->pf_att, T, pos0, AH, KV); break;
-        case 4: k_pf_attention_h<4><<<ag, 128, PFH_SMEM, s>>>(h->pf_q, h->pf_kvh, plane, h->pf_att, T, pos0, AH, KV); break;
-        case 8: k_pf_attention_h<8><<<ag, 128, PFH_SMEM, s>>>(h->pf_q, h->pf_kvh, plane, h->pf_att, T, pos0, AH, KV); break;
-        }
+        if ((rc = launch_pf_attention(map_kv, h->pf_q, h->pf_att, T, pos0, h->n_kv_l, h->kv_mul, AH, s))) return rc;
         GS_DISPATCH(gs, (k_pf_quantize<GS><<<T, 256, 0, s>>>(h->pf_att, h->pf_xq, h->pf_xsT, AH, Tpad)));
         PrefillGemmArgs o{};
         o.T = T; o.Tpad = Tpad; o.K = AH; o.N = dim; o.wsT = W.wo.sT; o.xsT = h->pf_xsT; o.out = h->pf_x; o.ld_out = dim;
@@ -1786,21 +1808,15 @@
     CK(cudaMemcpy(dq.p, q, (size_t)T * AH * 4, cudaMemcpyHostToDevice));
     CK(cudaMemcpy(dk.p, k, (size_t)nk * KV * 4, cudaMemcpyHostToDevice));
     CK(cudaMemcpy(dv.p, v, (size_t)nk * KV * 4, cudaMemcpyHostToDevice));
-    CK(cudaFuncSetAttribute(k_pf_attention_h<1>, cudaFuncAttributeMaxDynamicSharedMemorySize, PFH_SMEM));
-    CK(cudaFuncSetAttribute(k_pf_attention_h<2>, cudaFuncAttributeMaxDynamicSharedMemorySize, PFH_SMEM));
-    CK(cudaFuncSetAttribute(k_pf_attention_h<4>, cudaFuncAttributeMaxDynamicSharedMemorySize, PFH_SMEM));
-    CK(cudaFuncSetAttribute(k_pf_attention_h<8>, cudaFuncAttributeMaxDynamicSharedMemorySize, PFH_SMEM));
+    CK(cudaFuncSetAttribute(k_pf_attention_tc<1>, cudaFuncAttributeMaxDynamicSharedMemorySize, PFA_SMEM));
+    CK(cudaFuncSetAttribute(k_pf_attention_tc<2>, cudaFuncAttributeMaxDynamicSharedMemorySize, PFA_SMEM));
+    CK(cudaFuncSetAttribute(k_pf_attention_tc<4>, cudaFuncAttributeMaxDynamicSharedMemorySize, PFA_SMEM));
+    CK(cudaFuncSetAttribute(k_pf_attention_tc<8>, cudaFuncAttributeMaxDynamicSharedMemorySize, PFA_SMEM));
     const size_t plane = (size_t)nk * KV;
     k_pf_split_kv<<<296, 256>>>(dk.as<float>(), dv.as<float>(), dkvh.as<__half>(), plane / 4, plane);
-    const int bq = PFH_R / kv_mul;
-    dim3 ag(n_kv, (T + bq - 1) / bq);
-    switch (kv_mul) {
-    case 1: k_pf_attention_h<1><<<ag, 128, PFH_SMEM>>>(dq.as<float>(), dkvh.as<__half>(), plane, dout.as<float>(), T, pos0, AH, KV); break;
-    case 2: k_pf_attention_h<2><<<ag, 128, PFH_SMEM>>>(dq.as<float>(), dkvh.as<__half>(), plane, dout.as<float>(), T, pos0, AH, KV); break;
-    case 4: k_pf_attention_h<4><<<ag, 128, PFH_SMEM>>>(dq.as<float>(), dkvh.as<__half>(), plane, dout.as<float>(), T, pos0, AH, KV); break;
-    case 8: k_pf_attention_h<8><<<ag, 128, PFH_SMEM>>>(dq.as<float>(), dkvh.as<__half>(), plane, dout.as<float>(), T, pos0, AH, KV); break;
-    }
-    CK(cudaGetLastError());
+    CUtensorMap map_kv;
+    if ((rc = make_map_kvh(&map_kv, dkvh.as<__half>(), nk, KV, plane))) return rc;
+    if ((rc = launch_pf_attention(map_kv, dq.as<float>(), dout.as<float>(), T, pos0, n_kv, kv_mul, AH, 0))) return rc;
     CK(cudaDeviceSynchronize());
     CK(cudaMemcpy(out, dout.p, (size_t)T * AH * 4, cudaMemcpyDeviceToHost));
     return Q3_OK;
diff --git a/qwen3_rs_b200/csrc/q3_prefill.cuh b/qwen3_rs_b200/csrc/q3_prefill.cuh
--- a/qwen3_rs_b200/csrc/q3_prefill.cuh
+++ b/qwen3_rs_b200/csrc/q3_prefill.cuh
@@ -436,8 +436,18 @@
     reinterpret_cast<float4 *>(p)[lane] = r;
 }
 
-constexpr int PFH_R = 64, PFH_BK = 32;
-constexpr int PFH_SMEM = 2 * PFH_R * HEAD_DIM * 2 + 2 * 4 * PFH_BK * HEAD_DIM * 2;
+constexpr int PFA_M = 128, PFA_BK = 64, PFA_SLOTS = 4;
+constexpr int PFA_THREADS = 192, PFA_MMA_WARP = 4, PFA_TMA_WARP = 5;
+constexpr uint32_t PFA_OFF_Q = 0;
+constexpr uint32_t PFA_OFF_P = PFA_OFF_Q + 2 * PFA_M * HEAD_DIM * 2;
+constexpr uint32_t PFA_OFF_KV = PFA_OFF_P + 2 * PFA_M * PFA_BK * 2;
+constexpr uint32_t PFA_SLOT = 2 * PFA_BK * HEAD_DIM * 2;
+constexpr uint32_t PFA_OFF_BAR = PFA_OFF_KV + PFA_SLOTS * PFA_SLOT;
+constexpr uint32_t PFA_BAR_FULL = PFA_OFF_BAR, PFA_BAR_EMPTY = PFA_BAR_FULL + 8 * PFA_SLOTS, PFA_BAR_Q = PFA_BAR_EMPTY + 8 * PFA_SLOTS,
+                   PFA_BAR_SFULL = PFA_BAR_Q + 8, PFA_BAR_SEMPTY = PFA_BAR_SFULL + 16, PFA_BAR_PFULL = PFA_BAR_SEMPTY + 16,
+                   PFA_BAR_PVDONE = PFA_BAR_PFULL + 8, PFA_OFF_TMEM = PFA_BAR_PVDONE + 8;
+constexpr int PFA_SMEM = PFA_OFF_TMEM + 8 + 1024 ;
+static_assert(PFA_SMEM <= 232448, "shared memory per CTA");
 
 __global__ void __launch_bounds__(256) k_pf_split_kv(const float *__restrict__ kc, const float *__restrict__ vc, __half *out, size_t n4, size_t plane) {
     for (size_t i = (size_t)blockIdx.x * blockDim.x + threadIdx.x; i < 2 * n4; i += (size_t)gridDim.x * blockDim.x) {
@@ -453,193 +463,273 @@
     }
 }
 
-__device__ __forceinline__ void mma_f16(float (&c)[4], uint32_t a0, uint32_t a1, uint32_t a2, uint32_t a3, uint32_t b0, uint32_t b1) {
-    asm("mma.sync.aligned.m16n8k16.row.col.f32.f16.f16.f32 {%0,%1,%2,%3}, {%4,%5,%6,%7}, {%8,%9}, {%0,%1,%2,%3};"
-                 : "+f"(c[0]), "+f"(c[1]), "+f"(c[2]), "+f"(c[3])
-                 : "r"(a0), "r"(a1), "r"(a2), "r"(a3), "r"(b0), "r"(b1));
-}
-__device__ __forceinline__ void ldsm4(uint32_t (&r)[4], uint32_t saddr) {
-    asm volatile("ldmatrix.sync.aligned.m8n8.x4.shared.b16 {%0,%1,%2,%3}, [%4];" : "=r"(r[0]), "=r"(r[1]), "=r"(r[2]), "=r"(r[3]) : "r"(saddr));
-}
-__device__ __forceinline__ void ldsm4t(uint32_t (&r)[4], uint32_t saddr) {
-    asm volatile("ldmatrix.sync.aligned.m8n8.x4.trans.shared.b16 {%0,%1,%2,%3}, [%4];" : "=r"(r[0]), "=r"(r[1]), "=r"(r[2]), "=r"(r[3]) : "r"(saddr));
-}
-__device__ __forceinline__ void pfh_split2(float x, float y, uint32_t &hi, uint32_t &lo) {
+__device__ __forceinline__ void pfa_split2(float x, float y, uint32_t &hi, uint32_t &lo) {
     const __half2 h = __floats2half2_rn(x, y);
     const float2 f = __half22float2(h);
     const __half2 l = __floats2half2_rn(__fsub_rn(x, f.x), __fsub_rn(y, f.y));
     hi = *reinterpret_cast<const uint32_t *>(&h);
     lo = *reinterpret_cast<const uint32_t *>(&l);
 }
+__device__ __forceinline__ void umma_f16(uint32_t tmem_d, uint64_t adesc, uint64_t bdesc, uint32_t idesc, uint32_t accumulate) {
+    asm volatile(
+        "{\n.reg .pred p;\nsetp.ne.b32 p, %4, 0;\ntcgen05.mma.cta_group::1.kind::f16 [%0], %1, %2, %3, p;\n}\n" ::"r"(tmem_d),
+        "l"(adesc), "l"(bdesc), "r"(idesc), "r"(accumulate)
+        : "memory");
+}
+__device__ __forceinline__ uint64_t umma_desc_mn_sw128(uint32_t saddr, uint32_t lbo) {
+    return (uint64_t)((saddr & 0x3FFFF) >> 4) | ((uint64_t)(lbo >> 4) << 16) | ((uint64_t)(1024 >> 4) << 32) | (1ULL << 46) | (2ULL << 61);
+}
+__device__ __forceinline__ void tma_load_3d(uint32_t dst, const CUtensorMap *map, int c0, int c1, int c2, uint32_t bar) {
+    asm volatile("cp.async.bulk.tensor.3d.shared::cluster.global.mbarrier::complete_tx::bytes [%0], [%1, {%2, %3, %4}], [%5];" ::"r"(dst),
+                 "l"(map), "r"(c0), "r"(c1), "r"(c2), "r"(bar)
+                 : "memory");
+}
+#define PFA_LD32(d, taddr)                                                                                                           \
+    asm volatile("tcgen05.ld.sync.aligned.32x32b.x32.b32 {%0,%1,%2,%3,%4,%5,%6,%7,%8,%9,%10,%11,%12,%13,%14,%15,%16,%17,%18,%19,%20,"  \
+                 "%21,%22,%23,%24,%25,%26,%27,%28,%29,%30,%31}, [%32];"                                                              \
+                 : "=r"(d[0]), "=r"(d[1]), "=r"(d[2]), "=r"(d[3]), "=r"(d[4]), "=r"(d[5]), "=r"(d[6]), "=r"(d[7]), "=r"(d[8]),        \
+                   "=r"(d[9]), "=r"(d[10]), "=r"(d[11]), "=r"(d[12]), "=r"(d[13]), "=r"(d[14]), "=r"(d[15]), "=r"(d[16]),            \
+                   "=r"(d[17]), "=r"(d[18]), "=r"(d[19]), "=r"(d[20]), "=r"(d[21]), "=r"(d[22]), "=r"(d[23]), "=r"(d[24]),           \
+                   "=r"(d[25]), "=r"(d[26]), "=r"(d[27]), "=r"(d[28]), "=r"(d[29]), "=r"(d[30]), "=r"(d[31])                         \
+                 : "r"(taddr)                                                                                                        \
+                 : "memory")
+#define PFA_ST32(taddr, d)                                                                                                           \
+    asm volatile("tcgen05.st.sync.aligned.32x32b.x32.b32 [%0], {%1,%2,%3,%4,%5,%6,%7,%8,%9,%10,%11,%12,%13,%14,%15,%16,%17,%18,%19,"  \
+                 "%20,%21,%22,%23,%24,%25,%26,%27,%28,%29,%30,%31,%32};" ::"r"(taddr),                                              \
+                 "r"(d[0]), "r"(d[1]), "r"(d[2]), "r"(d[3]), "r"(d[4]), "r"(d[5]), "r"(d[6]), "r"(d[7]), "r"(d[8]), "r"(d[9]),       \
+                 "r"(d[10]), "r"(d[11]), "r"(d[12]), "r"(d[13]), "r"(d[14]), "r"(d[15]), "r"(d[16]), "r"(d[17]), "r"(d[18]),         \
+                 "r"(d[19]), "r"(d[20]), "r"(d[21]), "r"(d[22]), "r"(d[23]), "r"(d[24]), "r"(d[25]), "r"(d[26]), "r"(d[27]),         \
+                 "r"(d[28]), "r"(d[29]), "r"(d[30]), "r"(d[31])                                                                      \
+                 : "memory")
 
 template <int KVMUL>
-__global__ void __launch_bounds__(128, 2) k_pf_attention_h(const float *__restrict__ q, const __half *__restrict__ kvh, size_t plane, float *out, int T,
-                                                           int pos0, int AH, int KV) {
-    extern __shared__ __align__(1024) uint8_t pfh_smem[];
-    const uint32_t sQ = smem_u32(pfh_smem);
-    const uint32_t sKV = sQ + 2 * PFH_R * HEAD_DIM * 2;
-    constexpr uint32_t QL = PFH_R * HEAD_DIM * 2, ARR = PFH_BK * HEAD_DIM * 2, STAGE = 4 * ARR;
-    constexpr int BQ = PFH_R / KVMUL;
+__global__ void __launch_bounds__(PFA_THREADS, 1)
+    k_pf_attention_tc(const __grid_constant__ CUtensorMap map_kv, const float *__restrict__ q, float *out, int T, int pos0, int AH) {
+    extern __shared__ __align__(1024) uint8_t pfa_smem_raw[];
+    uint8_t *smem = reinterpret_cast<uint8_t *>((reinterpret_cast<uintptr_t>(pfa_smem_raw) + 1023) & ~(uintptr_t)1023);
+    const uint32_t sb = smem_u32(smem);
+    const int warp = threadIdx.x >> 5, lane = threadIdx.x & 31;
+    constexpr int BQ = PFA_M / KVMUL;
     const int kvhd = blockIdx.x, q0 = ((int)gridDim.y - 1 - (int)blockIdx.y) * BQ;
-    const int tid = threadIdx.x, lane = tid & 31, warp = tid >> 5, g = lane >> 2, t = lane & 3;
-    const float scale = __fdiv_rn(1.0f, sqrtf((float)HEAD_DIM));
-    int last_q = q0 + BQ - 1;
-    if (last_q > T - 1) last_q = T - 1;
-    const int nkeys = pos0 + last_q + 1;
-    const int ntiles = (nkeys + PFH_BK - 1) / PFH_BK;
-
-    auto load_stage = [&](int tile, int st) {
-        const int k0 = tile * PFH_BK;
-#pragma unroll
-        for (int i = 0; i < 16; i++) {
-            const int idx = tid + i * 128, arr = idx >> 9, p = (idx >> 4) & 31, c = idx & 15;
-            const int key = k0 + p;
-            const bool ok = key < nkeys;
-            const __half *src = kvh + (size_t)arr * plane + (size_t)(ok ? key : 0) * KV + (size_t)kvhd * HEAD_DIM + c * 8;
-            const uint32_t dst = sKV + st * STAGE + arr * ARR + p * 256 + ((c ^ (p & 7)) << 4);
-            asm volatile("cp.async.cg.shared.global [%0], [%1], 16, %2;" ::"r"(dst), "l"(src), "r"(ok ? 16 : 0) : "memory");
-        }
-        asm volatile("cp.async.commit_group;" ::: "memory");
-    };
-    load_stage(0, 0);
-    for (int i = tid; i < PFH_R * 16; i += 128) {
-        const int r = i >> 4, c = i & 15;
+    const int last_q = min(q0 + BQ - 1, T - 1);
+    const int ntiles = (pos0 + last_q + 1 + PFA_BK - 1) / PFA_BK;
+
+    if (threadIdx.x == 0) {
+        for (int s = 0; s < PFA_SLOTS; s++) {
+            mbar_init(reinterpret_cast<uint64_t *>(smem + PFA_BAR_FULL) + s, 1);
+            mbar_init(reinterpret_cast<uint64_t *>(smem + PFA_BAR_EMPTY) + s, 1);
+        }
+        mbar_init(reinterpret_cast<uint64_t *>(smem + PFA_BAR_Q), 128);
+        for (int b = 0; b < 2; b++) {
+            mbar_init(reinterpret_cast<uint64_t *>(smem + PFA_BAR_SFULL) + b, 1);
+            mbar_init(reinterpret_cast<uint64_t *>(smem + PFA_BAR_SEMPTY) + b, 128);
+        }
+        mbar_init(reinterpret_cast<uint64_t *>(smem + PFA_BAR_PFULL), 128);
+        mbar_init(reinterpret_cast<uint64_t *>(smem + PFA_BAR_PVDONE), 1);
+        asm volatile("fence.mbarrier_init.release.cluster;" ::: "memory");
+        asm volatile("prefetch.tensormap [%0];" ::"l"(&map_kv) : "memory");
+    }
+    if (warp == PFA_MMA_WARP) {
+        asm volatile("tcgen05.alloc.cta_group::1.sync.aligned.shared::cta.b32 [%0], %1;" ::"r"(sb + PFA_OFF_TMEM), "n"(256) : "memory");
+        asm volatile("tcgen05.relinquish_alloc_permit.cta_group::1.sync.aligned;" ::: "memory");
+    }
+    asm volatile("tcgen05.fence::before_thread_sync;" ::: "memory");
+    __syncthreads();
+    asm volatile("tcgen05.fence::after_thread_sync;" ::: "memory");
+    const uint32_t tmem_base = *reinterpret_cast<uint32_t *>(smem + PFA_OFF_TMEM);
+
+    if (warp == PFA_TMA_WARP) {
+        int u = 0;
+        auto load = [&](int tile, int plane0) {
+            const int s = u % PFA_SLOTS;
+            pf_wait(sb + PFA_BAR_EMPTY + 8 * s, ((u / PFA_SLOTS) & 1) ^ 1);
+            if (pf_elect()) {
+                const uint32_t bar = sb + PFA_BAR_FULL + 8 * s, dst = sb + PFA_OFF_KV + s * PFA_SLOT;
+                asm volatile("mbarrier.arrive.expect_tx.shared::cta.b64 _, [%0], %1;" ::"r"(bar), "r"(PFA_SLOT) : "memory");
+#pragma unroll
+                for (int i = 0; i < 4; i++)
+                    tma_load_3d(dst + i * (PFA_SLOT / 4), &map_kv, kvhd * HEAD_DIM + (i & 1) * 64, tile * PFA_BK, plane0 + (i >> 1), bar);
+            }
+            __syncwarp();
+            u++;
+        };
+        load(0, 0);
+        for (int j = 0; j < ntiles; j++) {
+            if (j + 1 < ntiles) load(j + 1, 0);
+            load(j, 2);
+        }
+    } else if (warp == PFA_MMA_WARP) {
+        constexpr uint32_t IDESC_S = (1u << 4) | ((PFA_BK >> 3) << 17) | ((PFA_M >> 4) << 24);
+        constexpr uint32_t IDESC_PV = (1u << 4) | (1u << 16) | ((HEAD_DIM >> 3) << 17) | ((PFA_M >> 4) << 24);
+        constexpr uint32_t QL = PFA_M * HEAD_DIM * 2, PL = PFA_M * PFA_BK * 2, KVL = PFA_SLOT / 2;
+        int u = 0;
+        pf_wait(sb + PFA_BAR_Q, 0);
+        asm volatile("tcgen05.fence::after_thread_sync;" ::: "memory");
+        auto issue_s = [&](int j) {
+            const int s = u % PFA_SLOTS, b = j & 1;
+            pf_wait(sb + PFA_BAR_FULL + 8 * s, (u / PFA_SLOTS) & 1);
+            pf_wait(sb + PFA_BAR_SEMPTY + 8 * b, ((j >> 1) & 1) ^ 1);
+            asm volatile("tcgen05.fence::after_thread_sync;" ::: "memory");
+            if (pf_elect()) {
+                const uint32_t kb = sb + PFA_OFF_KV + s * PFA_SLOT;
+#pragma unroll
+                for (int term = 0; term < 3; term++) {
+                    const uint32_t qa = sb + PFA_OFF_Q + (term == 0 ? QL : 0), ka = kb + (term == 1 ? KVL : 0);
+#pragma unroll
+                    for (int kk = 0; kk < HEAD_DIM / 16; kk++)
+                        umma_f16(tmem_base + PFA_M + PFA_BK * b, umma_desc_k_sw128(qa + (kk >> 2) * (PFA_M * 128) + (kk & 3) * 32),
+                                 umma_desc_k_sw128(ka + (kk >> 2) * (PFA_BK * 128) + (kk & 3) * 32), IDESC_S, (term | kk) != 0);
+                }
+                umma_commit(reinterpret_cast<uint64_t *>(smem + PFA_BAR_SFULL) + b);
+                umma_commit(reinterpret_cast<uint64_t *>(smem + PFA_BAR_EMPTY) + s);
+            }
+            __syncwarp();
+            u++;
+        };
+        auto issue_pv = [&](int j) {
+            const int s = u % PFA_SLOTS;
+            pf_wait(sb + PFA_BAR_FULL + 8 * s, (u / PFA_SLOTS) & 1);
+            pf_wait(sb + PFA_BAR_PFULL, j & 1);
+            asm volatile("tcgen05.fence::after_thread_sync;" ::: "memory");
+            if (pf_elect()) {
+                const uint32_t vb = sb + PFA_OFF_KV + s * PFA_SLOT;
+#pragma unroll
+                for (int term = 0; term < 3; term++) {
+                    const uint32_t pa = sb + PFA_OFF_P + (term == 0 ? PL : 0), va = vb + (term == 1 ? KVL : 0);
+#pragma unroll
+                    for (int kk = 0; kk < PFA_BK / 16; kk++)
+                        umma_f16(tmem_base, umma_desc_k_sw128(pa + kk * 32), umma_desc_mn_sw128(va + kk * 2048, PFA_BK * 128), IDESC_PV,
+                                 (j | term | kk) != 0);
+                }
+                umma_commit(reinterpret_cast<uint64_t *>(smem + PFA_BAR_PVDONE));
+                umma_commit(reinterpret_cast<uint64_t *>(smem + PFA_BAR_EMPTY) + s);
+            }
+            __syncwarp();
+            u++;
+        };
+        issue_s(0);
+        for (int j = 0; j < ntiles; j++) {
+            if (j + 1 < ntiles) issue_s(j + 1);
+            issue_pv(j);
+        }
+    } else {
+        const int r = threadIdx.x;
+#pragma unroll 4
+        for (int i = r; i < PFA_M * 16; i += 128) {
+            const int rr = i >> 4, c = i & 15;
+            const int tq = q0 + rr / KVMUL;
+            float4 v0 = make_float4(0.f, 0.f, 0.f, 0.f), v1 = v0;
+            if (tq < T) {
+                const float4 *src = reinterpret_cast<const float4 *>(q + (size_t)tq * AH + (size_t)(kvhd * KVMUL + rr % KVMUL) * HEAD_DIM + c * 8);
+                v0 = src[0];
+                v1 = src[1];
+            }
+            uint32_t h[4], l[4];
+            pfa_split2(v0.x, v0.y, h[0], l[0]);
+            pfa_split2(v0.z, v0.w, h[1], l[1]);
+            pfa_split2(v1.x, v1.y, h[2], l[2]);
+            pfa_split2(v1.z, v1.w, h[3], l[3]);
+            const uint32_t off = PFA_OFF_Q + (c >> 3) * (PFA_M * 128) + rr * 128 + (((c & 7) ^ (rr & 7)) << 4);
+            asm volatile("st.shared.v4.b32 [%0], {%1,%2,%3,%4};" ::"r"(sb + off), "r"(h[0]), "r"(h[1]), "r"(h[2]), "r"(h[3]) : "memory");
+            asm volatile("st.shared.v4.b32 [%0], {%1,%2,%3,%4};" ::"r"(sb + off + PFA_M * HEAD_DIM * 2), "r"(l[0]), "r"(l[1]), "r"(l[2]), "r"(l[3]) : "memory");
+        }
+        asm volatile("fence.proxy.async.shared::cta;" ::: "memory");
+        pf_arrive(sb + PFA_BAR_Q);
+
+        const float scale = __fdiv_rn(1.0f, sqrtf((float)HEAD_DIM));
+        const int qp = pos0 + q0 + r / KVMUL;
+        const uint32_t trow = tmem_base + ((uint32_t)(warp * 32) << 16);
+        const uint32_t prow = sb + PFA_OFF_P + r * 128, psw = r & 7;
+        float m = -INFINITY, l = 0.0f;
+        for (int j = 0; j < ntiles; j++) {
+            const int b = j & 1, k0 = j * PFA_BK;
+            pf_wait(sb + PFA_BAR_SFULL + 8 * b, (j >> 1) & 1);
+            asm volatile("tcgen05.fence::after_thread_sync;" ::: "memory");
+            float s[PFA_BK];
+            {
+                uint32_t d[32];
+                PFA_LD32(d, trow + PFA_M + PFA_BK * b);
+                pf_wait_ld();
+#pragma unroll
+                for (int i = 0; i < 32; i++) s[i] = __uint_as_float(d[i]);
+                PFA_LD32(d, trow + PFA_M + PFA_BK * b + 32);
+                pf_wait_ld();
+#pragma unroll
+                for (int i = 0; i < 32; i++) s[32 + i] = __uint_as_float(d[i]);
+            }
+            asm volatile("tcgen05.fence::before_thread_sync;" ::: "memory");
+            pf_arrive(sb + PFA_BAR_SEMPTY + 8 * b);
+            const int lim = qp - k0;
+            float mx = -INFINITY;
+#pragma unroll
+            for (int i = 0; i < PFA_BK; i++) {
+                s[i] = (i <= lim) ? __fmul_rn(s[i], scale) : -INFINITY;
+                mx = fmaxf(mx, s[i]);
+            }
+            const float mn = fmaxf(m, mx);
+            const float c = (mn == -INFINITY) ? 1.0f : expf(m - mn);
+            m = mn;
+            l *= c;
+            uint32_t ph[PFA_BK / 2], pl[PFA_BK / 2];
+#pragma unroll
+            for (int i = 0; i < PFA_BK; i += 2) {
+                const float p0 = expf(s[i] - mn), p1 = expf(s[i + 1] - mn);
+                l += p0 + p1;
+                pfa_split2(p0, p1, ph[i / 2], pl[i / 2]);
+            }
+            if (j > 0) {
+                pf_wait(sb + PFA_BAR_PVDONE, (j - 1) & 1);
+                asm volatile("tcgen05.fence::after_thread_sync;" ::: "memory");
+            }
+#pragma unroll
+            for (int cc = 0; cc < 8; cc++) {
+                const uint32_t a = prow + ((cc ^ psw) << 4);
+                asm volatile("st.shared.v4.b32 [%0], {%1,%2,%3,%4};" ::"r"(a), "r"(ph[4 * cc]), "r"(ph[4 * cc + 1]), "r"(ph[4 * cc + 2]), "r"(ph[4 * cc + 3]) : "memory");
+                asm volatile("st.shared.v4.b32 [%0], {%1,%2,%3,%4};" ::"r"(a + PFA_M * PFA_BK * 2), "r"(pl[4 * cc]), "r"(pl[4 * cc + 1]), "r"(pl[4 * cc + 2]), "r"(pl[4 * cc + 3]) : "memory");
+            }
+            asm volatile("fence.proxy.async.shared::cta;" ::: "memory");
+            if (j > 0 && __any_sync(0xffffffffu, c != 1.0f)) {
+#pragma unroll 1
+                for (int cb = 0; cb < HEAD_DIM; cb += 32) {
+                    uint32_t d[32];
+                    PFA_LD32(d, trow + cb);
+                    pf_wait_ld();
+#pragma unroll
+                    for (int i = 0; i < 32; i++) d[i] = __float_as_uint(__fmul_rn(__uint_as_float(d[i]), c));
+                    PFA_ST32(trow + cb, d);
+                }
+                asm volatile("tcgen05.wait::st.sync.aligned;" ::: "memory");
+            }
+            asm volatile("tcgen05.fence::before_thread_sync;" ::: "memory");
+            pf_arrive(sb + PFA_BAR_PFULL);
+        }
+        pf_wait(sb + PFA_BAR_PVDONE, (ntiles - 1) & 1);
+        asm volatile("tcgen05.fence::after_thread_sync;" ::: "memory");
+        const float inv = __fdiv_rn(1.0f, l);
         const int tq = q0 + r / KVMUL;
-        float4 v0 = make_float4(0.f, 0.f, 0.f, 0.f), v1 = v0;
-        if (tq < T) {
-            const float4 *src = reinterpret_cast<const float4 *>(q + (size_t)tq * AH + (size_t)(kvhd * KVMUL + r % KVMUL) * HEAD_DIM + c * 8);
-            v0 = src[0];
-            v1 = src[1];
-        }
-        uint32_t h[4], l[4];
-        pfh_split2(v0.x, v0.y, h[0], l[0]);
-        pfh_split2(v0.z, v0.w, h[1], l[1]);
-        pfh_split2(v1.x, v1.y, h[2], l[2]);
-        pfh_split2(v1.z, v1.w, h[3], l[3]);
-        const uint32_t off = r * 256 + ((c ^ (r & 7)) << 4);
-        asm volatile("st.shared.v4.b32 [%0], {%1,%2,%3,%4};" ::"r"(sQ + off), "r"(h[0]), "r"(h[1]), "r"(h[2]), "r"(h[3]) : "memory");
-        asm volatile("st.shared.v4.b32 [%0], {%1,%2,%3,%4};" ::"r"(sQ + QL + off), "r"(l[0]), "r"(l[1]), "r"(l[2]), "r"(l[3]) : "memory");
-    }
-    const int r0 = warp * 16 + g, r1 = r0 + 8;
-    const int qp0 = pos0 + q0 + r0 / KVMUL, qp1 = pos0 + q0 + r1 / KVMUL;
-    float m0 = -INFINITY, m1 = -INFINITY, l0 = 0.0f, l1 = 0.0f;
-    float o[16][4];
-#pragma unroll
-    for (int j = 0; j < 16; j++) o[j][0] = o[j][1] = o[j][2] = o[j][3] = 0.0f;
-    const int a_row = warp * 16 + (lane & 7) + ((lane >> 3) & 1) * 8, a_cg = (lane >> 4) & 1;
-    const int b_key = (lane & 7) + ((lane >> 4) & 1) * 8, b_cg = (lane >> 3) & 1;
-    const int v_key = (lane & 7) + ((lane >> 3) & 1) * 8, v_cg = (lane >> 4) & 1;
-
-    for (int tile = 0; tile < ntiles; tile++) {
-        const int st = tile & 1, k0 = tile * PFH_BK;
-        if (tile + 1 < ntiles) {
-            load_stage(tile + 1, st ^ 1);
-            asm volatile("cp.async.wait_group 1;" ::: "memory");
-        } else {
-            asm volatile("cp.async.wait_group 0;" ::: "memory");
-        }
-        __syncthreads();
-        const uint32_t sKh = sKV + st * STAGE, sKl = sKh + ARR, sVh = sKh + 2 * ARR, sVl = sKh + 3 * ARR;
-        float s[4][4];
-#pragma unroll
-        for (int j = 0; j < 4; j++) s[j][0] = s[j][1] = s[j][2] = s[j][3] = 0.0f;
-#pragma unroll
-        for (int ks = 0; ks < 8; ks++) {
-            uint32_t ah[4], al[4];
-            const uint32_t aoff = a_row * 256 + (((2 * ks + a_cg) ^ (a_row & 7)) << 4);
-            ldsm4(ah, sQ + aoff);
-            ldsm4(al, sQ + QL + aoff);
-            uint32_t bh[2][4], bl[2][4];
-#pragma unroll
-            for (int jj = 0; jj < 2; jj++) {
-                const int key = 16 * jj + b_key;
-                const uint32_t boff = key * 256 + (((2 * ks + b_cg) ^ (key & 7)) << 4);
-                ldsm4(bh[jj], sKh + boff);
-                ldsm4(bl[jj], sKl + boff);
-            }
-#pragma unroll
-            for (int j = 0; j < 4; j++) mma_f16(s[j], al[0], al[1], al[2], al[3], bh[j >> 1][2 * (j & 1)], bh[j >> 1][2 * (j & 1) + 1]);
-#pragma unroll
-            for (int j = 0; j < 4; j++) mma_f16(s[j], ah[0], ah[1], ah[2], ah[3], bl[j >> 1][2 * (j & 1)], bl[j >> 1][2 * (j & 1) + 1]);
-#pragma unroll
-            for (int j = 0; j < 4; j++) mma_f16(s[j], ah[0], ah[1], ah[2], ah[3], bh[j >> 1][2 * (j & 1)], bh[j >> 1][2 * (j & 1) + 1]);
-        }
-        float mx0 = -INFINITY, mx1 = -INFINITY;
-#pragma unroll
-        for (int j = 0; j < 4; j++) {
-            const int key = k0 + 8 * j + 2 * t;
-            s[j][0] = (key <= qp0) ? __fmul_rn(s[j][0], scale) : -INFINITY;
-            s[j][1] = (key + 1 <= qp0) ? __fmul_rn(s[j][1], scale) : -INFINITY;
-            s[j][2] = (key <= qp1) ? __fmul_rn(s[j][2], scale) : -INFINITY;
-            s[j][3] = (key + 1 <= qp1) ? __fmul_rn(s[j][3], scale) : -INFINITY;
-            mx0 = fmaxf(mx0, fmaxf(s[j][0], s[j][1]));
-            mx1 = fmaxf(mx1, fmaxf(s[j][2], s[j][3]));
-        }
-        mx0 = fmaxf(mx0, __shfl_xor_sync(0xffffffffu, mx0, 1));
-        mx0 = fmaxf(mx0, __shfl_xor_sync(0xffffffffu, mx0, 2));
-        mx1 = fmaxf(mx1, __shfl_xor_sync(0xffffffffu, mx1, 1));
-        mx1 = fmaxf(mx1, __shfl_xor_sync(0xffffffffu, mx1, 2));
-        const float mn0 = fmaxf(m0, mx0), mn1 = fmaxf(m1, mx1);
-        const float c0 = (mn0 == -INFINITY) ? 1.0f : expf(m0 - mn0), c1 = (mn1 == -INFINITY) ? 1.0f : expf(m1 - mn1);
-        m0 = mn0;
-        m1 = mn1;
-        l0 *= c0;
-        l1 *= c1;
-#pragma unroll
-        for (int j = 0; j < 16; j++) {
-            o[j][0] *= c0;
-            o[j][1] *= c0;
-            o[j][2] *= c1;
-            o[j][3] *= c1;
-        }
-#pragma unroll
-        for (int kk = 0; kk < 2; kk++) {
-            uint32_t ph[4], pl[4];
-#pragma unroll
-            for (int h2 = 0; h2 < 2; h2++) {
-                const float *sj = s[2 * kk + h2];
-                const float p00 = (sj[0] == -INFINITY) ? 0.0f : expf(sj[0] - mn0), p01 = (sj[1] == -INFINITY) ? 0.0f : expf(sj[1] - mn0);
-                const float p10 = (sj[2] == -INFINITY) ? 0.0f : expf(sj[2] - mn1), p11 = (sj[3] == -INFINITY) ? 0.0f : expf(sj[3] - mn1);
-                l0 += p00 + p01;
-                l1 += p10 + p11;
-                pfh_split2(p00, p01, ph[2 * h2], pl[2 * h2]);
-                pfh_split2(p10, p11, ph[2 * h2 + 1], pl[2 * h2 + 1]);
-            }
-            const int key = 16 * kk + v_key;
-#pragma unroll
-            for (int n4 = 0; n4 < 4; n4++) {
-                uint32_t vh[2][4], vl[2][4];
-#pragma unroll
-                for (int h2 = 0; h2 < 2; h2++) {
-                    const int nn = 2 * n4 + h2;
-                    const uint32_t voff = key * 256 + (((2 * nn + v_cg) ^ (key & 7)) << 4);
-                    ldsm4t(vh[h2], sVh + voff);
-                    ldsm4t(vl[h2], sVl + voff);
-                }
-#pragma unroll
-                for (int j = 0; j < 4; j++) mma_f16(o[4 * n4 + j], pl[0], pl[1], pl[2], pl[3], vh[j >> 1][2 * (j & 1)], vh[j >> 1][2 * (j & 1) + 1]);
-#pragma unroll
-                for (int j = 0; j < 4; j++) mma_f16(o[4 * n4 + j], ph[0], ph[1], ph[2], ph[3], vl[j >> 1][2 * (j & 1)], vl[j >> 1][2 * (j & 1) + 1]);
-#pragma unroll
-                for (int j = 0; j < 4; j++) mma_f16(o[4 * n4 + j], ph[0], ph[1], ph[2], ph[3], vh[j >> 1][2 * (j & 1)], vh[j >> 1][2 * (j & 1) + 1]);
-            }
-        }
-        __syncthreads();
-    }
-    l0 += __shfl_xor_sync(0xffffffffu, l0, 1);
-    l0 += __shfl_xor_sync(0xffffffffu, l0, 2);
-    l1 += __shfl_xor_sync(0xffffffffu, l1, 1);
-    l1 += __shfl_xor_sync(0xffffffffu, l1, 2);
-    const float i0 = __fdiv_rn(1.0f, l0), i1 = __fdiv_rn(1.0f, l1);
-    const int tq0 = q0 + r0 / KVMUL, tq1 = q0 + r1 / KVMUL;
-    float *d0 = out + (size_t)tq0 * AH + (size_t)(kvhd * KVMUL + r0 % KVMUL) * HEAD_DIM + 2 * t;
-    float *d1 = out + (size_t)tq1 * AH + (size_t)(kvhd * KVMUL + r1 % KVMUL) * HEAD_DIM + 2 * t;
-#pragma unroll
-    for (int n = 0; n < 16; n++) {
-        if (tq0 < T) *reinterpret_cast<float2 *>(d0 + 8 * n) = make_float2(__fmul_rn(o[n][0], i0), __fmul_rn(o[n][1], i0));
-        if (tq1 < T) *reinterpret_cast<float2 *>(d1 + 8 * n) = make_float2(__fmul_rn(o[n][2], i1), __fmul_rn(o[n][3], i1));
-    }
-}
+        float *dst = out + (size_t)tq * AH + (size_t)(kvhd * KVMUL + r % KVMUL) * HEAD_DIM;
+#pragma unroll 1
+        for (int cb = 0; cb < HEAD_DIM; cb += 32) {
+            uint32_t d[32];
+            PFA_LD32(d, trow + cb);
+            pf_wait_ld();
+            if (tq < T) {
+#pragma unroll
+                for (int i = 0; i < 32; i += 4)
+                    *reinterpret_cast<float4 *>(dst + cb + i) = make_float4(__fmul_rn(__uint_as_float(d[i]), inv), __fmul_rn(__uint_as_float(d[i + 1]), inv),
+                                                                            __fmul_rn(__uint_as_float(d[i + 2]), inv), __fmul_rn(__uint_as_float(d[i + 3]), inv));
+            }
+        }
+    }
+    asm volatile("tcgen05.fence::before_thread_sync;" ::: "memory");
+    __syncthreads();
+    if (warp == PFA_MMA_WARP) {
+        asm volatile("tcgen05.fence::after_thread_sync;" ::: "memory");
+        asm volatile("tcgen05.dealloc.cta_group::1.sync.aligned.b32 %0, %1;" ::"r"(tmem_base), "n"(256) : "memory");
+    }
+}
+#undef PFA_LD32
+#undef PFA_ST32
 
 struct PfPeers {
     const float *part[MEGA_MAX_TP];
```

Result: no change. 454.5 (median of 6 runs) (-0.1%).
